# SpectacularAI/3dgs-deblur

Hardware: AMD Instinct MI355X
Metric: fwd+bwd rasterize MPix/s at 1M Gaussians, 1080p, 5 sub-poses (higher is better)
Workload: dtype f32

## Files before the change

3dgs-deblur_amd/_lib.py:

```python
from __future__ import annotations

import ctypes
from pathlib import Path

from ._build import LIB_PATH, build_library

_P, _I, _F, _L = ctypes.c_void_p, ctypes.c_int, ctypes.c_float, ctypes.c_longlong

_SIGS = {
    "gs_subpose_viewmats_fwd": [_I, _P, _P, _P, _P, _P, _P],
    "gs_subpose_viewmats_bwd": [_I, _P, _P, _P, _P, _P, _P, _P, _P, _P],
    "gs_project_fwd": [_I, _P, _P, _F, _P, _P, _F, _F, _F, _F, _I, _I, _F, _P, _P, _P, _P, _P, _P, _P, _P, _P],
    "gs_project_bwd": [_I, _P, _P, _F, _P, _P, _F, _F, _F, _F, _I, _I, _F, _P, _P, _P, _P, _P, _P, _P, _P, _I, _P, _L, _P],
    "gs_sh_fwd": [_I, _I, _I, _P, _P, _P, _P],
    "gs_sh_bwd": [_I, _I, _I, _P, _P, _P, _P],
    "gs_project_fused_fwd": [_I, _I, _P, _P, _F, _P, _P, _P, _I, _I, _P, _F, _F, _F, _F, _I, _I, _F, _I, _I,
                             _P, _P, _P, _P, _P, _I, _P],
    "gs_slice_colors": [_I, _P, _P, _I, _P, _P, _P, _I, _I, _P, _P, _P],
    "gs_project_fused_bwd": [_I, _I, _P, _P, _F, _P, _P, _P, _I, _I, _P, _F, _F, _F, _F, _I, _I, _F, _I,
                             _P, _P, _P, _P, _P, _P, _P, _P, _P, _P, _I, _P, _I, _P, _P, _L, _P],
    "gs_project_pixvel_fwd": [_I, _I, _P, _P, _F, _P, _P, _P, _I, _I, _P, _P, _P, _F, _F, _F, _F, _I, _I, _F, _I, _I,
                              _P, _P, _P, _P, _F, _P, _P, _I, _P],
    "gs_rasterize_fwd_rs_slice": [_P, _P, _P, _P, _I, _I, _I, _P, _P, _P, _P, _P, _I, _I, _P, _I, _P, _P, _P, _I, _F, _P,
                                  _P],
    "gs_rasterize_bwd_rs_slice": [_P, _P, _P, _P, _P, _I, _I, _I, _P, _P, _P, _P, _P, _P, _P, _P, _P, _I, _I, _P, _F, _F,
                                  _P, _I, _F, _P, _P],
    "gs_project_pixvel_bwd": [_I, _I, _P, _P, _F, _P, _P, _P, _I, _I, _P, _P, _P, _F, _F, _F, _F, _I, _I, _F, _I,
                              _P, _P, _P, _P, _P, _P, _P, _P, _P, _P, _P, _I, _P, _I, _P, _P, _L, _P],
    "gs_pack_records": [_I, _P, _P, _P, _P, _P, _P, _I, _I, _P, _P, _P, _P],
    "gs_unpack_record_grads": [_I, _P, _P, _P, _P, _P, _P],
    "gs_exclusive_scan_u32": [_L, _P, _P, _P, _P, _L, _P],
    "gs_radix_sort_pairs_u32": [_L, _P, _P, _P, _P, _I, _I, _I, _P, _L, ctypes.POINTER(_I), _P],
    "gs_radix_sort_pairs_u64": [_L, _P, _P, _P, _P, _I, _I, _I, _P, _L, ctypes.POINTER(_I), _P],
    "gs_radix_sort_pairs_gather_u32": [_L, _P, _P, _P, _P, _I, _I, _I, _P, _L, ctypes.POINTER(_I), _P, _P, _P, _P],
    "gs_radix_sort_pairs_carry_u32": [_L, _P, _P, _P, _P, _I, _I, _I, _P, _L, ctypes.POINTER(_I), _P, _P, _P,
                                      ctypes.POINTER(_I), _P, _P],
    "gs_segmented_sort_pairs_u32": [_L, _L, _P, _P, _P, _P, _I, _I, _I, _P, _L, ctypes.POINTER(_I), _P],
    "gs_segmented_sort_compact_u32": [_L, _L, _P, _P, _P, _P, _I, _I, _I, ctypes.c_uint, _P, _P, _P, _P, _L,
                                      ctypes.POINTER(_I), _P],
    "gs_segmented_sort_select_u32": [_L, _L, _P, _P, _P, _P, _P, _I, _I, _I, ctypes.c_uint, _P, _P, _P, _P, _P, _P, _L,
                                     ctypes.POINTER(_I), _L, _P],
    "gs_depth_select": [_L, _L, _P, _P, _L, _P, _P, _P, _L, _P],
    "gs_exclusive_scan_segments_u32": [_L, _L, _P, _P, _P, _P, _P, _L, _P],
    "gs_make_depth_keys64": [_L, _I, _P, _P, _P],
    "gs_gather_counts": [_L, _P, _P, _P, _P],
    "gs_emit_intersects": [_L, _I, _I, _I, _P, _P, _P, _L, _P, _P, ctypes.c_uint, _P],
    "gs_tile_bin_edges_u32": [_L, _P, _I, _P, _P, _P],
    "gs_tile_bin_edges_u64": [_L, _P, _I, _P, _P],
    "gs_tile_bin_edges_ids_u32": [_L, _P, _I, _P, _P, _P, _P, _P],
    "gs_map_gaussian_to_intersects": [_I, _P, _P, _P, _P, _I, _I, _P, _P, _P],
    "gs_rasterize_fwd": [_P, _P, _P, _P, _P, _I, _I, _I, _I, _P, _P, _P, _I, _I, _P],
    "gs_rasterize_bwd": [_P, _P, _P, _P, _P, _I, _I, _I, _I, _P, _P, _P, _P, _P, _I, _I, _P],
    "gs_slice_plan": [_I, _I, _I, _P, _P, _L, _P, _P, _P, _P, _P, _P],
    "gs_slice_plan_select": [_I, _I, _I, _P, _P, _P, _P, _P, _P, _P, _P, _P],
    "gs_tile_open_sat": [_I, _I, _I, _P, _P, _P, _P, _P],
    "gs_slice_counts": [_I, _I, _I, _P, _P, _P, _P, _P, _I, _I, _P, _P, _P],
    "gs_emit_open_intersects": [_I, _I, _I, _I, _P, _P, _P, _P, _P, _P, _P, ctypes.c_uint, _I, _I, _P, _P, _P, _P],
    "gs_slice_counts_exact": [_I, _I, _I, _P, _P, _P, _P, _P, _P, _I, _I, _P, _P, _I, _P, _P, _P, _P, _P, _P],
    "gs_slice_counts_exact_swept": [_I, _I, _I, _P, _P, _P, _P, _P, _P, _I, _I, _P, _P, _I, _P, _P, _P, _P, _P, _F, _F, _F,
                                    _P],
    "gs_rasterize_fwd_slice": [_P, _P, _P, _P, _P, _I, _I, _I, _I, _P, _P, _P, _P, _P, _I, _I, _P, _P, _I, _P, _P, _P,
                               _I, _P],
    "gs_rasterize_bwd_slice": [_P, _P, _P, _P, _P, _I, _I, _I, _I, _P, _P, _P, _P, _P, _P, _P, _P, _P, _P, _P, _I, _P,
                               _I, _P, _F, _F, _P],
    "gs_rasterize_fwd_slice_stats": [_P, _P, _P, _P, _P, _I, _I, _I, _I, _P, _P, _P, _P, _P, _I, _I, _P, _P, _P, _P],
    "gs_reduce_grad_tuples": [_I, _P, _P, _P, _P, _P, _P, _P, _L, _P, _I, _P],
    "gs_combine_fwd": [_I, _L, _P, _F, _F, _P, _P],
    "gs_combine_bwd": [_I, _L, _P, _F, _F, _P, _P, _P, _P],
    "gs_combine_bwd_scale": [_I, _L, _F, _P, _P, _P, _P],
    "gs_combine_fwd_batched": [_I, _I, _L, _P, _F, _F, _P, _P],
    "gs_combine_bwd_batched": [_I, _I, _L, _P, _F, _F, _P, _P, _P, _P],
    "gs_combine_bwd_scale_batched": [_I, _I, _L, _F, _P, _P, _P, _P],
    "gs_dp_row_mask": [_I, _I, _P, _P, _P, _P],
    "gs_dp_pack_rows": [_L, _P, _I, _P, _P, _P, _P],
    "gs_dp_scatter_add_rows": [_L, _P, _I, _P, _P, _F, _P],
    "gs_dp_pack_masked_rows": [_I, _P, _P, _I, _P, _I, _P, _P, _P, _P],
    "gs_dp_scatter_add_payload": [_I, _P, _I, _P, _P, _F, _P],
    "gs_slice_project_records": [_I, _I, _I, _P, _P, _P, _P, _I, _I, _P, _P],
    "gs_project_records": [_I, _I, _P, _I, _I, _P, _P],
    "gs_frame_forward": [_P, _P, _P, _P, _P, _P, _P, _P, _P, _P, _I, _I, _P, _P, _P, _P, _P, _P, _P, _P, _L, _P, _L, _P, _P],
    "gs_frame_backward": [_P, _P, _P, _P, _P, _P, _P, _P, _F, _F, _I, _P, _P, _P, _P, _P, _L, _P],
    "gs_frame_backward_depth": [_P, _P, _P, _P, _P, _P, _P, _P, _F, _F, _I, _P, _P, _P, _P, _P, _L, _P, _P],
    "gs_xy_absgrad_sum": [_I, _I, _I, _P, _P, _P, _P],
    "gs_frame_profile_enable": [ctypes.c_uint],
    "gs_frame_profile_read": [_I, _P, _P],
    "gs_image_loss_fwd_bwd": [_I, _I, _P, _P, _F, _P, _P, _P, _L, _P],
    "gs_adam_step": [_I, _P, _P, _P, _P, _P, _P, ctypes.c_double, ctypes.c_double, ctypes.c_double, _I, _P],
    "gs_adam_step_rows": [_I, _I, _P, _P, _P, _P, _P, _P, _P, ctypes.c_double, ctypes.c_double, ctypes.c_double, _I,
                          _P, _L, _P],
    "gs_visible_rows": [_I, _I, _P, _P, _P],
    "gs_mcmc_inject_noise": [_I, _P, _P, _P, _P, _F, _L, _L, _P, _P, _P],
    "gs_mcmc_relocation": [_I, _P, _P, _P, _P, _P, _P],
    "gs_bilagrid_slice_fwd": [_I, _I, _I, _I, _I, _I, _I, _P, _P, _P, _P, _P],
    "gs_bilagrid_slice_bwd": [_I, _I, _I, _I, _I, _I, _I, _P, _P, _P, _P, _P, _P, _P, _L, _P],
    "gs_bilagrid_tv_fwd_bwd": [_I, _I, _I, _I, _P, _F, _P, _P, _P, _L, _P],
}
_SIGS_LL = {
    "gs_scan_workspace_bytes": [_L],
    "gs_radix_sort_workspace_bytes": [_L, _I, _I],
    "gs_segmented_sort_workspace_bytes": [_L, _L, _I, _I],
    "gs_segmented_sort_compact_workspace_bytes": [_L, _L, _I, _I, _I],
    "gs_depth_select_workspace_bytes": [_I],
    "gs_project_pose_scratch_bytes": [_I, _I, _I],
    "gs_image_loss_workspace_bytes": [_I, _I],
    "gs_adam_step_rows_workspace_bytes": [_I],
    "gs_frame_backward_bytes": [_P],
    "gs_bilagrid_slice_bwd_workspace_bytes": [_I, _I, _I, _I, _I, _I, _I],
    "gs_bilagrid_tv_workspace_bytes": [_I, _I, _I, _I],
}

_lib = None


class HipLibraryError(RuntimeError):
    pass


def load(build_if_missing: bool = True) -> ctypes.CDLL:
    global _lib
    if _lib is not None:
        return _lib
    import os
    import shutil
    override = os.environ.get("GSD_LIB_PATH")
    path = Path(override) if override else LIB_PATH
    if not override and build_if_missing and shutil.which(os.environ.get("HIPCC", "/opt/rocm/bin/hipcc")):
        from ._build import is_current, HASH_PATH, CSRC
        stale = not is_current()
        if stale and path.exists() and not HASH_PATH.exists():
            t = path.stat().st_mtime
            stale = any(f.stat().st_mtime > t for f in list(CSRC.glob("*.hip")) + list(CSRC.glob("*.h")))
        if stale:
            import fcntl
            try:
                lock = open(str(path) + ".lock", "w")
            except OSError as e:
                if not path.exists():
                    raise HipLibraryError(f"{path} is missing and {path.parent} is not writable: {e}") from e
                import warnings
                warnings.warn(f"{path} may be older than its sources and {path.parent} is not writable; loading it as is")
            else:
                with lock:
                    fcntl.flock(lock, fcntl.LOCK_EX)
                    try:
                        build_library()
                    finally:
                        fcntl.flock(lock, fcntl.LOCK_UN)
    if not path.exists():
        raise HipLibraryError(f"{path} is missing; run __graft_entry__.build()")
    try:
        lib = ctypes.CDLL(str(path))
    except OSError as e:
        raise HipLibraryError(f"cannot load HIP library {path}: {e}") from e
    for name, args in _SIGS.items():
        fn = getattr(lib, name)
        fn.argtypes = args
        fn.restype = _I
    for name, args in _SIGS_LL.items():
        fn = getattr(lib, name)
        fn.argtypes = args
        fn.restype = _L
    lib.gs_version.restype = ctypes.c_char_p
    lib.gs_version.argtypes = []
    _lib = lib
    return lib


def exported_names():
    return sorted(list(_SIGS) + list(_SIGS_LL) + ["gs_version"])


def check(status: int, what: str) -> None:
    if status != 0:
# ... 5 lines not shown
```

3dgs-deblur_amd/csrc/project.hip:

```cpp
#include "gs_common.h"
#include "../../include/gsdeblur.h"

namespace gs {

__global__ void subpose_fwd_kernel(int P, const float* __restrict__ V0, const float* __restrict__ lin,
                                   const float* __restrict__ ang, const float* __restrict__ times,
                                   float* __restrict__ out) {
  int p = blockIdx.x * blockDim.x + threadIdx.x;
  if (p >= P) return;
  float v0[12], l[3], a[3], o[12];
  for (int j = 0; j < 12; ++j) v0[j] = V0[j];
  for (int j = 0; j < 3; ++j) { l[j] = lin[j]; a[j] = ang[j]; }
  subpose_viewmat<float>(v0, l, a, times[p], o);
  for (int j = 0; j < 12; ++j) out[16 * p + j] = o[j];
  out[16 * p + 12] = 0.f; out[16 * p + 13] = 0.f; out[16 * p + 14] = 0.f; out[16 * p + 15] = 1.f;
}

__global__ __launch_bounds__(256) void subpose_bwd_kernel(int P, const float* __restrict__ V0, const float* __restrict__ lin,
                                   const float* __restrict__ ang, const float* __restrict__ times,
                                   const float* __restrict__ v_out, float* __restrict__ v_V0,
                                   float* __restrict__ v_lin, float* __restrict__ v_ang) {
  typedef Dual<1> D;
  extern __shared__ float sp_part[];
  for (int gid = threadIdx.x; gid < P * 18; gid += blockDim.x) {
    const int p = gid / 18, t = gid - p * 18;
    D dV[12], dl[3], da[3], o[12];
    for (int j = 0; j < 12; ++j) { dV[j] = D(V0[j]); dV[j].d[0] = (j == t) ? 1.f : 0.f; }
    for (int j = 0; j < 3; ++j) {
      dl[j] = D(lin[j]); dl[j].d[0] = (12 + j == t) ? 1.f : 0.f;
      da[j] = D(ang[j]); da[j].d[0] = (15 + j == t) ? 1.f : 0.f;
    }
    subpose_viewmat<D>(dV, dl, da, D(times[p]), o);
    float acc = 0.f;
    for (int j = 0; j < 12; ++j) acc += v_out[16 * p + j] * o[j].d[0];
    sp_part[gid] = acc;
  }
  __syncthreads();
  if (threadIdx.x < 18) {
    const int t = threadIdx.x;
    float sum = 0.f;
    for (int p = 0; p < P; ++p) sum += sp_part[p * 18 + t];
    float* dst = t < 12 ? v_V0 + t : (t < 15 ? v_lin + (t - 12) : v_ang + (t - 15));
    *dst += sum;
  }
}

struct Intrin { float fx, fy, cx, cy; int W, H, tiles_x, tiles_y; float clip; };

__global__ __launch_bounds__(256) void project_fwd_kernel(int N, const float* __restrict__ means,
    const float* __restrict__ scales, float glob, const float* __restrict__ quats, const float* __restrict__ V,
    Intrin in, float* __restrict__ xys, float* __restrict__ depths, int* __restrict__ radii,
    float* __restrict__ conics, float* __restrict__ comp, int* __restrict__ ntiles, float* __restrict__ cov3d,
    int* __restrict__ tbounds) {
  int i = blockIdx.x * blockDim.x + threadIdx.x;
  if (i >= N) return;
  float Vm[12];
  for (int j = 0; j < 12; ++j) Vm[j] = V[j];
  float m[3] = {means[3 * i], means[3 * i + 1], means[3 * i + 2]};
  float s[3] = {scales[3 * i], scales[3 * i + 1], scales[3 * i + 2]};
  float q[4] = {quats[4 * i], quats[4 * i + 1], quats[4 * i + 2], quats[4 * i + 3]};
  float R[9], qn[4], inv, M[9], c3[6];
  quat_to_rotmat(q, R, qn, &inv);
  scale_rot_to_cov3d(s, glob, R, M, c3);
  Proj o; ProjCtx k;
  bool ok = project_one(m, c3, Vm, in.fx, in.fy, in.cx, in.cy, in.W, in.H, in.tiles_x, in.tiles_y, in.clip, o, k);
  for (int j = 0; j < 6; ++j) cov3d[6 * i + j] = c3[j];
  depths[i] = o.depth;
  radii[i] = ok ? o.radius : 0;
  ntiles[i] = ok ? o.ntiles : 0;
  xys[2 * i] = ok ? o.x : 0.f; xys[2 * i + 1] = ok ? o.y : 0.f;
  conics[3 * i] = ok ? o.conic_x : 0.f; conics[3 * i + 1] = ok ? o.conic_y : 0.f; conics[3 * i + 2] = ok ? o.conic_z : 0.f;
  comp[i] = ok ? o.comp : 0.f;
  if (tbounds) {
    tbounds[4 * i] = o.tmin_x; tbounds[4 * i + 1] = o.tmin_y; tbounds[4 * i + 2] = o.tmax_x; tbounds[4 * i + 3] = o.tmax_y;
  }
}

__device__ __forceinline__ void reduce_vV(const float vV[12], float* __restrict__ acc , float* lds ) {
  const int lane = lane_id(), wave = threadIdx.x >> 6;
#pragma unroll
  for (int j = 0; j < 12; ++j) {
    float t = wave_sum_to_lane63(vV[j]);
    if (lane == 63) lds[wave * 12 + j] = t;
  }
  __syncthreads();
  if (threadIdx.x < 12) acc[threadIdx.x] += (lds[threadIdx.x] + lds[12 + threadIdx.x]) + (lds[24 + threadIdx.x] + lds[36 + threadIdx.x]);
  __syncthreads();
}

struct PoseDst { float* slot0; float* slot1; int stride; };
__global__ __launch_bounds__(256) void pose_reduce_kernel(const float* __restrict__ partial, int nblocks, int slots,
                                                          PoseDst dst) {
  __shared__ double red[256][13];
  const int sl = blockIdx.x;
  float* out = (sl == 1 && dst.slot1) ? dst.slot1 : dst.slot0 + (size_t)sl * dst.stride;
  if (!out) return;
  double a[12];
#pragma unroll
  for (int j = 0; j < 12; ++j) a[j] = 0.0;
  for (int b = threadIdx.x; b < nblocks; b += 256) {
    const float* row = partial + ((size_t)b * slots + sl) * 12;
#pragma unroll
    for (int j = 0; j < 12; ++j) a[j] += (double)row[j];
  }
#pragma unroll
  for (int j = 0; j < 12; ++j) red[threadIdx.x][j] = a[j];
  __syncthreads();
  for (int w = 128; w > 0; w >>= 1) {
    if ((int)threadIdx.x < w)
#pragma unroll
      for (int j = 0; j < 12; ++j) red[threadIdx.x][j] += red[threadIdx.x + w][j];
    __syncthreads();
  }
  if (threadIdx.x < 12) out[threadIdx.x] += (float)red[0][threadIdx.x];
}

__global__ __launch_bounds__(256) void project_bwd_kernel(int N, const float* __restrict__ means,
    const float* __restrict__ scales, float glob, const float* __restrict__ quats, const float* __restrict__ V,
    Intrin in, const float* __restrict__ v_xys, const float* __restrict__ v_depths,
    const float* __restrict__ v_conics, const float* __restrict__ v_comp, float* __restrict__ v_means,
    float* __restrict__ v_scales, float* __restrict__ v_quats, float* __restrict__ v_V ,
    int flags) {
  __shared__ float lds[48];
  __shared__ float acc[12];
  if (threadIdx.x < 12) acc[threadIdx.x] = 0.f;
  int i = blockIdx.x * blockDim.x + threadIdx.x;
  float vV[12];
  for (int j = 0; j < 12; ++j) vV[j] = 0.f;
  if (i < N) {
    float Vm[12];
    for (int j = 0; j < 12; ++j) Vm[j] = V[j];
    float m[3] = {means[3 * i], means[3 * i + 1], means[3 * i + 2]};
    float s[3] = {scales[3 * i], scales[3 * i + 1], scales[3 * i + 2]};
    float q[4] = {quats[4 * i], quats[4 * i + 1], quats[4 * i + 2], quats[4 * i + 3]};
    float R[9], qn[4], inv, M[9], c3[6];
    quat_to_rotmat(q, R, qn, &inv);
    scale_rot_to_cov3d(s, glob, R, M, c3);
    Proj o; ProjCtx k;
    bool ok = project_one(m, c3, Vm, in.fx, in.fy, in.cx, in.cy, in.W, in.H, in.tiles_x, in.tiles_y, in.clip, o, k);
    float vm[3] = {0.f, 0.f, 0.f}, vs[3] = {0.f, 0.f, 0.f}, vq[4] = {0.f, 0.f, 0.f, 0.f};
    if (ok) {
      float vxy[2] = {v_xys[2 * i], v_xys[2 * i + 1]};
      float vc[3] = {v_conics[3 * i], v_conics[3 * i + 1], v_conics[3 * i + 2]};
      float vc3[6];
      project_one_bwd(m, c3, Vm, in.fx, in.fy, k, o.comp, vxy, v_depths ? v_depths[i] : 0.f, vc,
                      v_comp ? v_comp[i] : 0.f, vm, vc3, vV, nullptr, (flags & 1) != 0);
      cov3d_bwd(s, glob, q, vc3, vs, vq, (flags & 2) != 0);
    }
    for (int j = 0; j < 3; ++j) { v_means[3 * i + j] = vm[j]; v_scales[3 * i + j] = vs[j]; }
    for (int j = 0; j < 4; ++j) v_quats[4 * i + j] = vq[j];
  }
  if (v_V) {
    __syncthreads();
    reduce_vV(vV, acc, lds);
    if (threadIdx.x < 12) v_V[(size_t)blockIdx.x * 12 + threadIdx.x] = acc[threadIdx.x];
  }
}

__global__ __launch_bounds__(256) void sh_fwd_kernel(int N, int K_stride, int deg, const float* __restrict__ dirs,
                                                     const float* __restrict__ coeffs, float* __restrict__ colors) {
  int i = blockIdx.x * blockDim.x + threadIdx.x;
  if (i >= N) return;
  float x = dirs[3 * i], y = dirs[3 * i + 1], z = dirs[3 * i + 2];
  float inv = 1.0f / sqrtf(x * x + y * y + z * z);
  float B[25];
  sh_basis(deg, x * inv, y * inv, z * inv, B);
  int nb = (deg + 1) * (deg + 1);
  float r = 0.f, g = 0.f, b = 0.f;
  const float* c = coeffs + (size_t)i * K_stride * 3;
#pragma unroll
  for (int k = 0; k < 25; ++k)
    if (k < nb) { r += B[k] * c[3 * k]; g += B[k] * c[3 * k + 1]; b += B[k] * c[3 * k + 2]; }
  colors[3 * i] = r; colors[3 * i + 1] = g; colors[3 * i + 2] = b;
}

__global__ __launch_bounds__(256) void sh_bwd_kernel(int N, int K_stride, int deg, const float* __restrict__ dirs,
                                                     const float* __restrict__ v_colors, float* __restrict__ v_coeffs) {
  int i = blockIdx.x * blockDim.x + threadIdx.x;
  if (i >= N) return;
  float x = dirs[3 * i], y = dirs[3 * i + 1], z = dirs[3 * i + 2];
  float inv = 1.0f / sqrtf(x * x + y * y + z * z);
  float B[25];
  sh_basis(deg, x * inv, y * inv, z * inv, B);
  int nb = (deg + 1) * (deg + 1);
  float r = v_colors[3 * i], g = v_colors[3 * i + 1], b = v_colors[3 * i + 2];
  float* c = v_coeffs + (size_t)i * K_stride * 3;
#pragma unroll
  for (int k = 0; k < 25; ++k) {
    if (k < K_stride) {
      float bk = k < nb ? B[k] : 0.f;
      c[3 * k] = bk * r; c[3 * k + 1] = bk * g; c[3 * k + 2] = bk * b;
    }
  }
  for (int k = 25; k < K_stride; ++k) { c[3 * k] = 0.f; c[3 * k + 1] = 0.f; c[3 * k + 2] = 0.f; }
}

__device__ __forceinline__ void tile_bbox(float x, float y, int radius, int tiles_x, int tiles_y, int& x0, int& y0,
                                          int& x1, int& y1) {
  const float inv_tile = 1.0f / (float)K::kTile;
  float radf = (float)radius;
  float tcx = x * inv_tile, tcy = y * inv_tile, tr = radf * inv_tile;
  x0 = (int)(tcx - tr); x1 = (int)(tcx + tr + 1.0f);
  y0 = (int)(tcy - tr); y1 = (int)(tcy + tr + 1.0f);
  x0 = x0 < 0 ? 0 : (x0 > tiles_x ? tiles_x : x0);
  x1 = x1 < 0 ? 0 : (x1 > tiles_x ? tiles_x : x1);
  y0 = y0 < 0 ? 0 : (y0 > tiles_y ? tiles_y : y0);
  y1 = y1 < 0 ? 0 : (y1 > tiles_y ? tiles_y : y1);
}

__global__ __launch_bounds__(256) void pack_records_kernel(int N, const float* __restrict__ xys,
    const float* __restrict__ depths, const int* __restrict__ radii, const float* __restrict__ conics,
    const float* __restrict__ colors, const float* __restrict__ opacity, int tiles_x, int tiles_y,
    float* __restrict__ records, unsigned* __restrict__ depth_keys, int* __restrict__ ntiles) {
  int i = blockIdx.x * blockDim.x + threadIdx.x;
  if (i >= N) return;
  int rad = radii[i];
  int x0 = 0, y0 = 0, x1 = 0, y1 = 0;
  float x = xys[2 * i], y = xys[2 * i + 1];
  if (rad > 0) tile_bbox(x, y, rad, tiles_x, tiles_y, x0, y0, x1, y1);
  int area = (x1 - x0) * (y1 - y0);
  bool ok = rad > 0 && area > 0;
  float4* r = reinterpret_cast<float4*>(records + (size_t)i * kRecFloats);
  float d = depths[i];
  if (ok) {
    r[0] = make_float4(x, y, conics[3 * i], conics[3 * i + 1]);
    r[1] = make_float4(conics[3 * i + 2], opacity[i], colors[3 * i], colors[3 * i + 1]);
    r[2] = make_float4(colors[3 * i + 2], d, __int_as_float(x0 | (y0 << 16)), __int_as_float(x1 | (y1 << 16)));
    float aux[4];
    rec_aux(opacity[i], conics[3 * i], conics[3 * i + 2], aux);
    r[3] = make_float4(aux[0], aux[1], aux[2], aux[3]);
  } else {
    r[0] = make_float4(0.f, 0.f, 0.f, 0.f); r[1] = r[0]; r[2] = r[0]; r[3] = r[0];
  }
  depth_keys[i] = ok ? (unsigned)__float_as_int(d) : 0xFFFFFFFFu;
  ntiles[i] = ok ? area : 0;
}

__global__ __launch_bounds__(256) void unpack_grads_kernel(int N, const float* __restrict__ v_records,
    float* __restrict__ v_xys, float* __restrict__ v_conics, float* __restrict__ v_colors,
    float* __restrict__ v_opacity) {
  int i = blockIdx.x * blockDim.x + threadIdx.x;
  if (i >= N) return;
  const float4* r = reinterpret_cast<const float4*>(v_records + (size_t)i * kGradFloats);
  float4 a = r[0], b = r[1], c = r[2];
  v_xys[2 * i] = a.x; v_xys[2 * i + 1] = a.y;
  v_conics[3 * i] = a.z; v_conics[3 * i + 1] = a.w; v_conics[3 * i + 2] = b.x;
  v_opacity[i] = b.y;
  v_colors[3 * i] = b.z; v_colors[3 * i + 1] = b.w; v_colors[3 * i + 2] = c.x;
}

struct FusedParams {
  int N, P;
  const float* means; const float* scales; const float* quats; const float* opacities;
  const float* sh;
  const float* viewmats;
  float glob;
  int K_stride, deg, antialiased;
  int defer_color;
  int skip_culled;
  int no_records;
  int records_only;
  int rs_bands;
  Intrin in;
  int pixvel;
  const float* twist;
  const float* times;
  int flags;
  float rs_half;
  float* pix_vel_out;
  int act;
  const float* sh_rest;
};
constexpr int GS_ACT_LOG_SCALES = 1, GS_ACT_OPACITY_LOGITS = 2;

__device__ __forceinline__ void load_scales(const FusedParams& fp, int i, float s[3]) {
  s[0] = fp.scales[3 * i]; s[1] = fp.scales[3 * i + 1]; s[2] = fp.scales[3 * i + 2];
  if (fp.act & GS_ACT_LOG_SCALES) { s[0] = expf(s[0]); s[1] = expf(s[1]); s[2] = expf(s[2]); }
}
__device__ __forceinline__ float load_opacity(const FusedParams& fp, int i) {
  const float o = fp.opacities[i];
  return (fp.act & GS_ACT_OPACITY_LOGITS) ? 1.0f / (1.0f + expf(-o)) : o;
}
__device__ __forceinline__ void sh_rows(const float* __restrict__ sh, const float* __restrict__ sh_rest, int K_stride,
                                        size_t i, const float*& c0, const float*& c1) {
  if (sh_rest) { c0 = sh + i * 3; c1 = sh_rest + i * (size_t)(K_stride - 1) * 3; }
  else { c0 = sh + i * (size_t)K_stride * 3; c1 = c0 + 3; }
}

constexpr int GS_FLAG_UPSTREAM_FOV_CLAMP_GRAD = 1;
constexpr int GS_FLAG_RAW_QUAT_GRAD = 2;
constexpr int GS_FLAG_NO_NEEDLE_HP = 8;
constexpr int GS_FLAG_RS_PIXVEL_GRAD = 16;
constexpr int GS_FLAG_DEPTH_GRAD = 64;
constexpr float kNeedleRatio = 8.0f;

template <int MAXB, bool DEFER>
__global__ __launch_bounds__(256) void project_fused_fwd_kernel(FusedParams fp, float* __restrict__ records,
    unsigned* __restrict__ depth_keys, int* __restrict__ ntiles, int* __restrict__ radii) {
  int i = blockIdx.x * blockDim.x + threadIdx.x;
  if (i >= fp.N) return;
  float m[3] = {fp.means[3 * i], fp.means[3 * i + 1], fp.means[3 * i + 2]};
  float s[3];
  load_scales(fp, i, s);
  float q[4] = {fp.quats[4 * i], fp.quats[4 * i + 1], fp.quats[4 * i + 2], fp.quats[4 * i + 3]};
  float opac = load_opacity(fp, i);
  float R[9], qn[4], inv, M[9], c3[6];
  quat_to_rotmat(q, R, qn, &inv);
  scale_rot_to_cov3d(s, fp.glob, R, M, c3);
  const int nb = (fp.deg + 1) * (fp.deg + 1);
  float coef[DEFER ? 1 : MAXB * 3];
  if (!DEFER) {
    const float *c0, *c1;
    sh_rows(fp.sh, fp.sh_rest, fp.K_stride, (size_t)i, c0, c1);
#pragma unroll
    for (int k = 0; k < MAXB * 3; ++k) coef[DEFER ? 0 : k] = (k < nb * 3) ? (k < 3 ? c0[k] : c1[k - 3]) : 0.f;
  }
  Proj o0; ProjCtx k0;
  float pv[2] = {0.f, 0.f};
  if (fp.pixvel) {
    float Vm0[12];
#pragma unroll
    for (int j = 0; j < 12; ++j) Vm0[j] = fp.viewmats[j];
    project_one(m, c3, Vm0, fp.in.fx, fp.in.fy, fp.in.cx, fp.in.cy, fp.in.W, fp.in.H, fp.in.tiles_x, fp.in.tiles_y,
                fp.in.clip, o0, k0);
    if (k0.geom_ok) {
      const float lin[3] = {fp.twist[0], fp.twist[1], fp.twist[2]}, ang[3] = {fp.twist[3], fp.twist[4], fp.twist[5]};
      pixel_velocity(k0.pc, k0.clamp_x ? k0.tx : k0.pc[0], k0.clamp_y ? k0.ty : k0.pc[1], k0.rz, fp.in.fx, fp.in.fy,
                     lin, ang, pv);
    }
    if (fp.pix_vel_out) { fp.pix_vel_out[2 * i] = pv[0]; fp.pix_vel_out[2 * i + 1] = pv[1]; }
  }
  for (int p = 0; p < fp.P; ++p) {
    const float* V = fp.viewmats + (fp.pixvel ? 0 : 16 * p);
    float Vm[12];
#pragma unroll
    for (int j = 0; j < 12; ++j) Vm[j] = V[j];
    Proj o; ProjCtx k;
    bool ok;
    if (fp.pixvel) {
      o = o0; k = k0;
      ok = k0.geom_ok != 0;
      if (ok) {
        const float tau = fp.times[p];
        o.x = o0.x + tau * pv[0];
        o.y = o0.y + tau * pv[1];
        o.radius = (int)k0.radf;
        if (fp.rs_half != 0.f)
          ok = tile_bounds_swept(o.x - fp.rs_half * pv[0], o.y - fp.rs_half * pv[1], o.x + fp.rs_half * pv[0],
                                 o.y + fp.rs_half * pv[1], k0.radf, fp.in.tiles_x, fp.in.tiles_y, o);
        else
          ok = tile_bounds(o.x, o.y, k0.radf, fp.in.tiles_x, fp.in.tiles_y, o);
      }
    } else {
      ok = project_one(m, c3, Vm, fp.in.fx, fp.in.fy, fp.in.cx, fp.in.cy, fp.in.W, fp.in.H, fp.in.tiles_x,
                       fp.in.tiles_y, fp.in.clip, o, k);
    }
    size_t idx = (size_t)p * fp.N + i;
    float4* r = reinterpret_cast<float4*>(records + idx * kRecFloats);
    const int radius_out = ok ? o.radius : 0;
    if (ok && fp.rs_bands > 1) {
      const int rb = p % fp.rs_bands;
      const int by0 = (rb * fp.in.tiles_y) / fp.rs_bands, by1 = ((rb + 1) * fp.in.tiles_y) / fp.rs_bands;
      o.tmin_y = max(o.tmin_y, by0);
      o.tmax_y = min(o.tmax_y, by1);
      ok = o.tmax_y > o.tmin_y;
      o.ntiles = ok ? (o.tmax_x - o.tmin_x) * (o.tmax_y - o.tmin_y) : 0;
    }
    if (fp.no_records) {
    } else if (ok) {
      float cxw = -(Vm[0] * Vm[3] + Vm[4] * Vm[7] + Vm[8] * Vm[11]);
      float cyw = -(Vm[1] * Vm[3] + Vm[5] * Vm[7] + Vm[9] * Vm[11]);
      float czw = -(Vm[2] * Vm[3] + Vm[6] * Vm[7] + Vm[10] * Vm[11]);
      float dx = m[0] - cxw, dy = m[1] - cyw, dz = m[2] - czw;
      float dinv = 1.0f / sqrtf(dx * dx + dy * dy + dz * dz);
      float cr = 0.f, cg = 0.f, cb = 0.f;
      if (!DEFER) {
        float B[MAXB];
        sh_basis(fp.deg, dx * dinv, dy * dinv, dz * dinv, B);
        cr = 0.5f; cg = 0.5f; cb = 0.5f;
#pragma unroll
        for (int b = 0; b < MAXB; ++b) {
          if (b < nb) {
            cr += B[b] * coef[DEFER ? 0 : 3 * b]; cg += B[b] * coef[DEFER ? 0 : 3 * b + 1];
            cb += B[b] * coef[DEFER ? 0 : 3 * b + 2];
          }
        }
        cr = fmaxf(cr, 0.f); cg = fmaxf(cg, 0.f); cb = fmaxf(cb, 0.f);
      }
      float op = fp.antialiased ? opac * o.comp : opac;
      float aux[4];
      rec_aux(op, o.conic_x, o.conic_z, aux);
      r[0] = make_float4(o.x, o.y, o.conic_x, o.conic_y);
      if (fp.records_only) {
        float* rf = reinterpret_cast<float*>(r);
        rf[4] = o.conic_z; rf[5] = op; rf[9] = o.depth;
        rf[10] = __int_as_float(o.tmin_x | (o.tmin_y << 16)); rf[11] = __int_as_float(o.tmax_x | (o.tmax_y << 16));
      } else {
        r[1] = make_float4(o.conic_z, op, cr, cg);
        r[2] = make_float4(cb, o.depth, __int_as_float(o.tmin_x | (o.tmin_y << 16)),
                           __int_as_float(o.tmax_x | (o.tmax_y << 16)));
      }
      r[3] = make_float4(aux[0], aux[1], aux[2], aux[3]);
    } else if (!fp.skip_culled) {
      float4 z = make_float4(0.f, 0.f, 0.f, 0.f);
      r[0] = z; r[1] = z; r[2] = z; r[3] = z;
    }
    if (fp.records_only) continue;
    depth_keys[idx] = ok ? (unsigned)__float_as_int(o.depth) : 0xFFFFFFFFu;
    ntiles[idx] = ok ? o.ntiles : 0;
    if (radii) radii[idx] = radius_out;
  }
}

struct FusedOut {
  float* v_means; float* v_scales; float* v_quats; float* v_opac; float* v_sh; float* v_sh_rest;
  float* v_viewmats;
  float* v_xy_sum;
  float* v_twist;
  float* pose_partial;
};

template <int MAXB, bool DEPTH>
__device__ __forceinline__ void fused_bwd_body(const FusedParams& fp, const float* __restrict__ records,
    const float* __restrict__ v_records, const FusedOut& out, const unsigned char* __restrict__ touched,
    int i, bool live, float* lds, float* __restrict__ blk_acc ) {
  float* __restrict__ v_means = out.v_means; float* __restrict__ v_scales = out.v_scales;
  float* __restrict__ v_quats = out.v_quats; float* __restrict__ v_opac = out.v_opac;
  float* __restrict__ v_sh = out.v_sh; float* __restrict__ v_sh_rest = out.v_sh_rest;
  float* __restrict__ v_viewmats = out.v_viewmats; float* __restrict__ v_xy_sum = out.v_xy_sum;
  float* __restrict__ v_twist = out.v_twist;
  const int ii = live ? i : 0;
  float m[3] = {0.f, 0.f, 1.f}, s[3] = {1.f, 1.f, 1.f}, q[4] = {1.f, 0.f, 0.f, 0.f}, opac = 0.f;
  if (live) {
    m[0] = fp.means[3 * ii]; m[1] = fp.means[3 * ii + 1]; m[2] = fp.means[3 * ii + 2];
    load_scales(fp, ii, s);
    q[0] = fp.quats[4 * ii]; q[1] = fp.quats[4 * ii + 1]; q[2] = fp.quats[4 * ii + 2]; q[3] = fp.quats[4 * ii + 3];
    opac = load_opacity(fp, ii);
  }
  float R[9], qn[4], inv, M[9], c3[6];
  quat_to_rotmat(q, R, qn, &inv);
  scale_rot_to_cov3d(s, fp.glob, R, M, c3);
  const int nb = (fp.deg + 1) * (fp.deg + 1);
  float vcoef[MAXB * 3];
#pragma unroll
  for (int k = 0; k < MAXB * 3; ++k) vcoef[k] = 0.f;
  float vm[3] = {0.f, 0.f, 0.f}, vc3[6] = {0.f, 0.f, 0.f, 0.f, 0.f, 0.f}, vop = 0.f, vxs = 0.f, vys = 0.f;
  const bool up_clamp = (fp.flags & GS_FLAG_UPSTREAM_FOV_CLAMP_GRAD) != 0;
  if (fp.pixvel) {
    float Vm[12];
#pragma unroll
    for (int j = 0; j < 12; ++j) Vm[j] = fp.viewmats[j];
    float vV[12], vtw[12];
#pragma unroll
    for (int j = 0; j < 12; ++j) { vV[j] = 0.f; vtw[j] = 0.f; }
    bool mine = false;
    if (live)
      for (int p = 0; p < fp.P; ++p) mine |= (!touched || touched[(size_t)p * fp.N + ii]);
    if (mine) {
      Proj o; ProjCtx k;
      project_one(m, c3, Vm, fp.in.fx, fp.in.fy, fp.in.cx, fp.in.cy, fp.in.W, fp.in.H, fp.in.tiles_x, fp.in.tiles_y,
                  fp.in.clip, o, k);
      if (k.geom_ok) {
        float vxy[2] = {0.f, 0.f}, vpv[2] = {0.f, 0.f}, vcon[3] = {0.f, 0.f, 0.f}, v_comp = 0.f;
        float vr = 0.f, vg = 0.f, vb = 0.f, vz = 0.f;
        for (int p = 0; p < fp.P; ++p) {
          if (touched && !touched[(size_t)p * fp.N + ii]) continue;
          const float tau = fp.times[p];
          size_t idx = (size_t)p * fp.N + ii;
          const float4* g4 = reinterpret_cast<const float4*>(v_records + idx * kGradFloats);
          float4 ga = g4[0], gb = g4[1], gc = g4[2];
          const float4* r4 = reinterpret_cast<const float4*>(records + idx * kRecFloats);
          float4 ra = r4[0], rb = r4[1], rc = r4[2];
          if (ra.z == 0.f && ra.w == 0.f && rb.x == 0.f) continue;
          vr += rb.z > 0.f ? gb.z : 0.f; vg += rb.w > 0.f ? gb.w : 0.f; vb += rc.x > 0.f ? gc.x : 0.f;
          if (fp.antialiased) { vop += gb.y * o.comp; v_comp += gb.y * opac; } else { vop += gb.y; }
          vxy[0] += ga.x; vxy[1] += ga.y;
          vpv[0] += tau * ga.x; vpv[1] += tau * ga.y;
          if (fp.flags & GS_FLAG_RS_PIXVEL_GRAD) { vpv[0] += gc.y; vpv[1] += gc.z; }
          vcon[0] += ga.z; vcon[1] += ga.w; vcon[2] += gb.x;
          if (DEPTH) vz += gc.w;
        }
        vxs = vxy[0]; vys = vxy[1];
        if (vr != 0.f || vg != 0.f || vb != 0.f) {
          float cxw = -(Vm[0] * Vm[3] + Vm[4] * Vm[7] + Vm[8] * Vm[11]);
          float cyw = -(Vm[1] * Vm[3] + Vm[5] * Vm[7] + Vm[9] * Vm[11]);
          float czw = -(Vm[2] * Vm[3] + Vm[6] * Vm[7] + Vm[10] * Vm[11]);
          float dx = m[0] - cxw, dy = m[1] - cyw, dz = m[2] - czw;
          float dinv = 1.0f / sqrtf(dx * dx + dy * dy + dz * dz);
          float B[MAXB];
          sh_basis(fp.deg, dx * dinv, dy * dinv, dz * dinv, B);
#pragma unroll
          for (int b = 0; b < MAXB; ++b) {
            if (b < nb) { vcoef[3 * b] += B[b] * vr; vcoef[3 * b + 1] += B[b] * vg; vcoef[3 * b + 2] += B[b] * vb; }
          }
        }
        const float lin[3] = {fp.twist[0], fp.twist[1], fp.twist[2]}, ang[3] = {fp.twist[3], fp.twist[4], fp.twist[5]};
        float vpc[3], vlin[3], vang[3];
        pixel_velocity_bwd(k.pc, k.clamp_x ? k.tx : k.pc[0], k.clamp_y ? k.ty : k.pc[1], k.clamp_x, k.clamp_y, up_clamp,
                           k.rz, fp.in.fx, fp.in.fy, lin, ang, vpv, vpc, vlin, vang);
        vtw[0] = vlin[0]; vtw[1] = vlin[1]; vtw[2] = vlin[2]; vtw[3] = vang[0]; vtw[4] = vang[1]; vtw[5] = vang[2];
        project_one_bwd(m, c3, Vm, fp.in.fx, fp.in.fy, k, o.comp, vxy, DEPTH ? vz : 0.f, vcon, v_comp, vm, vc3, vV, vpc,
                        up_clamp);
      }
    }
    if (__syncthreads_or(mine)) {
      if (v_viewmats) reduce_vV(vV, blk_acc, lds);
      if (v_twist) reduce_vV(vtw, blk_acc + 12, lds);
    }
  } else
  for (int p = 0; p < fp.P; ++p) {
    const float* V = fp.viewmats + 16 * p;
    float Vm[12];
#pragma unroll
    for (int j = 0; j < 12; ++j) Vm[j] = V[j];
    float vV[12];
#pragma unroll
    for (int j = 0; j < 12; ++j) vV[j] = 0.f;
    const bool mine = live && (!touched || touched[(size_t)p * fp.N + ii]);
    if (mine) {
      Proj o; ProjCtx k;
      bool ok = project_one(m, c3, Vm, fp.in.fx, fp.in.fy, fp.in.cx, fp.in.cy, fp.in.W, fp.in.H, fp.in.tiles_x,
                            fp.in.tiles_y, fp.in.clip, o, k);
      if (ok) {
        size_t idx = (size_t)p * fp.N + ii;
        const float4* g4 = reinterpret_cast<const float4*>(v_records + idx * kGradFloats);
        float4 ga = g4[0], gb = g4[1], gc = g4[2];
        const float4* r4 = reinterpret_cast<const float4*>(records + idx * kRecFloats);
        float4 rb = r4[1], rc = r4[2];
        float vr = rb.z > 0.f ? gb.z : 0.f, vg = rb.w > 0.f ? gb.w : 0.f, vb = rc.x > 0.f ? gc.x : 0.f;
        if (vr != 0.f || vg != 0.f || vb != 0.f) {
          float cxw = -(Vm[0] * Vm[3] + Vm[4] * Vm[7] + Vm[8] * Vm[11]);
          float cyw = -(Vm[1] * Vm[3] + Vm[5] * Vm[7] + Vm[9] * Vm[11]);
          float czw = -(Vm[2] * Vm[3] + Vm[6] * Vm[7] + Vm[10] * Vm[11]);
          float dx = m[0] - cxw, dy = m[1] - cyw, dz = m[2] - czw;
          float dinv = 1.0f / sqrtf(dx * dx + dy * dy + dz * dz);
          float B[MAXB];
          sh_basis(fp.deg, dx * dinv, dy * dinv, dz * dinv, B);
#pragma unroll
          for (int b = 0; b < MAXB; ++b) {
            if (b < nb) { vcoef[3 * b] += B[b] * vr; vcoef[3 * b + 1] += B[b] * vg; vcoef[3 * b + 2] += B[b] * vb; }
          }
        }
        float v_comp = 0.f;
        if (fp.antialiased) { vop += gb.y * o.comp; v_comp = gb.y * opac; } else { vop += gb.y; }
        float vxy[2] = {ga.x, ga.y};
        vxs += ga.x; vys += ga.y;
        float vcon[3] = {ga.z, ga.w, gb.x};
        float vm1[3], vc31[6];
        project_one_bwd(m, c3, Vm, fp.in.fx, fp.in.fy, k, o.comp, vxy, DEPTH ? gc.w : 0.f, vcon, v_comp, vm1, vc31, vV,
                        nullptr, up_clamp);
        for (int j = 0; j < 3; ++j) vm[j] += vm1[j];
        for (int j = 0; j < 6; ++j) vc3[j] += vc31[j];
      }
    }
    if (v_viewmats && __syncthreads_or(mine)) reduce_vV(vV, blk_acc + 12 * p, lds);
  }
  if (!live) return;
  float vs[3], vq[4];
  cov3d_bwd(s, fp.glob, q, vc3, vs, vq, (fp.flags & GS_FLAG_RAW_QUAT_GRAD) != 0);
  if (fp.act & GS_ACT_LOG_SCALES) { vs[0] *= s[0]; vs[1] *= s[1]; vs[2] *= s[2]; }
  if (fp.act & GS_ACT_OPACITY_LOGITS) vop *= opac * (1.0f - opac);
  for (int j = 0; j < 3; ++j) { v_means[3 * i + j] = vm[j]; v_scales[3 * i + j] = vs[j]; }
  for (int j = 0; j < 4; ++j) v_quats[4 * i + j] = vq[j];
  v_opac[i] = vop;
  if (v_xy_sum) { v_xy_sum[2 * i] = vxs; v_xy_sum[2 * i + 1] = vys; }
  float *c0, *c1;
  if (v_sh_rest) { c0 = v_sh + (size_t)i * 3; c1 = v_sh_rest + (size_t)i * (fp.K_stride - 1) * 3; }
  else { c0 = v_sh + (size_t)i * fp.K_stride * 3; c1 = c0 + 3; }
  const int kn = fp.K_stride * 3;
#pragma unroll
  for (int k = 0; k < MAXB * 3; ++k)
    if (k < kn) { if (k < 3) c0[k] = vcoef[k]; else c1[k - 3] = vcoef[k]; }
  for (int k = MAXB * 3; k < kn; ++k) c1[k - 3] = 0.f;
}

template <bool DEPTH>
__device__ __forceinline__ void needle_item_se3(const FusedParams& fp, const float* __restrict__ records,
                                                const float* __restrict__ v_records,
                                                const unsigned char* __restrict__ touched, int i, int p, double out[9]) {
#pragma unroll
  for (int j = 0; j < 9; ++j) out[j] = 0.0;
  if (touched && !touched[(size_t)p * fp.N + i]) return;
  float s[3];
  load_scales(fp, i, s);
  const float m[3] = {fp.means[3 * i], fp.means[3 * i + 1], fp.means[3 * i + 2]};
  const float q[4] = {fp.quats[4 * i], fp.quats[4 * i + 1], fp.quats[4 * i + 2], fp.quats[4 * i + 3]};
  float R[9], qn[4], inv, M[9], c3[6];
  quat_to_rotmat(q, R, qn, &inv);
  scale_rot_to_cov3d(s, fp.glob, R, M, c3);
  const float* V = fp.viewmats + 16 * p;
  float Vm[12];
#pragma unroll
  for (int j = 0; j < 12; ++j) Vm[j] = V[j];
  Proj o; ProjCtx k;
  if (!project_one(m, c3, Vm, fp.in.fx, fp.in.fy, fp.in.cx, fp.in.cy, fp.in.W, fp.in.H, fp.in.tiles_x, fp.in.tiles_y,
                   fp.in.clip, o, k))
    return;
  double Rd[9], qnd[4], invd, Md[9], c3d[6];
  quat_to_rotmat_t<double>(q, Rd, qnd, &invd);
  scale_rot_to_cov3d_t<double>(s, fp.glob, Rd, Md, c3d);
  ProjCtxT<double> kd;
  project_ctx_t<double>(m, c3d, Vm, fp.in.fx, fp.in.fy, fp.in.W, fp.in.H, kd);
  kd.clamp_x = k.clamp_x; kd.clamp_y = k.clamp_y;
  const double comp = ::sqrt(fmax(0.0, kd.det0 / kd.det));
  const size_t idx = (size_t)p * fp.N + i;
  const float4* g4 = reinterpret_cast<const float4*>(v_records + idx * kGradFloats);
  const float4 ga = g4[0], gb = g4[1];
  const double vxy[2] = {ga.x, ga.y}, vcon[3] = {ga.z, ga.w, gb.x};
  const double v_comp = fp.antialiased ? (double)gb.y * (double)load_opacity(fp, i) : 0.0;
  const double vz = DEPTH ? (double)g4[2].w : 0.0;
  double vV[12];
  project_one_bwd_t<double>(m, c3d, Vm, fp.in.fx, fp.in.fy, kd, comp, vxy, vz, vcon, v_comp, out, out + 3, vV, nullptr,
                            (fp.flags & GS_FLAG_UPSTREAM_FOV_CLAMP_GRAD) != 0);
}

template <bool DEPTH>
__device__ __forceinline__ void needle_item_pixvel(const FusedParams& fp, const float* __restrict__ records,
                                                   const float* __restrict__ v_records,
                                                   const unsigned char* __restrict__ touched, int i, double out[9]) {
#pragma unroll
  for (int j = 0; j < 9; ++j) out[j] = 0.0;
  float s[3];
  load_scales(fp, i, s);
  const float m[3] = {fp.means[3 * i], fp.means[3 * i + 1], fp.means[3 * i + 2]};
  const float q[4] = {fp.quats[4 * i], fp.quats[4 * i + 1], fp.quats[4 * i + 2], fp.quats[4 * i + 3]};
  const float opac = load_opacity(fp, i);
  float R[9], qn[4], inv, M[9], c3[6];
  quat_to_rotmat(q, R, qn, &inv);
  scale_rot_to_cov3d(s, fp.glob, R, M, c3);
  float Vm[12];
#pragma unroll
  for (int j = 0; j < 12; ++j) Vm[j] = fp.viewmats[j];
  Proj o; ProjCtx k;
  project_one(m, c3, Vm, fp.in.fx, fp.in.fy, fp.in.cx, fp.in.cy, fp.in.W, fp.in.H, fp.in.tiles_x, fp.in.tiles_y,
              fp.in.clip, o, k);
  if (!k.geom_ok) return;
  double Rd[9], qnd[4], invd, Md[9], c3d[6];
  quat_to_rotmat_t<double>(q, Rd, qnd, &invd);
  scale_rot_to_cov3d_t<double>(s, fp.glob, Rd, Md, c3d);
  ProjCtxT<double> kd;
  project_ctx_t<double>(m, c3d, Vm, fp.in.fx, fp.in.fy, fp.in.W, fp.in.H, kd);
  kd.clamp_x = k.clamp_x; kd.clamp_y = k.clamp_y;
  const double comp = ::sqrt(fmax(0.0, kd.det0 / kd.det));
  double vxy[2] = {0., 0.}, vcon[3] = {0., 0., 0.}, v_comp = 0., vz = 0.;
  float vpv[2] = {0.f, 0.f};
  for (int p = 0; p < fp.P; ++p) {
    if (touched && !touched[(size_t)p * fp.N + i]) continue;
    const size_t idx = (size_t)p * fp.N + i;
    const float4* g4 = reinterpret_cast<const float4*>(v_records + idx * kGradFloats);
    const float4 ga = g4[0], gb = g4[1], gc = g4[2];
    const float4* r4 = reinterpret_cast<const float4*>(records + idx * kRecFloats);
    const float4 ra = r4[0], rb = r4[1];
    if (ra.z == 0.f && ra.w == 0.f && rb.x == 0.f) continue;
    if (fp.antialiased) v_comp += (double)gb.y * (double)opac;
    vxy[0] += ga.x; vxy[1] += ga.y;
    vpv[0] += fp.times[p] * ga.x; vpv[1] += fp.times[p] * ga.y;
    if (fp.flags & GS_FLAG_RS_PIXVEL_GRAD) { vpv[0] += gc.y; vpv[1] += gc.z; }
    vcon[0] += ga.z; vcon[1] += ga.w; vcon[2] += gb.x;
    if (DEPTH) vz += (double)gc.w;
  }
  const float lin[3] = {fp.twist[0], fp.twist[1], fp.twist[2]}, ang[3] = {fp.twist[3], fp.twist[4], fp.twist[5]};
  float vpc[3], vlin[3], vang[3];
  pixel_velocity_bwd(k.pc, k.clamp_x ? k.tx : k.pc[0], k.clamp_y ? k.ty : k.pc[1], k.clamp_x, k.clamp_y,
                     (fp.flags & GS_FLAG_UPSTREAM_FOV_CLAMP_GRAD) != 0, k.rz, fp.in.fx, fp.in.fy, lin, ang, vpv, vpc,
                     vlin, vang);
  const double vpcd[3] = {vpc[0], vpc[1], vpc[2]};
  double vV[12];
  project_one_bwd_t<double>(m, c3d, Vm, fp.in.fx, fp.in.fy, kd, comp, vxy, vz, vcon, v_comp, out, out + 3, vV, vpcd,
                            (fp.flags & GS_FLAG_UPSTREAM_FOV_CLAMP_GRAD) != 0);
}

constexpr int kNeedleChunk = 2048;

#define GS_NEEDLE_HP_KERNEL(NAME, DEPTH)                                                                                \
__global__ __launch_bounds__(256) void NAME(FusedParams fp, const float* __restrict__ records,                          \
    const float* __restrict__ v_records, float* __restrict__ v_means, float* __restrict__ v_scales,                    \
    float* __restrict__ v_quats, const unsigned char* __restrict__ touched, float ratio_limit) {                       \
  __shared__ int list[kNeedleChunk];                                                                                          \
  __shared__ int n_list;                                                                                                      \
  __shared__ double part[256][9];                                                                                             \
  if (threadIdx.x == 0) n_list = 0;                                                                                           \
  __syncthreads();                                                                                                            \
  const int i0 = blockIdx.x * kNeedleChunk + (int)threadIdx.x * 8;                                                            \
  if (i0 < fp.N) {                                                                                                            \
    unsigned long long any = ~0ull;                                                                                           \
    if (touched) {                                                                                                            \
      any = 0ull;                                                                                                             \
      const bool word = (fp.N % 8) == 0 && i0 + 8 <= fp.N;                                                                    \
      for (int p = 0; p < fp.P; ++p) {                                                                                        \
        const unsigned char* t = touched + (size_t)p * fp.N + i0;                                                             \
        if (word) any |= *reinterpret_cast<const unsigned long long*>(t);                                                     \
        else for (int j = 0; j < 8 && i0 + j < fp.N; ++j) any |= (unsigned long long)t[j] << (8 * j);                         \
      }                                                                                                                       \
    }                                                                                                                         \
    if (any != 0ull) {                                                                                                        \
      for (int j = 0; j < 8 && i0 + j < fp.N; ++j) {                                                                          \
        if (((any >> (8 * j)) & 0xFFull) == 0ull) continue;                                                                   \
        const int i = i0 + j;                                                                                                 \
                                                             \
        const float s0 = fp.scales[3 * i], s1 = fp.scales[3 * i + 1], s2 = fp.scales[3 * i + 2];                              \
        const float smax = fmaxf(s0, fmaxf(s1, s2)), smin = fminf(s0, fminf(s1, s2));                                         \
        const bool needle = (fp.act & GS_ACT_LOG_SCALES) ? (smax - smin > __logf(ratio_limit)) : (smax > ratio_limit * smin); \
        if (needle) list[atomicAdd(&n_list, 1)] = i;                                                                          \
      }                                                                                                                       \
    }                                                                                                                         \
  }                                                                                                                           \
  __syncthreads();                                                                                                            \
  const int n = n_list;                                                                                                       \
  if (n == 0) return;                                                                                                         \
  const int items_per = fp.pixvel ? 1 : fp.P;                                                      \
  const int per_round = max(1, 256 / items_per);                                                       \
  for (int base = 0; base < n; base += per_round) {                                                                           \
    const int cnt = min(per_round, n - base);                                                                                 \
    const int a = (int)threadIdx.x / items_per, p = (int)threadIdx.x - a * items_per;                                         \
    if (a < cnt) {                                                                                                            \
      double o9[9];                                                                                                           \
      if (fp.pixvel) needle_item_pixvel<DEPTH>(fp, records, v_records, touched, list[base + a], o9);                          \
      else needle_item_se3<DEPTH>(fp, records, v_records, touched, list[base + a], p, o9);                                    \
_Pragma("unroll")                                                                                                             \
      for (int j = 0; j < 9; ++j) part[threadIdx.x][j] = o9[j];                                                               \
    }                                                                                                                         \
    __syncthreads();                                                                                                          \
    if ((int)threadIdx.x < cnt) {                                                                                             \
      const int i = list[base + threadIdx.x];                                                                                 \
      double acc[9] = {0., 0., 0., 0., 0., 0., 0., 0., 0.};                                                                   \
      for (int pp = 0; pp < items_per; ++pp)                                                                                  \
_Pragma("unroll")                                                                                                             \
        for (int j = 0; j < 9; ++j) acc[j] += part[threadIdx.x * items_per + pp][j];                                          \
      float s[3];                                                                                                             \
  load_scales(fp, i, s);                                                                                                      \
      const float q[4] = {fp.quats[4 * i], fp.quats[4 * i + 1], fp.quats[4 * i + 2], fp.quats[4 * i + 3]};                    \
      double vs[3], vq[4];                                                                                                    \
      cov3d_bwd_t<double>(s, fp.glob, q, acc + 3, vs, vq, (fp.flags & GS_FLAG_RAW_QUAT_GRAD) != 0);                           \
      if (fp.act & GS_ACT_LOG_SCALES) { vs[0] *= (double)s[0]; vs[1] *= (double)s[1]; vs[2] *= (double)s[2]; }                \
      for (int j = 0; j < 3; ++j) { v_means[3 * i + j] = (float)acc[j]; v_scales[3 * i + j] = (float)vs[j]; }                 \
      for (int j = 0; j < 4; ++j) v_quats[4 * i + j] = (float)vq[j];                                                          \
    }                                                                                                                         \
    __syncthreads();                                                                                                          \
  }                                                                                                                           \
}

GS_NEEDLE_HP_KERNEL(project_needle_hp_kernel, false)
GS_NEEDLE_HP_KERNEL(project_needle_hp_depth_kernel, true)

#define GS_FUSED_BWD_KERNEL(NAME, DEPTH)                                                                                \
template <int MAXB>                                                                                                     \
__global__ __launch_bounds__(256) void NAME(FusedParams fp, const float* __restrict__ records,                          \
    const float* __restrict__ v_records, FusedOut out) {                                                                \
  __shared__ float lds[48];                                                                                               \
  extern __shared__ float blk_acc[];                        \
  const int slots = out.pose_partial ? (fp.pixvel ? 2 : fp.P) : 0;                                                        \
  for (int k = threadIdx.x; k < slots * 12; k += 256) blk_acc[k] = 0.f;                                                   \
  __syncthreads();                                                                                                        \
  const int i = blockIdx.x * blockDim.x + threadIdx.x;                                                                    \
  fused_bwd_body<MAXB, DEPTH>(fp, records, v_records, out, nullptr, i, i < fp.N, lds, blk_acc);                           \
  __syncthreads();                                                                                                        \
  for (int k = threadIdx.x; k < slots * 12; k += 256) out.pose_partial[(size_t)blockIdx.x * slots * 12 + k] = blk_acc[k]; \
}

GS_FUSED_BWD_KERNEL(project_fused_bwd_kernel, false)
GS_FUSED_BWD_KERNEL(project_fused_bwd_depth_kernel, true)

constexpr int kFusedChunk = 2048;

__device__ __forceinline__ void zero_rows(float* __restrict__ base, size_t first, size_t count) {
  if (!base || count == 0) return;
  float* p = base + first;
  const size_t mis = ((reinterpret_cast<uintptr_t>(p) & 15u) != 0) ? ((16u - (reinterpret_cast<uintptr_t>(p) & 15u)) >> 2) : 0;
  const size_t head = mis < count ? mis : count;
  for (size_t k = threadIdx.x; k < head; k += blockDim.x) p[k] = 0.f;
  const size_t n4 = (count - head) >> 2;
  float4* p4 = reinterpret_cast<float4*>(p + head);
  for (size_t k = threadIdx.x; k < n4; k += blockDim.x) p4[k] = make_float4(0.f, 0.f, 0.f, 0.f);
  for (size_t k = head + 4 * n4 + threadIdx.x; k < count; k += blockDim.x) p[k] = 0.f;
}

#define GS_FUSED_BWD_SPARSE_KERNEL(NAME, DEPTH)                                                                         \
template <int MAXB, bool ZERO_FILL>                                                                                     \
__global__ __launch_bounds__(256, 2) void NAME(FusedParams fp,                                                          \
    const float* __restrict__ records, const float* __restrict__ v_records, FusedOut out,                               \
    const unsigned char* __restrict__ touched ) {                                                            \
  __shared__ float lds[48];                                                                                               \
  __shared__ int list[kFusedChunk];                                                                                       \
  __shared__ int wave_cnt[4];                                                                                             \
  extern __shared__ float blk_acc[];                        \
  const int slots = out.pose_partial ? (fp.pixvel ? 2 : fp.P) : 0;                                                        \
  for (int k = threadIdx.x; k < slots * 12; k += 256) blk_acc[k] = 0.f;                                                   \
  const int lane = lane_id(), wave = threadIdx.x >> 6;                                                                    \
  const int base = blockIdx.x * kFusedChunk;                                                                              \
  if (ZERO_FILL) {                                                                                                        \
    const size_t g0 = (size_t)base, cnt = (size_t)min(kFusedChunk, fp.N - base);                                          \
    zero_rows(out.v_means, 3 * g0, 3 * cnt);                                                                              \
    zero_rows(out.v_scales, 3 * g0, 3 * cnt);                                                                             \
    zero_rows(out.v_quats, 4 * g0, 4 * cnt);                                                                              \
    zero_rows(out.v_opac, g0, cnt);                                                                                       \
    if (out.v_sh_rest) {                                                                                                  \
      zero_rows(out.v_sh, 3 * g0, 3 * cnt);                                                                               \
      zero_rows(out.v_sh_rest, (size_t)(fp.K_stride - 1) * 3 * g0, (size_t)(fp.K_stride - 1) * 3 * cnt);                  \
    } else {                                                                                                              \
      zero_rows(out.v_sh, (size_t)fp.K_stride * 3 * g0, (size_t)fp.K_stride * 3 * cnt);                                   \
    }                                                                                                                     \
    zero_rows(out.v_xy_sum, 2 * g0, 2 * cnt);                                                                             \
                   \
    __threadfence_block();                                                                                                \
  }                                                                                                                       \
  int n_list = 0;                                                                                                         \
  for (int r = 0; r < kFusedChunk / 256; ++r) {                                                                           \
    const int g = base + r * 256 + (int)threadIdx.x;                                                                      \
    bool any = false;                                                                                                     \
    if (g < fp.N)                                                                                                         \
      for (int p = 0; p < fp.P; ++p) any |= touched[(size_t)p * fp.N + g] != 0;                                           \
    const unsigned long long bal = __ballot(any);                                                                         \
    if (lane == 0) wave_cnt[wave] = __popcll(bal);                                                                        \
    __syncthreads();                                                                                                      \
    int off = n_list, total = 0;                                                                                          \
_Pragma("unroll")                                                                                                         \
    for (int w = 0; w < 4; ++w) { const int c = wave_cnt[w]; if (w < wave) off += c; total += c; }                        \
    if (any) list[off + __popcll(bal & ((1ull << lane) - 1ull))] = g;                                                     \
    n_list += total;                                                                                                      \
    __syncthreads();                                                                                                      \
  }                                                                                                                       \
  for (int k0 = 0; k0 < n_list; k0 += 256) {                                                                              \
    const int k = k0 + (int)threadIdx.x;                                                                                  \
    const bool live = k < n_list;                                                                                         \
    fused_bwd_body<MAXB, DEPTH>(fp, records, v_records, out, touched, live ? list[k] : 0, live, lds, blk_acc);            \
  }                                                                                                                       \
  __syncthreads();                                                                                                        \
  for (int k = threadIdx.x; k < slots * 12; k += 256) out.pose_partial[(size_t)blockIdx.x * slots * 12 + k] = blk_acc[k]; \
}

GS_FUSED_BWD_SPARSE_KERNEL(project_fused_bwd_sparse_kernel, false)
GS_FUSED_BWD_SPARSE_KERNEL(project_fused_bwd_sparse_depth_kernel, true)

__global__ __launch_bounds__(256) void slice_records_kernel(int n_slice, SliceDesc sd, const unsigned* __restrict__ sorted_gi,
                                                            FusedParams fp, float* __restrict__ records) {
  const int j = blockIdx.x * 256 + threadIdx.x;
  if (j >= n_slice) return;
  const unsigned gi = sorted_gi[slice_rank(sd, j)];
  const int p = (int)(gi / (unsigned)fp.N), i = (int)(gi - (unsigned)p * (unsigned)fp.N);
  float m[3] = {fp.means[3 * i], fp.means[3 * i + 1], fp.means[3 * i + 2]};
  float sc[3];
  load_scales(fp, i, sc);
  float q[4] = {fp.quats[4 * i], fp.quats[4 * i + 1], fp.quats[4 * i + 2], fp.quats[4 * i + 3]};
  const float opac = load_opacity(fp, i);
  float R[9], qn[4], inv, M[9], c3[6];
  quat_to_rotmat(q, R, qn, &inv);
  scale_rot_to_cov3d(sc, fp.glob, R, M, c3);
  const float* V = fp.viewmats + 16 * p;
  float Vm[12];
#pragma unroll
  for (int k = 0; k < 12; ++k) Vm[k] = V[k];
  Proj o; ProjCtx k;
  bool ok = project_one(m, c3, Vm, fp.in.fx, fp.in.fy, fp.in.cx, fp.in.cy, fp.in.W, fp.in.H, fp.in.tiles_x,
                        fp.in.tiles_y, fp.in.clip, o, k);
  if (ok && fp.rs_bands > 1) {
    const int rb = p % fp.rs_bands;
    const int by0 = (rb * fp.in.tiles_y) / fp.rs_bands, by1 = ((rb + 1) * fp.in.tiles_y) / fp.rs_bands;
    o.tmin_y = max(o.tmin_y, by0);
    o.tmax_y = min(o.tmax_y, by1);
    ok = o.tmax_y > o.tmin_y;
  }
  float4* r = reinterpret_cast<float4*>(records + (size_t)gi * kRecFloats);
  if (ok) {
    const float op = fp.antialiased ? opac * o.comp : opac;
    float aux[4];
    rec_aux(op, o.conic_x, o.conic_z, aux);
    r[0] = make_float4(o.x, o.y, o.conic_x, o.conic_y);
    r[1] = make_float4(o.conic_z, op, 0.f, 0.f);
    r[2] = make_float4(0.f, o.depth, __int_as_float(o.tmin_x | (o.tmin_y << 16)),
                       __int_as_float(o.tmax_x | (o.tmax_y << 16)));
    r[3] = make_float4(aux[0], aux[1], aux[2], aux[3]);
  } else {
    const float4 z = make_float4(0.f, 0.f, 0.f, 0.f);
    r[0] = z; r[1] = z; r[2] = z; r[3] = z;
  }
}

template <int MAXB> constexpr int slice_colors_waves() { return MAXB <= 16 ? 4 : 2; }

template <int MAXB>
__global__ __launch_bounds__(256) void slice_colors_kernel(int n_slice, const unsigned* __restrict__ slice_gi,
                                                           const unsigned* __restrict__ counts, int N,
                                                           const float* __restrict__ means,
                                                           const float* __restrict__ sh,
                                                           const float* __restrict__ sh_rest, int K_stride, int deg,
                                                           const float* __restrict__ viewmats,
                                                           float* __restrict__ records) {
  constexpr int kRow = MAXB * 3 + 1;
  constexpr int kRowPad = (kRow & 1) ? kRow : kRow + 1;
  __shared__ float s_coef[slice_colors_waves<MAXB>()][64 * kRowPad];
  const int lane = threadIdx.x & 63;
  float* rows = s_coef[threadIdx.x >> 6];
  const int j = blockIdx.x * blockDim.x + threadIdx.x;
  const bool active = j < n_slice && counts[j] != 0;
  const unsigned gi = active ? slice_gi[j] : 0u;
  const unsigned p = gi / (unsigned)N, g = gi - p * (unsigned)N;
  const int nb = (deg + 1) * (deg + 1);
  const int grp = lane >> 4, q = lane & 15;
#pragma unroll 4
  for (int it = 0; it < 16; ++it) {
    const int r = it * 4 + grp;
    const unsigned g_r = (unsigned)__shfl((int)g, r);
    const int act_r = __shfl((int)active, r);
    if (act_r) {
      const float *r0, *r1;
      sh_rows(sh, sh_rest, K_stride, (size_t)g_r, r0, r1);
      for (int b = q; b < nb; b += 16) {
        const float* c = b == 0 ? r0 : r1 + 3 * (b - 1);
        const float c0 = c[0], c1 = c[1], c2 = c[2];
        float* d = rows + r * kRowPad + 3 * b;
        d[0] = c0; d[1] = c1; d[2] = c2;
      }
    }
  }
  __builtin_amdgcn_wave_barrier();
  if (!active) return;
  const float* V = viewmats + 16 * p;
  const float m0 = means[3 * g], m1 = means[3 * g + 1], m2 = means[3 * g + 2];
  float cxw = -(V[0] * V[3] + V[4] * V[7] + V[8] * V[11]);
  float cyw = -(V[1] * V[3] + V[5] * V[7] + V[9] * V[11]);
  float czw = -(V[2] * V[3] + V[6] * V[7] + V[10] * V[11]);
  float dx = m0 - cxw, dy = m1 - cyw, dz = m2 - czw;
  float dinv = 1.0f / sqrtf(dx * dx + dy * dy + dz * dz);
  float B[MAXB];
  sh_basis(deg, dx * dinv, dy * dinv, dz * dinv, B);
  const float* coef = rows + lane * kRowPad;
  float cr = 0.5f, cg = 0.5f, cb = 0.5f;
#pragma unroll
  for (int b = 0; b < MAXB; ++b) {
    if (b < nb) { cr += B[b] * coef[3 * b]; cg += B[b] * coef[3 * b + 1]; cb += B[b] * coef[3 * b + 2]; }
  }
  float* r = records + (size_t)gi * kRecFloats;
  r[6] = fmaxf(cr, 0.f); r[7] = fmaxf(cg, 0.f); r[8] = fmaxf(cb, 0.f);
}

}

using namespace gs;

static inline Intrin make_intrin(float fx, float fy, float cx, float cy, int H, int W, float clip) {
  Intrin in;
  in.fx = fx; in.fy = fy; in.cx = cx; in.cy = cy; in.W = W; in.H = H;
  in.tiles_x = (W + K::kTile - 1) / K::kTile; in.tiles_y = (H + K::kTile - 1) / K::kTile; in.clip = clip;
  return in;
}

GS_EXPORT int gs_subpose_viewmats_fwd(int P, const float* viewmat, const float* lin_vel, const float* ang_vel,
                                      const float* times, float* out_viewmats, void* stream) {
  if (P <= 0) return GS_ERR_INVALID;
  hipLaunchKernelGGL(subpose_fwd_kernel, dim3((P + 63) / 64), dim3(64), 0, (hipStream_t)stream, P, viewmat, lin_vel,
                     ang_vel, times, out_viewmats);
  return gs_launch_status();
}

GS_EXPORT int gs_subpose_viewmats_bwd(int P, const float* viewmat, const float* lin_vel, const float* ang_vel,
                                      const float* times, const float* v_out, float* v_viewmat, float* v_lin,
                                      float* v_ang, void* stream) {
  if (P <= 0) return GS_ERR_INVALID;
  hipLaunchKernelGGL(subpose_bwd_kernel, dim3(1), dim3(256), (size_t)P * 18 * sizeof(float), (hipStream_t)stream, P, viewmat, lin_vel,
                     ang_vel, times, v_out, v_viewmat, v_lin, v_ang);
  return gs_launch_status();
}

GS_EXPORT int gs_project_fwd(int N, const float* means, const float* scales, float glob_scale, const float* quats,
                             const float* viewmat, float fx, float fy, float cx, float cy, int H, int W, float clip,
                             float* xys, float* depths, int* radii, float* conics, float* comp, int* num_tiles_hit,
                             float* cov3d, int* tile_bounds, void* stream) {
  if (N <= 0) return GS_ERR_INVALID;
  Intrin in = make_intrin(fx, fy, cx, cy, H, W, clip);
  hipLaunchKernelGGL(project_fwd_kernel, dim3((N + 255) / 256), dim3(256), 0, (hipStream_t)stream, N, means, scales,
                     glob_scale, quats, viewmat, in, xys, depths, radii, conics, comp, num_tiles_hit, cov3d,
                     tile_bounds);
  return gs_launch_status();
}

GS_EXPORT int gs_project_bwd(int N, const float* means, const float* scales, float glob_scale, const float* quats,
                             const float* viewmat, float fx, float fy, float cx, float cy, int H, int W, float clip,
                             const float* v_xys, const float* v_depths, const float* v_conics, const float* v_comp,
                             float* v_means, float* v_scales, float* v_quats, float* v_viewmat, int grad_flags,
                             void* pose_scratch, long long pose_scratch_bytes_, void* stream) {
  if (N <= 0) return GS_ERR_INVALID;
  Intrin in = make_intrin(fx, fy, cx, cy, H, W, clip);
  const int blocks = (N + 255) / 256;
  if (v_viewmat && (!pose_scratch || pose_scratch_bytes_ < (long long)blocks * 12 * (long long)sizeof(float)))
    return GS_ERR_WORKSPACE;
  float* rows = v_viewmat ? reinterpret_cast<float*>(pose_scratch) : nullptr;
  hipLaunchKernelGGL(project_bwd_kernel, dim3(blocks), dim3(256), 0, (hipStream_t)stream, N, means, scales,
                     glob_scale, quats, viewmat, in, v_xys, v_depths, v_conics, v_comp, v_means, v_scales, v_quats,
                     rows, grad_flags);
  if (v_viewmat)
    hipLaunchKernelGGL(pose_reduce_kernel, dim3(1), dim3(256), 0, (hipStream_t)stream, rows, blocks, 1,
                       PoseDst{v_viewmat, nullptr, 0});
  return gs_launch_status();
}

GS_EXPORT int gs_sh_fwd(int N, int K_stride, int degrees_to_use, const float* dirs, const float* coeffs,
                        float* colors, void* stream) {
  if (N <= 0 || degrees_to_use < 0 || degrees_to_use > 4 || (degrees_to_use + 1) * (degrees_to_use + 1) > K_stride)
    return GS_ERR_INVALID;
  hipLaunchKernelGGL(sh_fwd_kernel, dim3((N + 255) / 256), dim3(256), 0, (hipStream_t)stream, N, K_stride,
                     degrees_to_use, dirs, coeffs, colors);
  return gs_launch_status();
}

GS_EXPORT int gs_sh_bwd(int N, int K_stride, int degrees_to_use, const float* dirs, const float* v_colors,
                        float* v_coeffs, void* stream) {
  if (N <= 0 || degrees_to_use < 0 || degrees_to_use > 4 || (degrees_to_use + 1) * (degrees_to_use + 1) > K_stride)
    return GS_ERR_INVALID;
  hipLaunchKernelGGL(sh_bwd_kernel, dim3((N + 255) / 256), dim3(256), 0, (hipStream_t)stream, N, K_stride,
                     degrees_to_use, dirs, v_colors, v_coeffs);
  return gs_launch_status();
}

GS_EXPORT int gs_pack_records(int N, const float* xys, const float* depths, const int* radii, const float* conics,
                              const float* colors, const float* opacity, int H, int W, float* records,
                              unsigned* depth_keys, int* ntiles, void* stream) {
  if (N <= 0) return GS_ERR_INVALID;
  int tiles_x = (W + K::kTile - 1) / K::kTile, tiles_y = (H + K::kTile - 1) / K::kTile;
  hipLaunchKernelGGL(pack_records_kernel, dim3((N + 255) / 256), dim3(256), 0, (hipStream_t)stream, N, xys, depths,
                     radii, conics, colors, opacity, tiles_x, tiles_y, records, depth_keys, ntiles);
  return gs_launch_status();
}

GS_EXPORT int gs_unpack_record_grads(int N, const float* v_records, float* v_xys, float* v_conics, float* v_colors,
                                     float* v_opacity, void* stream) {
  if (N <= 0) return GS_ERR_INVALID;
  hipLaunchKernelGGL(unpack_grads_kernel, dim3((N + 255) / 256), dim3(256), 0, (hipStream_t)stream, N, v_records,
                     v_xys, v_conics, v_colors, v_opacity);
  return gs_launch_status();
}

static inline FusedParams make_fused(int N, int P, const float* means, const float* scales, float glob,
                                     const float* quats, const float* opac, const float* sh, int K_stride, int deg,
                                     const float* viewmats, float fx, float fy, float cx, float cy, int H, int W,
                                     float clip, int antialiased, int defer_color = 0) {
  FusedParams fp;
  fp.N = N; fp.P = P; fp.means = means; fp.scales = scales; fp.quats = quats; fp.opacities = opac; fp.sh = sh;
  fp.viewmats = viewmats; fp.glob = glob; fp.K_stride = K_stride; fp.deg = deg; fp.antialiased = antialiased;
  fp.defer_color = defer_color & 1;
  fp.skip_culled = (defer_color >> 1) & 1;
  fp.no_records = (defer_color >> 4) & 1;
  fp.records_only = 0;
  fp.rs_bands = (defer_color & 4) ? ((defer_color >> 8) & 0xFFFF) : 0;
  fp.in = make_intrin(fx, fy, cx, cy, H, W, clip);
  fp.pixvel = 0; fp.twist = nullptr; fp.times = nullptr; fp.flags = 0; fp.rs_half = 0.f; fp.pix_vel_out = nullptr;
  fp.act = 0; fp.sh_rest = nullptr;
  return fp;
}

GS_EXPORT int gs_project_fused_fwd(int N, int P, const float* means, const float* scales, float glob_scale,
                                   const float* quats, const float* opacities, const float* sh, int K_stride,
                                   int sh_degree, const float* viewmats, float fx, float fy, float cx, float cy,
                                   int H, int W, float clip, int antialiased, int defer_color, float* records,
                                   unsigned* depth_keys, int* num_tiles_hit, int* radii, const float* sh_rest,
                                   int param_flags, void* stream) {
  if (N <= 0 || P <= 0 || sh_degree < 0 || sh_degree > 4 || (sh_degree + 1) * (sh_degree + 1) > K_stride)
    return GS_ERR_INVALID;
  FusedParams fp = make_fused(N, P, means, scales, glob_scale, quats, opacities, sh, K_stride, sh_degree, viewmats,
                              fx, fy, cx, cy, H, W, clip, antialiased, defer_color);
  fp.act = param_flags; fp.sh_rest = sh_rest;
  dim3 grid((N + 255) / 256), block(256);
  if (fp.defer_color)
    hipLaunchKernelGGL((project_fused_fwd_kernel<16, true>), grid, block, 0, (hipStream_t)stream, fp, records,
                       depth_keys, num_tiles_hit, radii);
  else if (sh_degree <= 3)
    hipLaunchKernelGGL((project_fused_fwd_kernel<16, false>), grid, block, 0, (hipStream_t)stream, fp, records,
                       depth_keys, num_tiles_hit, radii);
  else
    hipLaunchKernelGGL((project_fused_fwd_kernel<25, false>), grid, block, 0, (hipStream_t)stream, fp, records,
                       depth_keys, num_tiles_hit, radii);
  return gs_launch_status();
}

GS_EXPORT int gs_slice_project_records(int n_slice, int P, int N, const int* slice_begin, const int* slice_prefix,
                                       const unsigned* sorted_gi, const gs_project_inputs* in, int H, int W,
                                       float* records, void* stream) {
  SliceDesc sd;
  if (n_slice <= 0 || N <= 0 || !in || !sorted_gi || !records || !make_slice_desc(P, slice_begin, slice_prefix, sd))
    return GS_ERR_INVALID;
  if (!in->means || !in->scales || !in->quats || !in->opacities || !in->viewmats) return GS_ERR_INVALID;
  FusedParams fp = make_fused(N, P, in->means, in->scales, in->glob_scale, in->quats, in->opacities, nullptr, 1, 0,
                              in->viewmats, in->fx, in->fy, in->cx, in->cy, H, W, in->clip_thresh, in->antialiased,
                              in->defer_color | 1);
  fp.act = in->param_flags;
  hipLaunchKernelGGL(slice_records_kernel, dim3((n_slice + 255) / 256), dim3(256), 0, (hipStream_t)stream, n_slice, sd,
                     sorted_gi, fp, records);
  return gs_launch_status();
}

GS_EXPORT int gs_project_records(int P, int N, const gs_project_inputs* in, int H, int W, float* records, void* stream) {
  if (P <= 0 || N <= 0 || !in || !records) return GS_ERR_INVALID;
  if (!in->means || !in->scales || !in->quats || !in->opacities || !in->viewmats) return GS_ERR_INVALID;
  FusedParams fp = make_fused(N, P, in->means, in->scales, in->glob_scale, in->quats, in->opacities, nullptr, 1, 0,
                              in->viewmats, in->fx, in->fy, in->cx, in->cy, H, W, in->clip_thresh, in->antialiased,
                              (in->defer_color | 1 | 2) & ~16);
  fp.act = in->param_flags;
  fp.records_only = 1;
  hipLaunchKernelGGL((project_fused_fwd_kernel<16, true>), dim3((N + 255) / 256), dim3(256), 0, (hipStream_t)stream, fp,
                     records, (unsigned*)nullptr, (int*)nullptr, (int*)nullptr);
  return gs_launch_status();
}

GS_EXPORT int gs_slice_colors(int n_slice, const unsigned* slice_gi, const unsigned* counts, int N,
                              const float* means, const float* sh, const float* sh_rest, int K_stride, int sh_degree,
                              const float* viewmats, float* records, void* stream) {
  if (n_slice <= 0 || N <= 0 || sh_degree < 0 || sh_degree > 4 || (sh_degree + 1) * (sh_degree + 1) > K_stride)
    return GS_ERR_INVALID;
  if (sh_degree <= 3) {
    const int th = 64 * slice_colors_waves<16>();
    hipLaunchKernelGGL(slice_colors_kernel<16>, dim3((n_slice + th - 1) / th), dim3(th), 0, (hipStream_t)stream,
                       n_slice, slice_gi, counts, N, means, sh, sh_rest, K_stride, sh_degree, viewmats, records);
  } else {
    const int th = 64 * slice_colors_waves<25>();
    hipLaunchKernelGGL(slice_colors_kernel<25>, dim3((n_slice + th - 1) / th), dim3(th), 0, (hipStream_t)stream,
                       n_slice, slice_gi, counts, N, means, sh, sh_rest, K_stride, sh_degree, viewmats, records);
  }
  return gs_launch_status();
}

constexpr int GS_FLAG_XY_PER_CAMERA = 128;
constexpr int GS_FLAG_ZERO_FILL = 32;

static long long pose_scratch_bytes(int N, int P, bool pixvel, bool with_touched) {
  const long long blocks = with_touched ? (N + kFusedChunk - 1) / kFusedChunk : (N + 255) / 256;
  return blocks * (long long)(pixvel ? 2 : P) * 12 * (long long)sizeof(float);
}

static int launch_fused_bwd(const FusedParams& fp, int sh_degree, const float* records, const float* v_records,
                            FusedOut out, const unsigned char* touched, void* scratch, long long scratch_bytes,
                            hipStream_t st) {
  dim3 block(256);
  const int N = fp.N;
  const bool pose = out.v_viewmats || out.v_twist;
  const int slots = pose ? (fp.pixvel ? 2 : fp.P) : 0;
  const size_t lds = (size_t)slots * 12 * sizeof(float);
  if (pose) {
    if (!scratch || scratch_bytes < pose_scratch_bytes(N, fp.P, fp.pixvel != 0, touched != nullptr)) return GS_ERR_WORKSPACE;
    out.pose_partial = reinterpret_cast<float*>(scratch);
  }
  dim3 grid(touched ? (N + kFusedChunk - 1) / kFusedChunk : (N + 255) / 256);
  const bool depth = (fp.flags & GS_FLAG_DEPTH_GRAD) != 0;
  if (touched) {
    const bool zf = (fp.flags & GS_FLAG_ZERO_FILL) != 0;
    if (depth) {
      if (sh_degree <= 3 && zf)
        hipLaunchKernelGGL((project_fused_bwd_sparse_depth_kernel<16, true>), grid, block, lds, st, fp, records, v_records, out, touched);
      else if (sh_degree <= 3)
        hipLaunchKernelGGL((project_fused_bwd_sparse_depth_kernel<16, false>), grid, block, lds, st, fp, records, v_records, out, touched);
      else if (zf)
        hipLaunchKernelGGL((project_fused_bwd_sparse_depth_kernel<25, true>), grid, block, lds, st, fp, records, v_records, out, touched);
      else
        hipLaunchKernelGGL((project_fused_bwd_sparse_depth_kernel<25, false>), grid, block, lds, st, fp, records, v_records, out, touched);
    } else if (sh_degree <= 3 && zf)
      hipLaunchKernelGGL((project_fused_bwd_sparse_kernel<16, true>), grid, block, lds, st, fp, records, v_records, out, touched);
    else if (sh_degree <= 3)
      hipLaunchKernelGGL((project_fused_bwd_sparse_kernel<16, false>), grid, block, lds, st, fp, records, v_records, out, touched);
    else if (zf)
      hipLaunchKernelGGL((project_fused_bwd_sparse_kernel<25, true>), grid, block, lds, st, fp, records, v_records, out, touched);
    else
      hipLaunchKernelGGL((project_fused_bwd_sparse_kernel<25, false>), grid, block, lds, st, fp, records, v_records, out, touched);
  } else {
    if (depth && sh_degree <= 3)
      hipLaunchKernelGGL(project_fused_bwd_depth_kernel<16>, grid, block, lds, st, fp, records, v_records, out);
    else if (depth)
      hipLaunchKernelGGL(project_fused_bwd_depth_kernel<25>, grid, block, lds, st, fp, records, v_records, out);
    else if (sh_degree <= 3)
      hipLaunchKernelGGL(project_fused_bwd_kernel<16>, grid, block, lds, st, fp, records, v_records, out);
    else
      hipLaunchKernelGGL(project_fused_bwd_kernel<25>, grid, block, lds, st, fp, records, v_records, out);
  }
  if (pose) {
    PoseDst dst{out.v_viewmats, fp.pixvel ? out.v_twist : nullptr, fp.pixvel ? 0 : 16};
    hipLaunchKernelGGL(pose_reduce_kernel, dim3(slots), dim3(256), 0, st, out.pose_partial, (int)grid.x, slots, dst);
  }
  if (!(fp.flags & GS_FLAG_NO_NEEDLE_HP))
  {
    if (depth)
      hipLaunchKernelGGL(project_needle_hp_depth_kernel, dim3((N + kNeedleChunk - 1) / kNeedleChunk), dim3(256), 0, st, fp,
                         records, v_records, out.v_means, out.v_scales, out.v_quats, touched, kNeedleRatio);
    else
      hipLaunchKernelGGL(project_needle_hp_kernel, dim3((N + kNeedleChunk - 1) / kNeedleChunk), dim3(256), 0, st, fp,
                         records, v_records, out.v_means, out.v_scales, out.v_quats, touched, kNeedleRatio);
  }
  return gs_launch_status();
}

__global__ __launch_bounds__(256) void xy_grad_cams_kernel(int N, int P, int B, const float* __restrict__ v_records,
                                                           const unsigned char* __restrict__ touched,
                                                           float* __restrict__ v_xy) {
  const int i = blockIdx.x * blockDim.x + threadIdx.x;
  if (i >= N) return;
  const int Pc = P / B;
  for (int b = 0; b < B; ++b) {
    float vxs = 0.f, vys = 0.f;
    for (int p = b * Pc; p < (b + 1) * Pc; ++p) {
      const size_t idx = (size_t)p * N + i;
      if (!touched[idx]) continue;
      const float2 g = *reinterpret_cast<const float2*>(v_records + idx * kGradFloats);
      vxs += g.x; vys += g.y;
    }
    *reinterpret_cast<float2*>(v_xy + ((size_t)b * N + i) * 2) = make_float2(vxs, vys);
  }
}

__global__ __launch_bounds__(256) void xy_absgrad_cams_kernel(int N, int P, int B, const float* __restrict__ v_records,
                                                              const unsigned char* __restrict__ touched,
                                                              float* __restrict__ out) {
  const int i = blockIdx.x * blockDim.x + threadIdx.x;
  if (i >= N) return;
  const int Pc = P / B;
  for (int b = 0; b < B; ++b) {
    float ax = 0.f, ay = 0.f;
    for (int p = b * Pc; p < (b + 1) * Pc; ++p) {
      const size_t idx = (size_t)p * N + i;
      if (!touched[idx]) continue;
      const float* g = v_records + idx * kGradFloats;
      ax += g[9]; ay += g[10];
    }
    *reinterpret_cast<float2*>(out + ((size_t)b * N + i) * 2) = make_float2(ax, ay);
  }
}

GS_EXPORT int gs_xy_absgrad_sum(int N, int P, int cameras, const float* v_records, const unsigned char* touched,
                                float* out, void* stream) {
  if (N <= 0 || P <= 0 || cameras < 1 || P % cameras != 0 || !v_records || !touched || !out) return GS_ERR_INVALID;
  hipLaunchKernelGGL(xy_absgrad_cams_kernel, dim3((N + 255) / 256), dim3(256), 0, (hipStream_t)stream, N, P, cameras,
                     v_records, touched, out);
  return gs_launch_status();
}

GS_EXPORT long long gs_project_pose_scratch_bytes(int N, int P, int with_touched) {
  if (N <= 0 || P <= 0) return 0;
  return pose_scratch_bytes(N, std::max(P, 2), false, with_touched != 0) + 256;
}

GS_EXPORT int gs_project_fused_bwd(int N, int P, const float* means, const float* scales, float glob_scale,
                                   const float* quats, const float* opacities, const float* sh, int K_stride,
                                   int sh_degree, const float* viewmats, float fx, float fy, float cx, float cy,
                                   int H, int W, float clip, int antialiased, const float* records,
                                   const float* v_records, float* v_means, float* v_scales, float* v_quats,
                                   float* v_opacities, float* v_sh, float* v_viewmats,
                                   const unsigned char* touched, float* v_xy_sum, int grad_flags, const float* sh_rest,
                                   int param_flags, float* v_sh_rest, void* pose_scratch, long long pose_scratch_bytes_,
                                   void* stream) {
  if (N <= 0 || P <= 0 || sh_degree < 0 || sh_degree > 4 || (sh_degree + 1) * (sh_degree + 1) > K_stride ||
      (sh_rest != nullptr) != (v_sh_rest != nullptr) || ((grad_flags & GS_FLAG_ZERO_FILL) && !touched))
    return GS_ERR_INVALID;
  FusedParams fp = make_fused(N, P, means, scales, glob_scale, quats, opacities, sh, K_stride, sh_degree, viewmats,
                              fx, fy, cx, cy, H, W, clip, antialiased);
  const bool per_cam = (grad_flags & GS_FLAG_XY_PER_CAMERA) != 0;
  const int cams = (grad_flags >> 8) & 0x1ff;
  if (per_cam && (!touched || !v_xy_sum || cams < 1 || P % cams != 0)) return GS_ERR_INVALID;
  fp.flags = per_cam ? (grad_flags & ~(GS_FLAG_XY_PER_CAMERA | (0x1ff << 8))) : grad_flags;
  fp.act = param_flags; fp.sh_rest = sh_rest;
  const FusedOut out = {v_means, v_scales, v_quats, v_opacities, v_sh, v_sh_rest, v_viewmats,
                        per_cam ? nullptr : v_xy_sum, nullptr, nullptr};
  const int rc = launch_fused_bwd(fp, sh_degree, records, v_records, out, touched, pose_scratch, pose_scratch_bytes_,
                                  (hipStream_t)stream);
  if (rc != GS_OK || !per_cam) return rc;
  hipLaunchKernelGGL(xy_grad_cams_kernel, dim3((N + 255) / 256), dim3(256), 0, (hipStream_t)stream, N, P, cams, v_records,
                     touched, v_xy_sum);
  return gs_launch_status();
}

GS_EXPORT int gs_project_pixvel_fwd(int N, int P, const float* means, const float* scales, float glob_scale,
                                    const float* quats, const float* opacities, const float* sh, int K_stride,
                                    int sh_degree, const float* viewmat, const float* twist, const float* times,
                                    float fx, float fy, float cx, float cy, int H, int W, float clip, int antialiased,
                                    int defer_color, float* records, unsigned* depth_keys, int* num_tiles_hit,
                                    int* radii, float rolling_shutter_time, float* pix_vel, const float* sh_rest,
                                    int param_flags, void* stream) {
  if (N <= 0 || P <= 0 || sh_degree < 0 || sh_degree > 4 || (sh_degree + 1) * (sh_degree + 1) > K_stride || !twist ||
      !times)
    return GS_ERR_INVALID;
  if (rolling_shutter_time != 0.f && !pix_vel) return GS_ERR_INVALID;
  FusedParams fp = make_fused(N, P, means, scales, glob_scale, quats, opacities, sh, K_stride, sh_degree, viewmat,
                              fx, fy, cx, cy, H, W, clip, antialiased, defer_color);
  fp.pixvel = 1; fp.twist = twist; fp.times = times;
  fp.rs_half = 0.5f * rolling_shutter_time; fp.pix_vel_out = pix_vel;
  fp.act = param_flags; fp.sh_rest = sh_rest;
  dim3 grid((N + 255) / 256), block(256);
  if (fp.defer_color)
    hipLaunchKernelGGL((project_fused_fwd_kernel<16, true>), grid, block, 0, (hipStream_t)stream, fp, records,
                       depth_keys, num_tiles_hit, radii);
  else if (sh_degree <= 3)
    hipLaunchKernelGGL((project_fused_fwd_kernel<16, false>), grid, block, 0, (hipStream_t)stream, fp, records,
                       depth_keys, num_tiles_hit, radii);
  else
    hipLaunchKernelGGL((project_fused_fwd_kernel<25, false>), grid, block, 0, (hipStream_t)stream, fp, records,
                       depth_keys, num_tiles_hit, radii);
  return gs_launch_status();
}

GS_EXPORT int gs_project_pixvel_bwd(int N, int P, const float* means, const float* scales, float glob_scale,
                                    const float* quats, const float* opacities, const float* sh, int K_stride,
                                    int sh_degree, const float* viewmat, const float* twist, const float* times,
                                    float fx, float fy, float cx, float cy, int H, int W, float clip, int antialiased,
                                    const float* records, const float* v_records, float* v_means, float* v_scales,
                                    float* v_quats, float* v_opacities, float* v_sh, float* v_viewmat, float* v_twist,
                                    const unsigned char* touched, float* v_xy_sum, int grad_flags, const float* sh_rest,
                                    int param_flags, float* v_sh_rest, void* pose_scratch, long long pose_scratch_bytes_,
                                    void* stream) {
  if (N <= 0 || P <= 0 || sh_degree < 0 || sh_degree > 4 || (sh_degree + 1) * (sh_degree + 1) > K_stride || !twist ||
      !times || (sh_rest != nullptr) != (v_sh_rest != nullptr) || ((grad_flags & GS_FLAG_ZERO_FILL) && !touched))
    return GS_ERR_INVALID;
  FusedParams fp = make_fused(N, P, means, scales, glob_scale, quats, opacities, sh, K_stride, sh_degree, viewmat,
                              fx, fy, cx, cy, H, W, clip, antialiased);
  fp.pixvel = 1; fp.twist = twist; fp.times = times; fp.flags = grad_flags;
  fp.act = param_flags; fp.sh_rest = sh_rest;
  const FusedOut out = {v_means, v_scales, v_quats, v_opacities, v_sh, v_sh_rest, v_viewmat, v_xy_sum, v_twist, nullptr};
  return launch_fused_bwd(fp, sh_degree, records, v_records, out, touched, pose_scratch, pose_scratch_bytes_,
                          (hipStream_t)stream);
}
```

3dgs-deblur_amd/dp.py:

```python
from __future__ import annotations

from typing import Iterable, List, Optional, Sequence

import torch
import torch.distributed as dist


def shard_views(num_views: int, rank: int, world_size: int) -> List[int]:
    if not (0 <= rank < world_size):
        raise ValueError("rank out of range")
    return list(range(rank, num_views, world_size))


def flatten_grads(params: Sequence[torch.Tensor]) -> torch.Tensor:
    total = sum(p.numel() for p in params)
    ref = params[0]
    flat = torch.zeros(total, dtype=torch.float32, device=ref.device)
    off = 0
    for p in params:
        n = p.numel()
        if p.grad is not None:
            flat[off:off + n].copy_(p.grad.reshape(-1))
        off += n
    return flat


def unflatten_grads(flat: torch.Tensor, params: Sequence[torch.Tensor]) -> None:
    off = 0
    for p in params:
        n = p.numel()
        g = flat[off:off + n].view_as(p)
        if p.grad is None:
            p.grad = g.clone()
        else:
            p.grad.copy_(g)
        off += n


FORCE = bool(int(__import__("os").environ.get("GSD_DP_FORCE", "0")))


def allreduce_gradients(params: Iterable[torch.Tensor], group: Optional[dist.ProcessGroup] = None,
                        mode: str = "allreduce", average: bool = False, sync_free: Optional[bool] = None,
                        force: Optional[bool] = None) -> None:
    params = [p for p in params if p.requires_grad]
    if not params or not dist.is_available() or not dist.is_initialized():
        return
    world = dist.get_world_size(group)
    if world == 1 and not (FORCE if force is None else force):
        return
    if mode == "sparse":
        if _allreduce_sparse_rows(params, group, world, average, sync_free):
            return
        mode = "allreduce"
    flat = flatten_grads(params)
    if mode == "allreduce":
        dist.all_reduce(flat, op=dist.ReduceOp.SUM, group=group)
    elif mode == "rs_ag":
        n = flat.numel()
        pad = (-n) % world
        if pad:
            flat = torch.cat([flat, flat.new_zeros(pad)])
        chunk = flat.numel() // world
        mine = torch.empty(chunk, dtype=flat.dtype, device=flat.device)
        if dist.get_backend(group) == "gloo":
            dist.all_reduce(flat, op=dist.ReduceOp.SUM, group=group)
        else:
            dist.reduce_scatter_tensor(mine, flat, op=dist.ReduceOp.SUM, group=group)
            dist.all_gather_into_tensor(flat, mine, group=group)
        flat = flat[:n]
    else:
        raise ValueError(f"unknown mode {mode!r}")
    if average:
        flat.div_(world)
    unflatten_grads(flat, params)


class _RowOps:

    def __init__(self, grads: Sequence[torch.Tensor]):
        self.grads = grads
        self.N = grads[0].shape[0]
        self.widths = [g[0].numel() if self.N else 1 for g in grads]
        self.wtot = sum(self.widths)
        self.dev = grads[0].device
        self.hip = self.dev.type == "cuda"
        if self.hip:
            import ctypes
            from . import _lib
            self._L = _lib.load()
            self._check = _lib.check
            n = len(grads)
            self._ptrs = (ctypes.c_void_p * n)(*[g.data_ptr() for g in grads])
            self._w = (ctypes.c_int * n)(*self.widths)
            self._stream = ctypes.c_void_p(torch.cuda.current_stream(self.dev).cuda_stream)
            self._vp = ctypes.c_void_p

    def row_mask(self) -> torch.Tensor:
        if self.hip:
            mask = torch.empty(self.N, dtype=torch.uint8, device=self.dev)
            self._check(self._L.gs_dp_row_mask(self.N, len(self.grads), self._ptrs, self._w,
                                               self._vp(mask.data_ptr()), self._stream), "dp_row_mask")
            return mask.bool()
        mask = torch.zeros(self.N, dtype=torch.bool, device=self.dev)
        for g in self.grads:
            mask |= (g.reshape(self.N, -1) != 0).any(dim=1)
        return mask

    def pack(self, idx: torch.Tensor, rows_padded: int) -> torch.Tensor:
        M = idx.numel()
        pay = torch.zeros(rows_padded, self.wtot + 1, dtype=torch.float32, device=self.dev)
        if M == 0:
            return pay
        if self.hip:
            self._check(self._L.gs_dp_pack_rows(M, self._vp(idx.data_ptr()), len(self.grads), self._ptrs, self._w,
                                                self._vp(pay.data_ptr()), self._stream), "dp_pack_rows")
        else:
            pay[:M, :self.wtot] = torch.cat([g.reshape(self.N, -1)[idx] for g in self.grads], dim=1)
            pay[:M, self.wtot] = idx.to(torch.int32).view(torch.float32)
        return pay

    def pack_masked(self, cap: int) -> torch.Tensor:
        stride = self.wtot + 1
        mask = self.row_mask()
        pay = torch.zeros(cap + 1, stride, dtype=torch.float32, device=self.dev)
        if self.hip:
            m8 = mask.view(torch.uint8) if mask.dtype == torch.bool else mask
            pos = torch.cumsum(m8, 0, dtype=torch.int32) - m8.to(torch.int32)
            idx_ws = torch.empty(cap, dtype=torch.int32, device=self.dev)
            self._check(self._L.gs_dp_pack_masked_rows(self.N, self._vp(m8.data_ptr()), self._vp(pos.data_ptr()), cap,
                                                       self._vp(idx_ws.data_ptr()), len(self.grads), self._ptrs, self._w,
                                                       self._vp(pay.data_ptr()), self._stream), "dp_pack_masked_rows")
            return pay
        idx = mask.nonzero(as_tuple=False).reshape(-1)
        total = idx.numel()
        idx = idx[:cap]
        M = idx.numel()
        hdr = torch.tensor([total, M], dtype=torch.int32).view(torch.float32)
        pay[0, :2] = hdr
        if M:
            pay[1:1 + M, :self.wtot] = torch.cat([g.reshape(self.N, -1)[idx] for g in self.grads], dim=1)
            pay[1:1 + M, self.wtot] = idx.to(torch.int32).view(torch.float32)
        return pay

    def scatter_add_payload(self, payload: torch.Tensor, cap: int, scale: float) -> None:
        if self.hip:
            payload = payload.contiguous()
            self._check(self._L.gs_dp_scatter_add_payload(cap, self._vp(payload.data_ptr()), len(self.grads), self._ptrs,
                                                          self._w, float(scale), self._stream), "dp_scatter_add_payload")
            return
        M = int(payload[0, 1].view(torch.int32))
        self.scatter_add(payload[1:], M, scale)

    def scatter_add(self, payload: torch.Tensor, M: int, scale: float) -> None:
        if M == 0:
            return
        if self.hip:
            self._check(self._L.gs_dp_scatter_add_rows(M, self._vp(payload.data_ptr()), len(self.grads), self._ptrs,
                                                       self._w, float(scale), self._stream), "dp_scatter_add_rows")
            return
        rows = payload[:M, self.wtot].contiguous().view(torch.int32).to(torch.int64)
        off = 0
        for g, w in zip(self.grads, self.widths):
            g.reshape(self.N, -1).index_add_(0, rows, payload[:M, off:off + w] * scale)
            off += w


class SparseExchangeState:

    def __init__(self, N: int, world: int, cap_min: int = 1024, dense_fraction: float = 0.25):
        self.N, self.world = N, world
        self.cap_max = max(1, int(N * dense_fraction / max(1, world)))
        self.cap_min = min(cap_min, self.cap_max)
        self.cap = self.cap_max
        self.dense = False
        self.pending = None
        self.history = []
        self.overflows = 0

    def observe(self, totals) -> None:
        self.history = (self.history + [max(int(v) for v in totals)])[-8:]
        want = 2 * max(self.history)
        if want > self.cap_max:
            self.dense = True
        else:
            self.dense = False
            cap = self.cap_min
            while cap < want:
                cap *= 2
            self.cap = min(cap, self.cap_max)

    def forget(self) -> None:
        self.pending = None
        self.history = []
        self.dense = False
        self.cap = self.cap_max

    def settle(self) -> None:
        if self.pending is None:
            return
        host, ev, cap_used = self.pending
        self.pending = None
        if ev is not None:
            ev.synchronize()
        totals = [int(v) for v in host.tolist()]
        if cap_used is not None and max(totals) > cap_used:
            self.forget()
            raise RuntimeError(f"row-sparse gradient exchange overflowed: a rank had {max(totals)} rows with a gradient, "
                               f"capacity was {cap_used}; the previous step's gradients are incomplete "
                               f"(use the guarded exchange, raise cap_min / dense_fraction or mode='allreduce')")
        self.observe(totals)


_SPARSE_STATES = {}
SYNC_FREE = bool(int(__import__("os").environ.get("GSD_DP_SYNC_FREE", "0")))


def _sparse_state(N: int, world: int, group) -> SparseExchangeState:
    key = (world, id(group))
    st = _SPARSE_STATES.get(key)
    if st is None or st.N != N:
        st = _SPARSE_STATES[key] = SparseExchangeState(N, world)
    return st


def reset_sparse_exchange_state() -> None:
    _SPARSE_STATES.clear()


def notify_regime_change() -> None:
    for st in _SPARSE_STATES.values():
        try:
            st.settle()
        finally:
            st.forget()


def _allreduce_sparse_rows(params: Sequence[torch.Tensor], group, world: int, average: bool,
                           sync_free: Optional[bool] = None) -> bool:
    N = params[0].shape[0]
    if N == 0 or any(p.shape[0] != N for p in params):
        return False
    sync_free = SYNC_FREE if sync_free is None else bool(sync_free)
    st = _sparse_state(N, world, group)
    st.settle()
    for p in params:
        if p.grad is None:
            p.grad = torch.zeros_like(p)
        elif not p.grad.is_contiguous() or p.grad.dtype != torch.float32:
            p.grad = p.grad.contiguous().float()
    ops = _RowOps([p.grad for p in params])
    stride = ops.wtot + 1
    if not st.history:
        total = ops.row_mask().sum(dtype=torch.int32).reshape(1)
        totals = torch.empty(world, dtype=torch.int32, device=ops.dev)
        dist.all_gather_into_tensor(totals, total, group=group)
        st.observe(totals.cpu().tolist())
    if st.dense:
        total = ops.row_mask().sum(dtype=torch.int32).reshape(1)
        totals = torch.empty(world, dtype=torch.int32, device=ops.dev)
        dist.all_gather_into_tensor(totals, total, group=group)
        st.pending = _async_to_host(totals) + (None,)
        return False
    cap = st.cap
    pay = ops.pack_masked(cap)
    pay_all = torch.empty(world * (cap + 1) * stride, dtype=torch.float32, device=ops.dev)
    dist.all_gather_into_tensor(pay_all, pay.reshape(-1), group=group)
    pay_all = pay_all.view(world, cap + 1, stride)
    headers = pay_all[:, 0, 0].contiguous().view(torch.int32)
    if sync_free:
        st.pending = _async_to_host(headers) + (cap,)
    else:
        totals = headers.cpu().tolist()
        st.observe(totals)
        if max(totals) > cap:
            st.overflows += 1
            return False
    for p in params:
        p.grad.zero_()
    scale = 1.0 / world if average else 1.0
    for r in range(world):
        ops.scatter_add_payload(pay_all[r], cap, scale)
    return True


def _async_to_host(t: torch.Tensor):
    if t.device.type != "cuda":
        return t.clone(), None
    host = torch.empty(t.shape, dtype=t.dtype, pin_memory=True)
    host.copy_(t, non_blocking=True)
    ev = torch.cuda.Event()
    ev.record()
    return host, ev


def allreduce_dense_(tensors: Sequence[torch.Tensor], group: Optional[dist.ProcessGroup] = None,
                     average: bool = False, force: Optional[bool] = None) -> None:
    tensors = [t for t in tensors if t is not None]
    if not tensors or not dist.is_available() or not dist.is_initialized():
        return
    world = dist.get_world_size(group)
    if world == 1 and not (FORCE if force is None else force):
        return
    flat = torch.cat([t.reshape(-1).float() for t in tensors])
    dist.all_reduce(flat, op=dist.ReduceOp.SUM, group=group)
    if average:
        flat.div_(world)
    off = 0
    for t in tensors:
        n = t.numel()
# ... 14 lines not shown
```

3dgs-deblur_amd/ops.py:

```python
from __future__ import annotations

import ctypes
import math
from typing import Optional, Tuple

import torch
from torch import Tensor
from torch.autograd import Function

from . import _lib

import os
import threading

TILE = 16
REC = 16
GRAD = 12
MAX_SUBPOSES = 256
SLICE_BASE = int(os.environ.get("GSD_SLICE_BASE", "512"))
SLICE_ADAPT = int(os.environ.get("GSD_SLICE_ADAPT", "1"))
SLICE_GROW_OPEN = float(os.environ.get("GSD_SLICE_GROW_OPEN", "0.5"))
_state_lock = threading.RLock()


# ... 396 lines not shown
        _band_done_cache[key] = t
    return t


def _background(background: Optional[Tensor], device) -> Tensor:
    if background is None:
        return torch.zeros(3, dtype=torch.float32, device=device)
    bg = background.detach().to(device=device, dtype=torch.float32).contiguous()
    if bg.numel() != 3:
        raise ValueError("background must have 3 channels")
    return bg


frame_backend = None


class _FrameDesc(ctypes.Structure):
    _fields_ = [(k, ctypes.c_int) for k in ("N", "P", "S", "R", "H", "W", "slice_base", "depth_sort_digit",
                                             "fwd_variant", "reserve_backward")] + [("merge_open_fraction", ctypes.c_float),
                                                                                     ("rolling_shutter_time", ctypes.c_float),
                                                                                     ("poll_readback", ctypes.c_int),
                                                                                     ("shared_list", ctypes.c_int),
                                                                                     ("combine_gamma", ctypes.c_float),
                                                                                     ("combine_min_level", ctypes.c_float),
                                                                                     ("band_clipped", ctypes.c_int),
                                                                                     ("depth_select", ctypes.c_int),
                                                                                     ("select_cap", ctypes.c_int),
                                                                                     ("sweep_t_min", ctypes.c_float),
                                                                                     ("sweep_t_max", ctypes.c_float),
                                                                                     ("lazy_records", ctypes.c_void_p),
                                                                                     ("cameras", ctypes.c_int)]


class _ProjectInputs(ctypes.Structure):
    _fields_ = ([(k, ctypes.c_void_p) for k in ("means", "scales", "quats", "opacities", "viewmats")] +
                [(k, ctypes.c_float) for k in ("glob_scale", "fx", "fy", "cx", "cy", "clip_thresh")] +
                [(k, ctypes.c_int) for k in ("antialiased", "defer_color", "param_flags")])


class _FrameSlice(ctypes.Structure):
    _fields_ = ([("I", ctypes.c_longlong)] + [(k, ctypes.c_int) for k in ("n", "wave_per_gaussian", "first", "last")] +
                [(k, ctypes.c_longlong) for k in ("svals", "bins", "fidx", "gi_of_e", "sorted_ids", "slice_gi", "counts",
                                                  "cum", "tile_hot", "n_emitted_dev")])


class _FrameState(ctypes.Structure):
    _fields_ = ([(k, ctypes.c_int) for k in ("n_slices", "P", "N", "S", "R", "H", "W")] +
                [("rolling_shutter_time", ctypes.c_float), ("shared_list", ctypes.c_int), ("depth_select", ctypes.c_int),
                 ("select_overflow", ctypes.c_int), ("open_after_first", ctypes.c_float)] +
                [(k, ctypes.c_longlong) for k in ("n_total", "max_selected", "arena_used", "arena_required")] +
                [("slice", _FrameSlice * 16), ("cameras", ctypes.c_int)])


def _box_share(state) -> Optional[float]:
    n_total = int(state.n_total)
    if n_total <= 0:
        return None
    held = sum(int(state.slice[i].I) for i in range(int(state.n_slices)))
    return min(1.0, held / n_total)


class _ArenaTooSmall(Exception):
    pass


_ARENA_ATTEMPTS = 16
_arena_pool = {}


class _Arena:
    __slots__ = ("tensor", "gen")

    def __init__(self, tensor):
        self.tensor, self.gen = tensor, 0

    def numel(self):
        return self.tensor.numel()

    def data_ptr(self):
        return self.tensor.data_ptr()


_lease_counter = 0


class _ArenaLease:
    __slots__ = ("arena", "key", "gen")

    def __init__(self, arena: _Arena, key):
        global _lease_counter
        self.arena, self.key = arena, key
        with _state_lock:
            _lease_counter += 1
            self.gen = arena.gen = _lease_counter

    @property
    def tensor(self):
        a = self.arena
        return None if a is None else a.tensor

    def release(self):
        try:
            with _state_lock:
                a, self.arena = self.arena, None
                if a is None:
                    return
                free = _arena_pool.setdefault(self.key, [])
                free.append(a)
                if len(free) > 2:
                    free.remove(min(free, key=lambda x: x.numel()))
        except Exception:
            pass

    __del__ = release


def _arena_acquire(dev, want_bytes: int) -> _ArenaLease:
    key = (str(dev), torch.cuda.current_stream(dev).cuda_stream)
    with _state_lock:
        free = _arena_pool.setdefault(key, [])
        free[:] = [x if isinstance(x, _Arena) else _Arena(x) for x in free]
        a = max(free, key=lambda x: x.numel()) if free else None
        if a is not None:
            free.remove(a)
    if a is None or a.numel() < want_bytes:
        a = None
        a = _Arena(torch.empty(int(want_bytes), dtype=torch.uint8, device=dev))
    return _ArenaLease(a, key)


def _arena_relend(frame) -> bool:
    a = frame["arena_obj"]
    with _state_lock:
        free = _arena_pool.get(frame["lease"].key, [])
        if a.gen != frame["gen"] or a not in free:
            raise RuntimeError("this frame's arena was handed back after its first backward and a later frame has "
                               "used it since: a second backward of one frame (retain_graph=True) must run before "
                               "the next frame's forward")
        free.remove(a)
    return True


def _arena_return(frame) -> None:
    with _state_lock:
        free = _arena_pool.setdefault(frame["lease"].key, [])
        free.append(frame["arena_obj"])
        if len(free) > 2:
            free.remove(min(free, key=lambda x: x.numel()))


def release_arenas() -> None:
    with _state_lock:
        _arena_pool.clear()


_pinned_cache = {}


def _profile_mask() -> int:
    if profiler is None:
        return 0
    names = FRAME_STAGES if profiler.only is None else [n for n in FRAME_STAGES if n in profiler.only]
    return sum(1 << FRAME_STAGES.index(n) for n in names)


def native_frame_forward(records: Tensor, depth_keys: Tensor, num_tiles_hit: Tensor, P: int, N: int, S: int, R: int,
                         H: int, W: int, bg: Tensor, edges: Tensor, slice_base: int, color=None,
                         out_depth: Optional[Tensor] = None, reserve_backward: bool = True, rs=None, combine=None,
                         hints: Optional[FrameHints] = None, band_clipped: bool = False, lazy=None,
                         depth_select: Optional[bool] = None, cameras: int = 1):
    global last_num_intersects, _slice_totals, last_depth_select
    L = _L()
    dev = records.device
    tx, ty = _tiles(H, W)
    shared = rs is not None and len(rs) > 2 and rs[2] is not None
    if hints is None:
        hints = hints_for((str(dev), N, P, S, H, W, shared))
    if depth_select is None:
        depth_select = bool(DEPTH_SELECT == 2 or (DEPTH_SELECT and hints.depth_select()))
    n = P * N
    nbytes = hints.arena_bytes
    if not nbytes:
        I0 = max(1, slice_base) * tx * ty * P
        nbytes = 44 * n + 16 * S * H * W + (80 + (56 * S if shared else 0)) * I0 + (64 << 20)
    lease = _arena_acquire(dev, nbytes)
    arena = lease.tensor
    nbytes = arena.numel()
    pin_key = (str(dev), threading.get_ident(), torch.cuda.current_stream().cuda_stream)
    pin = _pinned_cache.get(pin_key)
    need_pin = 4 * (2 * P * 16 + 2 * P + 2) + 64
    if pin is None or pin.numel() < need_pin:
        pin = _pinned_cache[pin_key] = torch.empty(max(8192, need_pin), dtype=torch.uint8, pin_memory=True)
    desc = _FrameDesc(N, P, S, R, H, W, int(slice_base), DEPTH_SORT_DIGIT, 0, int(reserve_backward),
                      float(SLICE_MERGE), float(rs[1]) if rs is not None else 0.0, frame_poll(), int(shared),
                      float(combine[0]) if combine is not None else 1.0, float(combine[1]) if combine is not None else 0.0,
                      int(bool(band_clipped)), int(bool(depth_select and slice_base > 0)),
                      int(min(hints.select_cap, 2 ** 31 - 1)) if depth_select else 0,
                      float(rs[3][0]) if shared and len(rs) > 3 else 0.0, float(rs[3][1]) if shared and len(rs) > 3 else 0.0,
                      ctypes.addressof(lazy) if lazy is not None else None, int(cameras))
    state = _FrameState()
    out_img = torch.empty(S, H, W, 3, device=dev)
    out_T = torch.empty(S, H, W, device=dev)
    band_done = _band_tile_done(S, R, ty, tx, dev) if R > 1 else None
    c_means = c_sh = c_rest = c_V = None
    c_K = c_deg = 0
    if color is not None:
        c_means, c_sh, c_rest, c_K, c_deg, c_V = color
    L.gs_frame_profile_enable(_profile_mask())
    st = L.gs_frame_forward(ctypes.byref(desc), _ptr(records), _ptr(depth_keys), _ptr(num_tiles_hit), _ptr(bg), _ptr(edges),
                            _ptr(band_done), _ptr(c_means), _ptr(c_sh), _ptr(c_rest), int(c_K), int(c_deg), _ptr(c_V),
                            _ptr(rs[0]) if rs is not None else None, _ptr(rs[2]) if shared else None, _ptr(out_img),
                            _ptr(out_T), _ptr(out_depth), _ptr(combine[2]) if combine is not None else None,
                            _ptr(arena), arena.numel(), ctypes.c_void_p(pin.data_ptr()), pin.numel(), ctypes.byref(state),
                            _stream())
    if st == 3:
        hints.arena_bytes = max(int(state.arena_required * 1.15) + (32 << 20), int(nbytes * 1.5))
        raise _ArenaTooSmall()
    _check(st, "frame_forward")
    hints.arena_bytes = max(int(hints.arena_bytes),
                            int((state.arena_used + L.gs_frame_backward_bytes(ctypes.byref(state))) * 1.15))
    last_num_intersects = int(state.n_total)
    last_depth_select = int(state.depth_select)
    _slice_totals = [arena[sl.n_emitted_dev:sl.n_emitted_dev + 4].view(torch.int32)
                     for sl in (state.slice[i] for i in range(state.n_slices))]
    return out_img, out_T, dict(arena=arena, arena_obj=lease.arena, lease=lease, gen=lease.gen, state=state,
                                pix_vel=rs[0] if rs is not None else None,
                                sample_times=rs[2] if shared else None)


def native_frame_backward(frame, records: Tensor, bg: Tensor, edges: Tensor, out_T: Tensor, v_img: Tensor,
                          v_alpha: Optional[Tensor], v_records: Tensor, touched: Tensor, combine=None,
                          v_depth: Optional[Tensor] = None, absgrad: bool = False):
    L = _L()
    cmb = combine if combine is not None else (None, 1.0, 0.0)
    arena, state = frame["arena"], frame["state"]
    lease = frame["lease"]
    relent = lease.arena is None and _arena_relend(frame)
    try:
        _native_frame_backward(L, frame, arena, state, records, bg, edges, out_T, v_img, v_alpha, v_records, touched, cmb,
                               v_depth, absgrad)
    finally:
        if relent:
            _arena_return(frame)
        else:
            lease.release()


def _native_frame_backward(L, frame, arena, state, records, bg, edges, out_T, v_img, v_alpha, v_records, touched, cmb,
                           v_depth=None, absgrad=False):
    L.gs_frame_profile_enable(_profile_mask())
    if v_depth is None:
        st = L.gs_frame_backward(ctypes.byref(state), _ptr(records), _ptr(bg), _ptr(edges), _ptr(out_T), _ptr(v_img),
                                 _ptr(v_alpha), _ptr(cmb[0]), float(cmb[1]), float(cmb[2]), _bwd_variant(absgrad),
                                 _ptr(v_records), _ptr(touched), _ptr(frame.get("pix_vel")), _ptr(frame.get("sample_times")), _ptr(arena),
                                 arena.numel(), _stream())
    else:
        st = L.gs_frame_backward_depth(ctypes.byref(state), _ptr(records), _ptr(bg), _ptr(edges), _ptr(out_T),
                                       _ptr(v_img), _ptr(v_alpha), _ptr(cmb[0]), float(cmb[1]), float(cmb[2]),
                                       _bwd_variant(absgrad), _ptr(v_records), _ptr(touched),
                                       _ptr(frame.get("pix_vel")),
                                       _ptr(frame.get("sample_times")), _ptr(arena), arena.numel(), _ptr(v_depth),
                                       _stream())
    if st == 3:
        raise _lib.HipLibraryError("frame_backward: the forward's arena cannot hold the backward's buffers "
                                   "(call native_frame_forward with reserve_backward=True)")
    _check(st, "frame_backward")


class _ProjectGaussians(Function):
    @staticmethod
    def forward(ctx, means3d, scales, glob_scale, quats, viewmat, fx, fy, cx, cy, img_height, img_width,
                block_width, clip_thresh):
        if block_width != TILE:
            raise ValueError("only block_width=16 is supported")
        means3d, scales, quats = _f32(means3d, "means3d"), _f32(scales, "scales"), _f32(quats, "quats")
        V = _viewmat16(viewmat)
        N = means3d.shape[0]
        dev = means3d.device
        xys = torch.empty(N, 2, device=dev)
        depths = torch.empty(N, device=dev)
        radii = torch.empty(N, dtype=torch.int32, device=dev)
        conics = torch.empty(N, 3, device=dev)
        comp = torch.empty(N, device=dev)
        ntiles = torch.empty(N, dtype=torch.int32, device=dev)
        cov3d = torch.empty(N, 6, device=dev)
        _check(_L().gs_project_fwd(N, _ptr(means3d), _ptr(scales), float(glob_scale), _ptr(quats), _ptr(V),
                                   float(fx), float(fy), float(cx), float(cy), int(img_height), int(img_width),
                                   float(clip_thresh), _ptr(xys), _ptr(depths), _ptr(radii), _ptr(conics),
                                   _ptr(comp), _ptr(ntiles), _ptr(cov3d), None, _stream()), "project_fwd")
        ctx.save_for_backward(means3d, scales, quats, V)
        ctx.args = (float(glob_scale), float(fx), float(fy), float(cx), float(cy), int(img_height),
                    int(img_width), float(clip_thresh))
        ctx.mark_non_differentiable(radii, ntiles)
        return xys, depths, radii, conics, comp, ntiles, cov3d

    @staticmethod
    def backward(ctx, v_xys, v_depths, v_radii, v_conics, v_comp, v_ntiles, v_cov3d):
        means3d, scales, quats, V = ctx.saved_tensors
        glob, fx, fy, cx, cy, H, W, clip = ctx.args
        N = means3d.shape[0]
        dev = means3d.device

        def z(g, shape):
            return torch.zeros(shape, device=dev) if g is None else g.contiguous().float()
        v_xys, v_depths, v_conics, v_comp = z(v_xys, (N, 2)), z(v_depths, (N,)), z(v_conics, (N, 3)), z(v_comp, (N,))
        v_means = torch.empty(N, 3, device=dev)
# ... 59 lines not shown
    def forward(ctx, xys, depths, radii, conics, num_tiles_hit, colors, opacity, img_height, img_width,
                block_width, background, return_alpha):
        if block_width != TILE:
            raise ValueError("only block_width=16 is supported")
        assert colors.shape[-1] == 3
        xys, depths, conics = _f32(xys, "xys"), _f32(depths, "depths"), _f32(conics, "conics")
        colors, opacity = _f32(colors, "colors"), _f32(opacity, "opacity").reshape(-1)
        radii = radii.to(torch.int32).contiguous()
        N = xys.shape[0]
        dev = xys.device
        H, W = int(img_height), int(img_width)
        L = _L()
        records = torch.empty(N, REC, device=dev)
        dkeys = torch.empty(N, dtype=torch.int32, device=dev)
        ntiles = torch.empty(N, dtype=torch.int32, device=dev)
        _check(L.gs_pack_records(N, _ptr(xys), _ptr(depths), _ptr(radii), _ptr(conics), _ptr(colors), _ptr(opacity),
                                 H, W, _ptr(records), _ptr(dkeys), _ptr(ntiles), _stream()), "pack_records")
        svals, bins, n_isect, _ = bin_and_sort_records(records, dkeys, ntiles, 1, N, H, W)
        bg = _background(background, dev)
        edges = _band_edges(H, 1, dev)
        out_img = torch.empty(1, H, W, 3, device=dev)
        out_T = torch.empty(1, H, W, device=dev)
        fidx = torch.empty(1, H, W, dtype=torch.int32, device=dev)
        _check(L.gs_rasterize_fwd(_ptr(records), _ptr(svals), _ptr(bins), _ptr(edges), _ptr(bg), 1, 1, H, W,
                                  _ptr(out_img), _ptr(out_T), _ptr(fidx), N if n_isect > 0 else 0, 0,
                                  _stream()), "rasterize_fwd")
        ctx.save_for_backward(records, svals, bins, edges, bg, out_T, fidx)
        ctx.dims = (N, H, W)
        ctx.bg_grad = background is not None and ctx.needs_input_grad[10]
        out = out_img[0]
        if return_alpha:
            return out, 1.0 - out_T[0]
        return out

    @staticmethod
    def backward(ctx, v_img, v_alpha=None):
        records, svals, bins, edges, bg, out_T, fidx = ctx.saved_tensors
        N, H, W = ctx.dims
        dev = records.device
        L = _L()
        v_img = v_img.contiguous().float()
        v_al = None if v_alpha is None else v_alpha.contiguous().float()
        v_records = torch.zeros(N, GRAD, device=dev)
        _check(L.gs_rasterize_bwd(_ptr(records), _ptr(svals), _ptr(bins), _ptr(edges), _ptr(bg), 1, 1, H, W,
                                  _ptr(out_T), _ptr(fidx), _ptr(v_img), _ptr(v_al), _ptr(v_records), N, _bwd_variant(),
                                  _stream()), "rasterize_bwd")
        v_xys = torch.empty(N, 2, device=dev)
        v_conics = torch.empty(N, 3, device=dev)
        v_colors = torch.empty(N, 3, device=dev)
        v_opacity = torch.empty(N, 1, device=dev)
        _check(L.gs_unpack_record_grads(N, _ptr(v_records), _ptr(v_xys), _ptr(v_conics), _ptr(v_colors),
                                        _ptr(v_opacity), _stream()), "unpack grads")
        v_bg = (out_T[0][..., None] * v_img).sum(dim=(0, 1)) if ctx.bg_grad else None
        return (v_xys, None, None, v_conics, None, v_colors, v_opacity, None, None, None, v_bg, None)


def rasterize_gaussians(xys: Tensor, depths: Tensor, radii: Tensor, conics: Tensor, num_tiles_hit: Tensor,
                        colors: Tensor, opacity: Tensor, img_height: int, img_width: int, block_width: int = TILE,
                        background: Optional[Tensor] = None, return_alpha: bool = False, *,
                        pix_vels: Optional[Tensor] = None, exposure_time: float = 0.0, rolling_shutter_time: float = 0.0,
                        blur_samples: int = 0, return_samples: bool = False):
    if pix_vels is not None:
        if block_width != TILE:
            raise ValueError("only block_width=16 is supported")
        if colors.shape[-1] != 3:
            raise ValueError("rasterize_gaussians with pix_vels composites 3 channels")
        from . import velocity_ops as VO
        _, times, span = VO.sample_span(blur_samples, exposure_time, rolling_shutter_time)
        img, alpha = VO.RasterizeGaussiansPixvel.apply(xys, depths, radii, conics, colors, opacity.reshape(-1, 1), pix_vels,
                                                       int(img_height), int(img_width), background, times,
                                                       float(rolling_shutter_time), span)
        if not return_samples:
            img, alpha = img.mean(dim=0), alpha.mean(dim=0)
        return (img, alpha) if return_alpha else img
    C = colors.shape[-1]
    if C == 3:
        return _RasterizeGaussians.apply(xys, depths, radii, conics, num_tiles_hit, colors, opacity.reshape(-1, 1),
                                         img_height, img_width, block_width, background, return_alpha)
    if background is not None and background.numel() != C:
        raise ValueError(f"background must have {C} channels")
    imgs, alpha = [], None
    for c0 in range(0, C, 3):
        n = min(3, C - c0)
        col = colors[:, c0:c0 + n]
        bg = None if background is None else background.reshape(-1)[c0:c0 + n]
        if n < 3:
            col = torch.cat([col, col.new_zeros(col.shape[0], 3 - n)], dim=1)
            bg = None if bg is None else torch.cat([bg, bg.new_zeros(3 - n)])
        res = _RasterizeGaussians.apply(xys, depths, radii, conics, num_tiles_hit, col, opacity.reshape(-1, 1),
                                        img_height, img_width, block_width, bg, return_alpha and alpha is None)
        if return_alpha and alpha is None:
            res, alpha = res
        imgs.append(res[..., :n])
    out = torch.cat(imgs, dim=-1)
    return (out, alpha) if return_alpha else out


def compute_cumulative_intersects(num_tiles_hit: Tensor) -> Tuple[int, Tensor]:
    nt = num_tiles_hit.to(torch.int32).contiguous()
    ex, total = exclusive_scan_u32(nt)
    return int(total.item()), ex + nt


def map_gaussian_to_intersects(num_points: int, num_intersects: int, xys: Tensor, depths: Tensor, radii: Tensor,
                               cum_tiles_hit: Tensor, tile_bounds, block_width: int = TILE):
    dev = xys.device
    isect = torch.zeros(max(1, num_intersects), dtype=torch.int64, device=dev)
    gids = torch.zeros(max(1, num_intersects), dtype=torch.int32, device=dev)
    W, H = int(tile_bounds[0]) * TILE, int(tile_bounds[1]) * TILE
    _check(_L().gs_map_gaussian_to_intersects(int(num_points), _ptr(_f32(xys, "xys")), _ptr(_f32(depths, "depths")),
                                              _ptr(radii.to(torch.int32).contiguous()),
                                              _ptr(cum_tiles_hit.to(torch.int32).contiguous()), H, W, _ptr(isect),
                                              _ptr(gids), _stream()), "map_gaussian_to_intersects")
    return isect[:num_intersects], gids[:num_intersects]


def get_tile_bin_edges(num_intersects: int, isect_ids_sorted: Tensor, tile_bounds) -> Tensor:
    T = int(tile_bounds[0]) * int(tile_bounds[1])
    bins = torch.empty(T, 2, dtype=torch.int32, device=isect_ids_sorted.device)
    _check(_L().gs_tile_bin_edges_u64(int(num_intersects), _ptr(isect_ids_sorted.contiguous()), T, _ptr(bins),
                                      _stream()), "tile_bin_edges")
    return bins


def bin_and_sort_gaussians(num_points: int, num_intersects: int, xys: Tensor, depths: Tensor, radii: Tensor,
                           cum_tiles_hit: Tensor, tile_bounds, block_width: int = TILE):
    isect, gids = map_gaussian_to_intersects(num_points, num_intersects, xys, depths, radii, cum_tiles_hit,
                                             tile_bounds, block_width)
    T = int(tile_bounds[0]) * int(tile_bounds[1])
    if num_intersects == 0:
        return isect, gids, isect, gids, torch.zeros(T, 2, dtype=torch.int32, device=xys.device)
    ks, vs = radix_sort_pairs(isect.clone(), gids.clone(), 0, 32 + _bits(T))
    bins = get_tile_bin_edges(num_intersects, ks, tile_bounds)
    return isect, gids, ks, vs, bins


class _SubposeViewmats(Function):
    @staticmethod
    def forward(ctx, viewmat, lin_vel, ang_vel, times):
        V = _viewmat16(viewmat)
        lin, ang, times = _f32(lin_vel, "lin_vel"), _f32(ang_vel, "ang_vel"), _f32(times, "times")
        P = times.numel()
        out = torch.empty(P, 4, 4, device=V.device)
        _check(_L().gs_subpose_viewmats_fwd(P, _ptr(V), _ptr(lin), _ptr(ang), _ptr(times), _ptr(out), _stream()),
               "subpose_viewmats_fwd")
        ctx.save_for_backward(V, lin, ang, times)
        return out

    @staticmethod
    def backward(ctx, v_out):
        V, lin, ang, times = ctx.saved_tensors
        P = times.numel()
        dev = V.device
        acc = torch.zeros(22, device=dev)
        v_V, v_lin, v_ang = acc[:16].view(4, 4), acc[16:19], acc[19:22]
        _check(_L().gs_subpose_viewmats_bwd(P, _ptr(V), _ptr(lin), _ptr(ang), _ptr(times),
                                            _ptr(v_out.contiguous().float()), _ptr(v_V), _ptr(v_lin), _ptr(v_ang),
                                            _stream()), "subpose_viewmats_bwd")
        return v_V, v_lin, v_ang, None


def subpose_viewmats(viewmat: Tensor, lin_vel: Tensor, ang_vel: Tensor, times: Tensor) -> Tensor:
    return _SubposeViewmats.apply(viewmat, lin_vel, ang_vel, times)


def subpose_schedule(blur_samples: int, exposure_time: float, rs_bands: int, rolling_shutter_time: float):
    S, R = max(1, int(blur_samples)), max(1, int(rs_bands))
    times, samp, band = [], [], []
    for s in range(S):
        ts = ((s + 0.5) / S - 0.5) * exposure_time if S > 1 else 0.0
        for r in range(R):
            tr = ((r + 0.5) / R - 0.5) * rolling_shutter_time if R > 1 else 0.0
            times.append(ts + tr)
            samp.append(s)
            band.append(r)
    return times, samp, band


class _RenderSubposes(Function):
    @staticmethod
    def forward(ctx, means3d, scales, quats, opacities, sh, viewmats, background, S, R, fx, fy, cx, cy,
                img_height, img_width, sh_degree, antialiased, glob_scale, clip_thresh, xy_grad_out, return_alpha,
                gamma, min_rgb_level, lin_vel=None, ang_vel=None, times=None, return_depth=False, rs_time=0.0,
                sh_rest=None, param_flags=0, shared_list=False, hints=None, cameras=1, xy_absgrad_out=None):
        ctx.set_materialize_grads(False)
        if xy_absgrad_out is not None:
            if times is not None:
                raise ValueError("xy_absgrad_out is not available with the pixel-velocity model (times=): its backward "
                                 "compositor uses gradient slots 9 and 10 for d loss / d pixel velocity")
            if frame_backend is not None and not frame_backend.native_ok():
                raise ValueError("xy_absgrad_out needs the library's frame path (the absgrad backward compositors); the "
                                 "frame backend in use has none")
        means3d, scales, quats = _f32(means3d, "means3d"), _f32(scales, "scales"), _f32(quats, "quats")
        opacities, sh = _f32(opacities, "opacities").reshape(-1), _f32(sh, "sh")
        param_flags = int(param_flags)
        if sh_rest is not None:
            sh_rest = _f32(sh_rest, "sh_rest")
            if sh.reshape(sh.shape[0], -1).shape[1] != 3 or sh_rest.dim() != 3 or sh_rest.shape[0] != sh.shape[0]:
                raise ValueError("with sh_rest [N,K-1,3], sh must be features_dc [N,3] (or [N,1,3])")
        B = max(1, int(cameras))
        xy_shape = (means3d.shape[0], 2) if B == 1 else (B, means3d.shape[0], 2)
        if xy_grad_out is not None:
            if (xy_grad_out.shape != xy_shape or xy_grad_out.dtype != torch.float32
                    or not xy_grad_out.is_contiguous() or xy_grad_out.device != means3d.device):
                raise ValueError(f"xy_grad_out must be a contiguous float32 {list(xy_shape)} tensor on the Gaussians' "
                                 f"device")
        ctx.xy_grad_out = xy_grad_out
        if xy_absgrad_out is not None:
            if (xy_absgrad_out.shape != xy_shape or xy_absgrad_out.dtype != torch.float32
                    or not xy_absgrad_out.is_contiguous() or xy_absgrad_out.device != means3d.device):
                raise ValueError(f"xy_absgrad_out must be a contiguous float32 {list(xy_shape)} tensor on the Gaussians' "
                                 f"device")
        ctx.xy_absgrad_out = xy_absgrad_out
        N, K = means3d.shape[0], (sh.shape[1] if sh_rest is None else 1 + sh_rest.shape[1])
        P = S * R
        if P > MAX_SUBPOSES:
            raise ValueError(f"{S} blur samples x {R} row bands = {P} sub-poses per frame; the slice descriptors travel "
                             f"in kernel arguments and hold at most {MAX_SUBPOSES} (kMaxSubposes, csrc/binning.hip)")
        pixvel = times is not None
        rs_time = float(rs_time or 0.0)
        if rs_time != 0.0 and (not pixvel or R != 1):
            raise ValueError("exact rolling shutter (rolling_shutter_time != 0) needs the pixel-velocity model "
                             "(times / lin_vel / ang_vel) and rs_bands == 1")
        shared = None
        if shared_list:
            if not pixvel or R != 1:
                raise ValueError("shared_list needs the pixel-velocity model (times / lin_vel / ang_vel) and rs_bands == 1")
            tl = [float(t) for t in (times.reshape(-1).tolist() if isinstance(times, Tensor) else times)]
            if len(tl) != S:
                raise ValueError(f"times must hold {S} sample times")
            t_c = 0.5 * (min(tl) + max(tl))
            shared = (torch.tensor([t - t_c for t in tl], dtype=torch.float32, device=means3d.device),
                      (max(tl) - min(tl)) + abs(rs_time), (min(tl) - t_c, max(tl) - t_c))
            times = torch.tensor([t_c], dtype=torch.float32, device=means3d.device)
            P = 1
        if pixvel:
            V = _viewmat16(viewmats).reshape(4, 4)
            twist = torch.cat([_f32(lin_vel, "lin_vel").reshape(3), _f32(ang_vel, "ang_vel").reshape(3)]).contiguous()
            times = _f32(times, "times").reshape(-1)
            if times.numel() != P:
                raise ValueError(f"times must hold {P} sub-pose times")
        else:
            V = _f32(viewmats, "viewmats")
            twist = None
            if V.shape != (P, 4, 4):
                raise ValueError(f"viewmats must be [{P},4,4]")
        H, W = int(img_height), int(img_width)
        dev = means3d.device
        L = _L()
        records = torch.empty(P * N, REC, device=dev)
        dkeys = torch.empty(P * N, dtype=torch.int32, device=dev)
        ntiles = torch.empty(P * N, dtype=torch.int32, device=dev)
        radii = torch.empty(P, N, dtype=torch.int32, device=dev)
        args = (N, P, float(glob_scale), K, int(sh_degree), float(fx), float(fy), float(cx), float(cy), H, W,
                float(clip_thresh), int(bool(antialiased)))
        backend = frame_backend if (frame_backend is not None and not frame_backend.native_ok()) else None
        defer_flags = 3 if backend is None else backend.defer_flags()
        if backend is None and R > 1 and BAND_AWARE:
            defer_flags |= 4 | (R << 8)
        if B > 1 and (pixvel or shared is not None or backend is not None):
            raise NotImplementedError("a frame of several cameras renders SE(3) sub-poses through the library's frame "
                                      "path (no pixel-velocity model, shared list or frame backend)")
        if backend is None and hints is None:
            key = (str(dev), N, P, S, H, W, shared is not None, means3d.untyped_storage().data_ptr())
            hints = hints_for(key if B == 1 else key + (B,))
        lazy = None
        if (backend is None and not pixvel and LAZY_RECORDS and hints.slice_base() > 0
                and (LAZY_RECORDS == 2 or hints.lazy_records())):
            defer_flags |= 16
        if shared is not None and backend is not None:
            raise ValueError("the shared-list mode runs through the library's frame path only")
        pix_vel = torch.empty(N, 2, device=dev) if (rs_time != 0.0 or shared is not None) else None
        rs = None if pix_vel is None else (pix_vel, rs_time) + ((shared[0], shared[2]) if shared is not None else ())
        box_sweep = shared[1] if shared is not None else rs_time
        ctx.rs = rs

        def _project():
            if pixvel:
                _check(L.gs_project_pixvel_fwd(N, P, _ptr(means3d), _ptr(scales), args[2], _ptr(quats), _ptr(opacities),
                                               _ptr(sh), K, args[4], _ptr(V), _ptr(twist), _ptr(times), args[5], args[6],
                                               args[7], args[8], H, W, args[11], args[12], defer_flags,
                                               _ptr(records), _ptr(dkeys), _ptr(ntiles), _ptr(radii), box_sweep,
                                               _ptr(pix_vel), _ptr(sh_rest), param_flags, _stream()),
                       "project_pixvel_fwd")
            else:
                _check(L.gs_project_fused_fwd(N, P, _ptr(means3d), _ptr(scales), args[2], _ptr(quats), _ptr(opacities),
                                              _ptr(sh), K, args[4], _ptr(V), args[5], args[6], args[7], args[8], H, W,
                                              args[11], args[12], defer_flags, _ptr(records), _ptr(dkeys),
                                              _ptr(ntiles), _ptr(radii), _ptr(sh_rest), param_flags, _stream()),
                       "project_fused_fwd")

        with _stage("project_fwd"):
            _project()
        if defer_flags & 16:
            lazy = _ProjectInputs(means3d.data_ptr(), scales.data_ptr(), quats.data_ptr(), opacities.data_ptr(),
                                  V.data_ptr(), args[2], args[5], args[6], args[7], args[8], args[11], args[12],
                                  defer_flags & ~16, param_flags)
        bg = _background(background, dev)
        edges = _band_edges(H, R, dev)
        V_col = V.reshape(1, 16).expand(P, 16).contiguous() if pixvel else V
        color = (means3d, sh, sh_rest, K, args[4], V_col) if (defer_flags & 1) else None
        depth_acc = torch.zeros(S, H, W, device=dev) if return_depth else None
        ctx.prealloc = None
        ctx.frame = None
        ctx.backend = backend
        if backend is None:
            if rs is not None and R != 1:
                raise ValueError("exact rolling shutter renders with rs_bands == 1")
            if any(ctx.needs_input_grad):
                t_len = (P * N + 15) // 16 * 16
                zbuf = torch.zeros(t_len + 4 * (16 * P + 12), dtype=torch.uint8, device=dev)
                zf = zbuf[t_len:].view(torch.float32)
                ctx.prealloc = {"touched": zbuf[:P * N], "v_records": torch.empty(P * N, GRAD, device=dev),
                                "v_V": zf[:16 * P], "v_tw": zf[16 * P:16 * P + 12],
                                "pose_scratch": _pose_scratch(N, P, True, dev)}
            averaged = None
            if gamma is not None:
                averaged = (float(gamma), float(min_rgb_level) / 255.0,
                            torch.empty((H, W, 3) if B == 1 else (B, H, W, 3), device=dev))
            retries = 0
            for attempt in range(_ARENA_ATTEMPTS):
                try:
                    out_img, out_T, ctx.frame = native_frame_forward(records, dkeys, ntiles, P, N, S, R, H, W, bg, edges,
                                                                     hints.slice_base(), color, depth_acc,
                                                                     any(ctx.needs_input_grad), rs, averaged, hints,
                                                                     bool(defer_flags & 4), lazy, cameras=B)
                    hints.feedback(int(ctx.frame["state"].n_slices), retries, _box_share(ctx.frame["state"]),
                                   int(ctx.frame["state"].depth_select), float(ctx.frame["state"].open_after_first),
                                   int(ctx.frame["state"].max_selected), int(ctx.frame["state"].select_overflow))
                    break
                except _ArenaTooSmall:
                    retries += 1
                    if attempt == _ARENA_ATTEMPTS - 1:
                        raise _lib.HipLibraryError("frame_forward: the arena estimate did not converge")
                    if depth_acc is not None:
                        depth_acc.zero_()
                    with _stage("project_fwd"):
                        _project()
            slices = []
        else:
            ctx.prealloc = {} if any(ctx.needs_input_grad) else None
            out_img, out_T, slices = backend.sliced_forward(records, dkeys, ntiles, P, N, S, R, H, W, bg, edges, SLICE_BASE,
                                                            color, depth_acc, ctx.prealloc, rs)
        ctx.slices = slices
        svals = bins = fidx = _placeholder_i32(dev)
        n_isect = last_num_intersects
        ctx.combine = None
        first = cmb_samples = cmb_rgb = out_img
        if gamma is not None:
            m = float(min_rgb_level) / 255.0
            if backend is None:
                first = cmb_rgb = averaged[2]
            else:
                first = cmb_rgb = torch.empty(H, W, 3, device=dev)
                with _stage("combine"):
                    _check(L.gs_combine_fwd(S, H * W * 3, _ptr(out_img), float(gamma), m, _ptr(first), _stream()),
                           "combine_fwd")
            ctx.combine = (float(gamma), m)
        else:
            cmb_samples = cmb_rgb = svals
        ctx.pixvel = (twist, times) if pixvel else None
        ctx.param_flags = param_flags
        ctx.sh_rest = sh_rest
        ctx.save_for_backward(means3d, scales, quats, opacities, sh, V, records, svals, bins, edges, bg, out_T, fidx,
                              cmb_samples, cmb_rgb)
        ctx.args = args
        ctx.SR = (S, R)
        ctx.n_isect = n_isect
        ctx.bg_grad = background is not None and ctx.needs_input_grad[6]
        ctx.mark_non_differentiable(radii)
        ctx.img_shape = (S, H, W, 3) if gamma is None else ((H, W, 3) if B == 1 else (B, H, W, 3))
        ctx.cameras = B
        return first, (1.0 - out_T) if return_alpha else None, radii, depth_acc

    @staticmethod
    def backward(ctx, v_img, v_alpha, _v_radii, v_depth=None):
        (means3d, scales, quats, opacities, sh, V, records, svals, bins, edges, bg, out_T, fidx, cmb_samples,
         cmb_rgb) = ctx.saved_tensors
        N, P, glob, K, deg, fx, fy, cx, cy, H, W, clip, aa = ctx.args
        S, R = ctx.SR
        dev = means3d.device
        L = _L()
        if v_img is None and v_alpha is None and v_depth is None:
            return (None,) * 34
        B = ctx.cameras
        if v_depth is not None:
            if ctx.frame is None:
                raise NotImplementedError("a depth gradient needs the native frame backward (gs_frame_backward_depth); "
                                          "the frame backend in use has no depth channel")
            v_depth = v_depth.contiguous().float()
        v_img = torch.zeros(ctx.img_shape, device=dev) if v_img is None else v_img.contiguous().float()
        v_al = None if v_alpha is None else v_alpha.contiguous().float()
        combine = None
        if ctx.combine is not None:
            samples, rgb = cmb_samples, cmb_rgb
            gamma, m = ctx.combine
            if ctx.bg_grad:
                v_samples = torch.empty_like(samples)
                if B > 1:
                    _check(L.gs_combine_bwd_batched(B, S // B, rgb.numel() // B, _ptr(samples), gamma, m, _ptr(rgb),
                                                    _ptr(v_img), _ptr(v_samples), _stream()), "combine_bwd_batched")
                else:
                    _check(L.gs_combine_bwd(S, rgb.numel(), _ptr(samples), gamma, m, _ptr(rgb), _ptr(v_img),
                                            _ptr(v_samples), _stream()), "combine_bwd")
                v_img = v_samples
            else:
                scale = torch.empty_like(rgb)
                with _stage("combine"):
                    if B > 1:
                        _check(L.gs_combine_bwd_scale_batched(B, S // B, rgb.numel() // B, gamma, _ptr(rgb), _ptr(v_img),
                                                              _ptr(scale), _stream()), "combine_bwd_scale_batched")
                    else:
                        _check(L.gs_combine_bwd_scale(S, rgb.numel(), gamma, _ptr(rgb), _ptr(v_img), _ptr(scale),
                                                      _stream()), "combine_bwd_scale")
                combine = (scale, gamma, m)
                v_img = samples
        all_tuples = ctx.frame is not None or all(sl["gi_of_e"] is not None for sl in ctx.slices)
        pre = ctx.prealloc if ctx.prealloc else {}
        ctx.prealloc = None
        if all_tuples and "touched" in pre:
            v_records, touched = pre["v_records"], pre["touched"]
        elif all_tuples:
            v_records = torch.empty(P * N, GRAD, device=dev)
            touched = torch.zeros(P * N, dtype=torch.uint8, device=dev)
        else:
            v_records = torch.zeros(P * N, GRAD, device=dev)
            touched = None

        if ctx.frame is not None:
            native_frame_backward(ctx.frame, records, bg, edges, out_T, v_img, v_al, v_records, touched, combine, v_depth,
                                  ctx.xy_absgrad_out is not None)
            if ctx.xy_absgrad_out is not None:
                _check(L.gs_xy_absgrad_sum(N, P, B, _ptr(v_records), _ptr(touched), _ptr(ctx.xy_absgrad_out), _stream()),
                       "xy_absgrad_sum")
        else:
            ctx.backend.sliced_backward(records, ctx.slices, S, R, H, W, bg, edges, out_T, v_img, v_al, v_records, touched,
                                        combine, ctx.rs)
        sh_rest = ctx.sh_rest
        sizes = [3 * N, 3 * N, 4 * N, N] + ([3 * K * N] if sh_rest is None else [3 * N, 3 * (K - 1) * N])
        shapes = [(N, 3), (N, 3), (N, 4), (N,)] + ([(N, K, 3)] if sh_rest is None else [tuple(sh.shape), (N, K - 1, 3)])
        flat = torch.empty(sum(sizes), device=dev)
        outs = [t.view(shape) for t, shape in zip(flat.split(sizes), shapes)]
        v_means, v_scales, v_quats, v_opac, v_sh = outs[:5]
        v_sh_rest = outs[5] if sh_rest is not None else None
        need_v = ctx.needs_input_grad[5]
        xy_out = ctx.xy_grad_out
        fill_flag = (32 if touched is not None else 0) | (64 if v_depth is not None else 0)
        xy_cams = (128 | (B << 8)) if (B > 1 and xy_out is not None) else 0
        pf = ctx.param_flags
        v_lin = v_ang = None
        psc = pre.get("pose_scratch") if touched is not None else None
        if psc is None and (need_v or ctx.needs_input_grad[23] or ctx.needs_input_grad[24]):
            psc = _pose_scratch(N, P, touched is not None, dev)
        psc_n = 0 if psc is None else psc.numel()
        with _stage("project_bwd"):
            if ctx.pixvel is not None:
                twist, times = ctx.pixvel
                v_V = (pre["v_V"][:16].view(4, 4) if "v_V" in pre else torch.zeros(4, 4, device=dev)) if need_v else None
                need_tw = ctx.needs_input_grad[23] or ctx.needs_input_grad[24]
                v_tw = (pre["v_tw"] if "v_tw" in pre else torch.zeros(12, device=dev)) if need_tw else None
                _check(L.gs_project_pixvel_bwd(N, P, _ptr(means3d), _ptr(scales), glob, _ptr(quats), _ptr(opacities),
                                               _ptr(sh), K, deg, _ptr(V), _ptr(twist), _ptr(times), fx, fy, cx, cy, H, W,
                                               clip, aa, _ptr(records), _ptr(v_records), _ptr(v_means), _ptr(v_scales),
                                               _ptr(v_quats), _ptr(v_opac), _ptr(v_sh), _ptr(v_V), _ptr(v_tw),
                                               _ptr(touched), _ptr(xy_out),
                                               _proj_grad_flags() | (16 if ctx.rs is not None else 0) | fill_flag,
                                               _ptr(sh_rest), pf, _ptr(v_sh_rest), _ptr(psc), psc_n, _stream()),
                       "project_pixvel_bwd")
                if v_tw is not None:
                    v_lin, v_ang = v_tw[0:3], v_tw[3:6]
            else:
                v_V = (pre["v_V"].view(P, 4, 4) if "v_V" in pre else torch.zeros(P, 4, 4, device=dev)) if need_v else None
                _check(L.gs_project_fused_bwd(N, P, _ptr(means3d), _ptr(scales), glob, _ptr(quats), _ptr(opacities),
                                              _ptr(sh), K, deg, _ptr(V), fx, fy, cx, cy, H, W, clip, aa, _ptr(records),
                                              _ptr(v_records), _ptr(v_means), _ptr(v_scales), _ptr(v_quats),
                                              _ptr(v_opac), _ptr(v_sh), _ptr(v_V), _ptr(touched), _ptr(xy_out),
                                              _proj_grad_flags() | fill_flag | xy_cams, _ptr(sh_rest), pf, _ptr(v_sh_rest),
                                              _ptr(psc), psc_n, _stream()), "project_fused_bwd")
        v_bg = (out_T[..., None] * v_img).sum(dim=(0, 1, 2)) if ctx.bg_grad else None
        return ((v_means, v_scales, v_quats, v_opac, v_sh, v_V, v_bg) + (None,) * 16
                + (v_lin, v_ang, None, None, None, v_sh_rest, None, None, None, None, None))


def render_subposes(means3d: Tensor, scales: Tensor, quats: Tensor, opacities: Tensor, sh: Tensor,
                    viewmats: Tensor, background: Optional[Tensor], blur_samples: int, rs_bands: int,
                    fx: float, fy: float, cx: float, cy: float, img_height: int, img_width: int,
                    sh_degree: int = 3, antialiased: bool = True, glob_scale: float = 1.0,
                    clip_thresh: float = 0.01, xy_grad_out: Optional[Tensor] = None, return_alpha: bool = True,
                    lin_vel: Optional[Tensor] = None, ang_vel: Optional[Tensor] = None,
                    times: Optional[Tensor] = None, return_depth: bool = False, rolling_shutter_time: float = 0.0,
                    sh_rest: Optional[Tensor] = None, raw_params: bool = False, shared_list: bool = False,
                    hints: Optional[FrameHints] = None, xy_absgrad_out: Optional[Tensor] = None):
    S, R = max(1, int(blur_samples)), max(1, int(rs_bands))
    out = _RenderSubposes.apply(means3d, scales, quats, opacities, sh, viewmats, background, S, R, fx, fy, cx, cy,
                                img_height, img_width, sh_degree, antialiased, glob_scale, clip_thresh, xy_grad_out,
                                bool(return_alpha), None, None, lin_vel, ang_vel, times, bool(return_depth),
                                float(rolling_shutter_time), sh_rest, 3 if raw_params else 0,
                                bool(shared_list), hints, 1, xy_absgrad_out)
    return out if return_depth else out[:3]


def render_combined(means3d: Tensor, scales: Tensor, quats: Tensor, opacities: Tensor, sh: Tensor,
                    viewmats: Tensor, background: Optional[Tensor], blur_samples: int, rs_bands: int,
                    fx: float, fy: float, cx: float, cy: float, img_height: int, img_width: int,
                    gamma: float = 1.0, min_rgb_level: float = 0.0, sh_degree: int = 3, antialiased: bool = True,
                    glob_scale: float = 1.0, clip_thresh: float = 0.01, xy_grad_out: Optional[Tensor] = None,
                    return_alpha: bool = True, lin_vel: Optional[Tensor] = None, ang_vel: Optional[Tensor] = None,
                    times: Optional[Tensor] = None, return_depth: bool = False, rolling_shutter_time: float = 0.0,
                    sh_rest: Optional[Tensor] = None, raw_params: bool = False, shared_list: bool = False,
                    hints: Optional[FrameHints] = None, xy_absgrad_out: Optional[Tensor] = None):
    S, R = max(1, int(blur_samples)), max(1, int(rs_bands))
    out = _RenderSubposes.apply(means3d, scales, quats, opacities, sh, viewmats, background, S, R, fx, fy, cx, cy,
                                img_height, img_width, sh_degree, antialiased, glob_scale, clip_thresh, xy_grad_out,
                                bool(return_alpha), float(gamma), float(min_rgb_level), lin_vel, ang_vel, times,
                                bool(return_depth), float(rolling_shutter_time), sh_rest, 3 if raw_params else 0,
                                bool(shared_list), hints, 1, xy_absgrad_out)
    return out if return_depth else out[:3]


MAX_FRAME_PIXELS = 1 << 30


def check_batch(n_cameras: int, blur_samples: int, rs_bands: int, img_height: int, img_width: int) -> None:
    B, S, R = int(n_cameras), int(blur_samples), int(rs_bands)
    if B < 1:
        raise ValueError("render_batch needs at least one camera")
    if B * S * R > MAX_SUBPOSES:
        raise ValueError(f"{B} cameras x {S} blur samples x {R} row bands = {B * S * R} sub-poses in one frame; a frame "
                         f"holds at most {MAX_SUBPOSES} (kMaxSubposes): render fewer cameras per call")
    if B * S * int(img_height) * int(img_width) >= MAX_FRAME_PIXELS:
        raise ValueError(f"{B} cameras x {S} blur samples x {img_height}x{img_width} pixels = "
                         f"{B * S * int(img_height) * int(img_width)} sample pixels in one frame; the compositors' 32-bit "
                         f"offsets need fewer than 2^30: render fewer cameras per call")


def render_batch(means3d: Tensor, scales: Tensor, quats: Tensor, opacities: Tensor, sh: Tensor, viewmats: Tensor,
                 background: Optional[Tensor], blur_samples: int, rs_bands: int, fx: float, fy: float, cx: float,
                 cy: float, img_height: int, img_width: int, gamma: float = 1.0, min_rgb_level: float = 0.0,
                 sh_degree: int = 3, antialiased: bool = True, glob_scale: float = 1.0, clip_thresh: float = 0.01,
                 return_alpha: bool = True, return_depth: bool = False, sh_rest: Optional[Tensor] = None,
                 raw_params: bool = False, xy_grad_out: Optional[Tensor] = None, hints: Optional[FrameHints] = None,
                 times: Optional[Tensor] = None, shared_list: bool = False, xy_absgrad_out: Optional[Tensor] = None):
    if times is not None and xy_absgrad_out is not None:
        raise ValueError("xy_absgrad_out is not available with the pixel-velocity model (times=)")
    if times is not None:
        raise NotImplementedError("render_batch renders SE(3) sub-poses; the pixel-velocity model (times=) renders one "
                                  "camera per call (render_combined)")
    if shared_list:
        raise NotImplementedError("render_batch has no shared-list mode (pixel-velocity model, one camera per call)")
    if frame_backend is not None and not frame_backend.native_ok():
        raise NotImplementedError("render_batch runs through the library's frame path only; the Python frame backend "
                                  "renders one camera per call")
    S, R = max(1, int(blur_samples)), max(1, int(rs_bands))
    if viewmats.dim() != 4 or tuple(viewmats.shape[1:]) != (S * R, 4, 4):
        raise ValueError(f"viewmats must be [B,{S * R},4,4] (B cameras x {S} blur samples x {R} row bands)")
    B = int(viewmats.shape[0])
    H, W = int(img_height), int(img_width)
    check_batch(B, S, R, H, W)
    N = means3d.shape[0]
    if xy_grad_out is not None and tuple(xy_grad_out.shape) != (B, N, 2):
        raise ValueError(f"xy_grad_out must be [B,N,2] = [{B},{N},2]")
    if xy_absgrad_out is not None and tuple(xy_absgrad_out.shape) != (B, N, 2):
        raise ValueError(f"xy_absgrad_out must be [B,N,2] = [{B},{N},2]")
    if B == 1:
        out = _RenderSubposes.apply(means3d, scales, quats, opacities, sh, viewmats[0], background, S, R, fx, fy, cx, cy,
                                    H, W, sh_degree, antialiased, glob_scale, clip_thresh,
                                    None if xy_grad_out is None else xy_grad_out[0], bool(return_alpha), float(gamma),
                                    float(min_rgb_level), None, None, None, bool(return_depth), 0.0, sh_rest,
                                    3 if raw_params else 0, False, hints, 1,
                                    None if xy_absgrad_out is None else xy_absgrad_out[0])
    else:
        out = _RenderSubposes.apply(means3d, scales, quats, opacities, sh, viewmats.reshape(B * S * R, 4, 4), background,
                                    B * S, R, fx, fy, cx, cy, H, W, sh_degree, antialiased, glob_scale, clip_thresh,
                                    xy_grad_out, bool(return_alpha), float(gamma), float(min_rgb_level), None, None, None,
                                    bool(return_depth), 0.0, sh_rest, 3 if raw_params else 0, False, hints, B,
                                    xy_absgrad_out)
    rgb, alphas, radii, depth = out
    rgb = rgb.reshape(B, H, W, 3)
    alphas = alphas.reshape(B, S, H, W) if alphas is not None else None
    radii = radii.reshape(B, S * R, N)
    if return_depth:
        return rgb, alphas, radii, depth.reshape(B, S, H, W)
    return rgb, alphas, radii


class _CombineSamples(Function):
    @staticmethod
    def forward(ctx, samples, gamma, min_rgb_level):
        samples = _f32(samples, "samples")
        S = samples.shape[0]
        n = samples[0].numel()
        out = torch.empty_like(samples[0])
        m = float(min_rgb_level) / 255.0
        _check(_L().gs_combine_fwd(S, n, _ptr(samples), float(gamma), m, _ptr(out), _stream()), "combine_fwd")
        ctx.save_for_backward(samples, out)
        ctx.gm = (float(gamma), m)
        return out

    @staticmethod
    def backward(ctx, v_out):
        samples, out = ctx.saved_tensors
        gamma, m = ctx.gm
        S = samples.shape[0]
        n = samples[0].numel()
        v_samples = torch.empty_like(samples)
        _check(_L().gs_combine_bwd(S, n, _ptr(samples), gamma, m, _ptr(out), _ptr(v_out.contiguous().float()),
                                   _ptr(v_samples), _stream()), "combine_bwd")
        return v_samples, None, None


def combine_samples(samples: Tensor, gamma: float = 1.0, min_rgb_level: float = 0.0) -> Tensor:
    return _CombineSamples.apply(samples, gamma, min_rgb_level)
```

include/gsdeblur.h:

```cpp
#ifndef GSDEBLUR_H
#define GSDEBLUR_H

#ifdef __cplusplus
extern "C" {
#endif

#define GS_BWD_ABSGRAD 2048

const char* gs_version(void);

int gs_subpose_viewmats_fwd(int P, const float* viewmat , const float* lin_vel ,
                            const float* ang_vel , const float* times ,
                            float* out_viewmats , void* stream);
int gs_subpose_viewmats_bwd(int P, const float* viewmat, const float* lin_vel, const float* ang_vel,
                            const float* times, const float* v_out , float* v_viewmat,
                            float* v_lin, float* v_ang, void* stream);

int gs_project_fwd(int N, const float* means3d , const float* scales , float glob_scale,
                   const float* quats , const float* viewmat , float fx, float fy,
                   float cx, float cy, int img_height, int img_width, float clip_thresh,
                   float* xys , float* depths , int* radii , float* conics ,
                   float* compensation , int* num_tiles_hit , float* cov3d ,
                   int* tile_bounds , void* stream);
long long gs_project_pose_scratch_bytes(int N, int P, int with_touched);
int gs_project_bwd(int N, const float* means3d, const float* scales, float glob_scale, const float* quats,
                   const float* viewmat, float fx, float fy, float cx, float cy, int img_height,
                   int img_width, float clip_thresh, const float* v_xys, const float* v_depths,
                   const float* v_conics, const float* v_comp, float* v_means3d, float* v_scales,
                   float* v_quats, float* v_viewmat,
                   int grad_flags ,
                   void* pose_scratch ,
                         long long pose_scratch_bytes,
                         void* stream);

int gs_sh_fwd(int N, int K_stride, int degrees_to_use, const float* viewdirs ,
              const float* coeffs, float* colors , void* stream);
int gs_sh_bwd(int N, int K_stride, int degrees_to_use, const float* viewdirs, const float* v_colors,
              float* v_coeffs , void* stream);

int gs_project_fused_fwd(int N, int P, const float* means3d, const float* scales, float glob_scale,
                         const float* quats, const float* opacities ,
                         const float* sh , int K_stride, int sh_degree,
                         const float* viewmats , float fx, float fy, float cx, float cy,
                         int img_height, int img_width, float clip_thresh, int antialiased,
                         int defer_color ,
                         float* records , unsigned* depth_keys ,
                         int* num_tiles_hit , int* radii ,
                         const float* sh_rest ,
                         int param_flags ,
                         void* stream);
int gs_slice_colors(int n_slice, const unsigned* slice_gi, const unsigned* counts, int N, const float* means3d,
                    const float* sh, const float* sh_rest , int K_stride, int sh_degree,
                    const float* viewmats, float* records, void* stream);
int gs_project_fused_bwd(int N, int P, const float* means3d, const float* scales, float glob_scale,
                         const float* quats, const float* opacities, const float* sh, int K_stride,
                         int sh_degree, const float* viewmats, float fx, float fy, float cx, float cy,
                         int img_height, int img_width, float clip_thresh, int antialiased,
                         const float* records, const float* v_records, float* v_means3d, float* v_scales,
                         float* v_quats, float* v_opacities, float* v_sh, float* v_viewmats,
                         const unsigned char* touched ,
                         float* v_xy_sum ,
                         int grad_flags ,
                         const float* sh_rest, int param_flags ,
                         float* v_sh_rest ,
                         void* pose_scratch ,
                         long long pose_scratch_bytes,
                         void* stream);

int gs_project_pixvel_fwd(int N, int P, const float* means3d, const float* scales, float glob_scale,
                          const float* quats, const float* opacities, const float* sh, int K_stride, int sh_degree,
                          const float* viewmat , const float* twist , const float* times ,
                          float fx, float fy, float cx, float cy, int img_height, int img_width, float clip_thresh,
                          int antialiased, int defer_color, float* records, unsigned* depth_keys,
                          int* num_tiles_hit, int* radii, float rolling_shutter_time ,
                          float* pix_vel ,
                          const float* sh_rest, int param_flags , void* stream);
int gs_project_pixvel_bwd(int N, int P, const float* means3d, const float* scales, float glob_scale,
                          const float* quats, const float* opacities, const float* sh, int K_stride, int sh_degree,
                          const float* viewmat, const float* twist, const float* times, float fx, float fy,
                          float cx, float cy, int img_height, int img_width, float clip_thresh, int antialiased,
                          const float* records, const float* v_records, float* v_means3d, float* v_scales,
                          float* v_quats, float* v_opacities, float* v_sh, float* v_viewmat, float* v_twist,
                          const unsigned char* touched, float* v_xy_sum, int grad_flags, const float* sh_rest,
                          int param_flags, float* v_sh_rest , void* pose_scratch ,
                         long long pose_scratch_bytes,
                         void* stream);

int gs_pack_records(int N, const float* xys, const float* depths, const int* radii, const float* conics,
                    const float* colors , const float* opacity , int img_height, int img_width,
                    float* records , unsigned* depth_keys , int* num_tiles_hit ,
                    void* stream);
int gs_unpack_record_grads(int N, const float* v_records, float* v_xys, float* v_conics, float* v_colors,
                           float* v_opacity, void* stream);

long long gs_scan_workspace_bytes(long long n);
long long gs_radix_sort_workspace_bytes(long long n, int begin_bit, int end_bit);
int gs_exclusive_scan_u32(long long n, const unsigned* in, unsigned* out, unsigned* total_out, void* ws,
                          long long ws_bytes, void* stream);
int gs_radix_sort_pairs_u32(long long n, unsigned* keys0, unsigned* vals0, unsigned* keys1,
                            unsigned* vals1, int vals0_is_iota, int begin_bit, int end_bit, void* ws,
                            long long ws_bytes, int* result_buf , void* stream);
int gs_radix_sort_pairs_gather_u32(long long n, unsigned* keys0, unsigned* vals0, unsigned* keys1, unsigned* vals1,
                                   int vals0_is_iota, int begin_bit, int end_bit, void* ws, long long ws_bytes,
                                   int* result_buf , const unsigned* gather_src, unsigned* gather_out,
                                   const unsigned* n_dev ,
                                   void* stream);
int gs_radix_sort_pairs_carry_u32(long long n, unsigned* keys0, unsigned* vals0, unsigned* keys1, unsigned* vals1,
                                  int vals0_is_iota, int begin_bit, int end_bit, void* ws, long long ws_bytes,
                                  int* result_buf , const unsigned* payload2_in, unsigned* payload2_a,
                                  unsigned* payload2_b, int* result_p2 ,
                                  const unsigned* n_dev , void* stream);
int gs_radix_sort_pairs_u64(long long n, unsigned long long* keys0, unsigned* vals0,
                            unsigned long long* keys1, unsigned* vals1, int vals0_is_iota, int begin_bit,
                            int end_bit, void* ws, long long ws_bytes, int* result_buf ,
                            void* stream);
long long gs_segmented_sort_workspace_bytes(long long n, long long seg_len, int begin_bit, int end_bit);
int gs_segmented_sort_pairs_u32(long long n, long long seg_len, unsigned* keys0, unsigned* vals0,
                                unsigned* keys1, unsigned* vals1, int vals0_is_iota, int begin_bit, int end_bit,
                                void* ws, long long ws_bytes, int* result_buf , void* stream);
long long gs_segmented_sort_compact_workspace_bytes(long long n, long long seg_len, int begin_bit, int end_bit,
                                                    int max_digit_bits);
int gs_segmented_sort_compact_u32(long long n, long long seg_len, unsigned* keys0, unsigned* vals0,
                                  unsigned* keys1, unsigned* vals1, int begin_bit, int end_bit,
                                  int max_digit_bits ,
                                  unsigned skip_key,
                                  unsigned* seg_counts , const unsigned* gather_src,
                                  unsigned* gather_out, void* ws, long long ws_bytes, int* result_buf ,
                                  void* stream);
long long gs_depth_select_workspace_bytes(int segments);
int gs_depth_select(long long n, long long seg_len, const unsigned* keys, const unsigned* weights, long long budget,
                    unsigned* thr_out , unsigned* grand_out, void* ws, long long ws_bytes,
                    void* stream);
int gs_segmented_sort_select_u32(long long n, long long seg_len, const unsigned* keys_src, unsigned* keys0,
                                 unsigned* vals0, unsigned* keys1, unsigned* vals1, int begin_bit, int end_bit,
                                 int max_digit_bits, unsigned skip_key, const unsigned* key_lo, const unsigned* key_hi,
                                 unsigned* seg_counts, const unsigned* gather_src, unsigned* gather_out, void* ws,
                                 long long ws_bytes, int* result_buf ,
                                 long long tail_cap ,
                                 void* stream);
int gs_exclusive_scan_segments_u32(long long n, long long seg_len, const unsigned* seg_counts ,
                                   const unsigned* in, unsigned* out, unsigned* total_out , void* ws,
                                   long long ws_bytes, void* stream);
int gs_make_depth_keys64(long long n, int N, const unsigned* depth_keys, unsigned long long* out,
                         void* stream);
int gs_gather_counts(long long n, const unsigned* sorted_gi, const int* num_tiles_hit,
                     unsigned* counts_out, void* stream);
int gs_emit_intersects(long long n_ranked, int N, int img_height, int img_width, const unsigned* sorted_gi,
                       const unsigned* cum_excl, const float* records, long long n_isect, unsigned* keys,
                       unsigned* vals, unsigned invalid_key, void* stream);
int gs_tile_bin_edges_u32(long long n, const unsigned* sorted_keys, int num_bins, int* bins ,
                          const unsigned* n_dev ,
                          void* stream);
int gs_tile_bin_edges_u64(long long n, const unsigned long long* sorted_isect_ids, int num_bins,
                          int* bins , void* stream);
int gs_tile_bin_edges_ids_u32(long long n, const unsigned* sorted_keys, int num_bins, int* bins ,
                              const unsigned* sorted_vals, const unsigned* gi_of_e, unsigned* ids_out ,
                              void* stream);
int gs_map_gaussian_to_intersects(int N, const float* xys, const float* depths, const int* radii,
                                  const int* cum_tiles_hit, int img_height, int img_width,
                                  long long* isect_ids, int* gaussian_ids, void* stream);

int gs_rasterize_fwd(const float* records, const int* sorted_vals, const int* tile_bins,
                     const int* band_edges , const float* background , int S, int R,
                     int img_height, int img_width, float* out_img , float* out_T ,
                     int* final_idx ,
                     int n_records ,
                     int variant ,
                     void* stream);
int gs_rasterize_bwd(const float* records, const int* sorted_vals, const int* tile_bins,
                     const int* band_edges, const float* background, int S, int R, int img_height,
                     int img_width, const float* out_T, const int* final_idx, const float* v_img,
                     const float* v_alpha, float* v_records,
                     int n_records ,
                     int variant ,
                     void* stream);

int gs_slice_plan(int P, int N, int K, const unsigned* cum_excl ,
                  const unsigned* total , long long base,
                  int* bounds , unsigned* rels ,
                  unsigned* seg_totals ,
                  const unsigned* n_live ,
                  unsigned* tail ,
                  void* stream);
int gs_slice_plan_select(int P, int N, int K, const unsigned* cum_excl, const unsigned* total, int* bounds,
                         unsigned* rels, unsigned* seg_totals, const unsigned* n_live, unsigned* tail,
                         const unsigned* grand, void* stream);
int gs_tile_open_sat(int P, int img_height, int img_width, const unsigned char* tile_done, int* sat,
                     unsigned long long* open_bits ,
                     const int* gate ,
                     void* stream);
int gs_slice_counts(int n_slice, int P, int N, const int* slice_begin , const int* slice_prefix ,
                    const unsigned* sorted_gi, const float* records, const int* sat, int img_height,
                    int img_width, unsigned* slice_gi, unsigned* counts, void* stream);
int gs_slice_counts_exact(int n_slice, int P, int N, const int* slice_begin , const int* slice_prefix ,
                          const unsigned* sorted_gi, const float* records, const int* sat,
                          const unsigned char* tile_done, int img_height, int img_width, unsigned* slice_gi,
                          unsigned* counts, int wave_per_gaussian ,
                          const unsigned* cum_rank ,
                          unsigned long long* hit_masks ,
                          unsigned* mask_off ,
                          const unsigned long long* open_bits ,
                          const int* gate ,
                          void* stream);
int gs_slice_counts_exact_swept(int n_slice, int P, int N, const int* slice_begin, const int* slice_prefix,
                                const unsigned* sorted_gi, const float* records, const int* sat,
                                const unsigned char* tile_done, int img_height, int img_width, unsigned* slice_gi,
                                unsigned* counts, int wave_per_gaussian, const unsigned* cum_rank,
                                unsigned long long* hit_masks, unsigned* mask_off, const unsigned long long* open_bits,
                                const float* pix_vel, float t_min, float t_max, float rolling_shutter_time,
                                void* stream);
int gs_emit_open_intersects(int n_slice, int N, int img_height, int img_width, const unsigned* slice_gi,
                            const unsigned* counts, const unsigned* cum_excl, const float* records,
                            const unsigned char* tile_done , unsigned* keys, unsigned* vals,
                            unsigned invalid_key, int compact ,
                            int wave_per_gaussian,
                            const unsigned long long* hit_masks ,
                            const unsigned* mask_off,
                            unsigned char* tile_hot ,
                            void* stream);
int gs_rasterize_fwd_slice(const float* records, const int* sorted_vals, const int* tile_bins,
// ... 185 lines not shown
```

Before: 1204.

## Pool gradient buffers across backward calls and zero only dirty rows

Adds a Python-side pool that recycles the flat gradient buffer, its per-Gaussian dirty mask and the touched mask across backward calls. A new pooled fused-backward entry zeroes only rows marked dirty from the previous call when few are dirty, and streams a full zero otherwise. The needle kernel clears the touched bytes itself, which removes a separate memset. Pose reductions and the subpose backward now store results instead of accumulating, so the zeros allocation for those outputs can go. Correctness now depends on version tracking and storage use counts detecting when the recycled gradient tensors are still referenced or were modified.

```diff
diff --git a/3dgs-deblur_amd/_lib.py b/3dgs-deblur_amd/_lib.py
--- a/3dgs-deblur_amd/_lib.py
+++ b/3dgs-deblur_amd/_lib.py
@@ -10,6 +10,7 @@
 _SIGS = {
     "gs_subpose_viewmats_fwd": [_I, _P, _P, _P, _P, _P, _P],
     "gs_subpose_viewmats_bwd": [_I, _P, _P, _P, _P, _P, _P, _P, _P, _P],
+    "gs_subpose_viewmats_bwd_store": [_I, _P, _P, _P, _P, _P, _P, _P, _P, _P],
     "gs_project_fwd": [_I, _P, _P, _F, _P, _P, _F, _F, _F, _F, _I, _I, _F, _P, _P, _P, _P, _P, _P, _P, _P, _P],
     "gs_project_bwd": [_I, _P, _P, _F, _P, _P, _F, _F, _F, _F, _I, _I, _F, _P, _P, _P, _P, _P, _P, _P, _P, _I, _P, _L, _P],
     "gs_sh_fwd": [_I, _I, _I, _P, _P, _P, _P],
@@ -19,6 +20,8 @@
     "gs_slice_colors": [_I, _P, _P, _I, _P, _P, _P, _I, _I, _P, _P, _P],
     "gs_project_fused_bwd": [_I, _I, _P, _P, _F, _P, _P, _P, _I, _I, _P, _F, _F, _F, _F, _I, _I, _F, _I,
                              _P, _P, _P, _P, _P, _P, _P, _P, _P, _P, _I, _P, _I, _P, _P, _L, _P],
+    "gs_project_fused_bwd_pooled": [_I, _I, _P, _P, _F, _P, _P, _P, _I, _I, _P, _F, _F, _F, _F, _I, _I, _F, _I,
+                                    _P, _P, _P, _P, _P, _P, _P, _P, _P, _P, _I, _P, _I, _P, _P, _L, _P, _P],
     "gs_project_pixvel_fwd": [_I, _I, _P, _P, _F, _P, _P, _P, _I, _I, _P, _P, _P, _F, _F, _F, _F, _I, _I, _F, _I, _I,
                               _P, _P, _P, _P, _F, _P, _P, _I, _P],
     "gs_rasterize_fwd_rs_slice": [_P, _P, _P, _P, _I, _I, _I, _P, _P, _P, _P, _P, _I, _I, _P, _I, _P, _P, _P, _I, _F, _P,
diff --git a/3dgs-deblur_amd/csrc/project.hip b/3dgs-deblur_amd/csrc/project.hip
--- a/3dgs-deblur_amd/csrc/project.hip
+++ b/3dgs-deblur_amd/csrc/project.hip
@@ -19,7 +19,7 @@
 __global__ __launch_bounds__(256) void subpose_bwd_kernel(int P, const float* __restrict__ V0, const float* __restrict__ lin,
                                    const float* __restrict__ ang, const float* __restrict__ times,
                                    const float* __restrict__ v_out, float* __restrict__ v_V0,
-                                   float* __restrict__ v_lin, float* __restrict__ v_ang) {
+                                   float* __restrict__ v_lin, float* __restrict__ v_ang, int store) {
   typedef Dual<1> D;
   extern __shared__ float sp_part[];
   for (int gid = threadIdx.x; gid < P * 18; gid += blockDim.x) {
@@ -41,8 +41,9 @@
     float sum = 0.f;
     for (int p = 0; p < P; ++p) sum += sp_part[p * 18 + t];
     float* dst = t < 12 ? v_V0 + t : (t < 15 ? v_lin + (t - 12) : v_ang + (t - 15));
-    *dst += sum;
-  }
+    *dst = (store ? 0.f : *dst) + sum;
+  }
+  if (store && threadIdx.x >= 18 && threadIdx.x < 22) v_V0[threadIdx.x - 6] = 0.f;
 }
 
 struct Intrin { float fx, fy, cx, cy; int W, H, tiles_x, tiles_y; float clip; };
@@ -88,7 +89,7 @@
   __syncthreads();
 }
 
-struct PoseDst { float* slot0; float* slot1; int stride; };
+struct PoseDst { float* slot0; float* slot1; int stride; int store; };
 __global__ __launch_bounds__(256) void pose_reduce_kernel(const float* __restrict__ partial, int nblocks, int slots,
                                                           PoseDst dst) {
   __shared__ double red[256][13];
@@ -112,7 +113,8 @@
       for (int j = 0; j < 12; ++j) red[threadIdx.x][j] += red[threadIdx.x + w][j];
     __syncthreads();
   }
-  if (threadIdx.x < 12) out[threadIdx.x] += (float)red[0][threadIdx.x];
+  if (threadIdx.x < 12) out[threadIdx.x] = (dst.store ? 0.f : out[threadIdx.x]) + (float)red[0][threadIdx.x];
+  else if (dst.store && threadIdx.x < 16) out[threadIdx.x] = 0.f;
 }
 
 __global__ __launch_bounds__(256) void project_bwd_kernel(int N, const float* __restrict__ means,
@@ -418,6 +420,8 @@
   float* v_xy_sum;
   float* v_twist;
   float* pose_partial;
+  unsigned char* dirty;
+  int clear_touched;
 };
 
 template <int MAXB, bool DEPTH>
@@ -672,10 +676,22 @@
 
 constexpr int kNeedleChunk = 2048;
 
+__device__ __noinline__ void needle_clear_touched(int N, int P, unsigned char* touched) {
+  if (!touched) return;
+  const int c0 = blockIdx.x * kNeedleChunk + (int)threadIdx.x * 8;
+  if (c0 >= N) return;
+  const bool word = (N % 8) == 0 && c0 + 8 <= N;
+  for (int p = 0; p < P; ++p) {
+    unsigned char* t = touched + (size_t)p * N + c0;
+    if (word) { unsigned long long* w = reinterpret_cast<unsigned long long*>(t); if (*w != 0ull) *w = 0ull; }
+    else for (int j = 0; j < 8 && c0 + j < N; ++j) if (t[j]) t[j] = 0;
+  }
+}
+
 #define GS_NEEDLE_HP_KERNEL(NAME, DEPTH)                                                                                \
 __global__ __launch_bounds__(256) void NAME(FusedParams fp, const float* __restrict__ records,                          \
     const float* __restrict__ v_records, float* __restrict__ v_means, float* __restrict__ v_scales,                    \
-    float* __restrict__ v_quats, const unsigned char* __restrict__ touched, float ratio_limit) {                       \
+    float* __restrict__ v_quats, unsigned char* __restrict__ touched, float ratio_limit, int clear_touched) {         \
   __shared__ int list[kNeedleChunk];                                                                                          \
   __shared__ int n_list;                                                                                                      \
   __shared__ double part[256][9];                                                                                             \
@@ -707,7 +723,10 @@
   }                                                                                                                           \
   __syncthreads();                                                                                                            \
   const int n = n_list;                                                                                                       \
-  if (n == 0) return;                                                                                                         \
+  if (n == 0) {                                                                                                               \
+    if (clear_touched) needle_clear_touched(fp.N, fp.P, touched);                                                                     \
+    return;                                                                                                                   \
+  }                                                                                                                           \
   const int items_per = fp.pixvel ? 1 : fp.P;                                                      \
   const int per_round = max(1, 256 / items_per);                                                       \
   for (int base = 0; base < n; base += per_round) {                                                                           \
@@ -738,6 +757,7 @@
     }                                                                                                                         \
     __syncthreads();                                                                                                          \
   }                                                                                                                           \
+  if (clear_touched) needle_clear_touched(fp.N, fp.P, touched);                                                                       \
 }
 
 GS_NEEDLE_HP_KERNEL(project_needle_hp_kernel, false)
@@ -775,55 +795,107 @@
   for (size_t k = head + 4 * n4 + threadIdx.x; k < count; k += blockDim.x) p[k] = 0.f;
 }
 
+__device__ __forceinline__ void zero_span(float* __restrict__ base, size_t first, size_t count) {
+  float* p = base + first;
+  size_t k = 0;
+  for (; k < count && (reinterpret_cast<uintptr_t>(p + k) & 15u) != 0; ++k) p[k] = 0.f;
+  for (; k + 4 <= count; k += 4) *reinterpret_cast<float4*>(p + k) = make_float4(0.f, 0.f, 0.f, 0.f);
+  for (; k < count; ++k) p[k] = 0.f;
+}
+
 #define GS_FUSED_BWD_SPARSE_KERNEL(NAME, DEPTH)                                                                         \
 template <int MAXB, bool ZERO_FILL>                                                                                     \
 __global__ __launch_bounds__(256, 2) void NAME(FusedParams fp,                                                          \
     const float* __restrict__ records, const float* __restrict__ v_records, FusedOut out,                               \
-    const unsigned char* __restrict__ touched ) {                                                            \
+    unsigned char* __restrict__ touched ) {                                                                  \
   __shared__ float lds[48];                                                                                               \
   __shared__ int list[kFusedChunk];                                                                                       \
-  __shared__ int wave_cnt[4];                                                                                             \
+  __shared__ int wave_cnt[kFusedChunk / 256][4];                                                                          \
+  __shared__ int n_dirty;                                                                                                 \
   extern __shared__ float blk_acc[];                        \
   const int slots = out.pose_partial ? (fp.pixvel ? 2 : fp.P) : 0;                                                        \
   for (int k = threadIdx.x; k < slots * 12; k += 256) blk_acc[k] = 0.f;                                                   \
   const int lane = lane_id(), wave = threadIdx.x >> 6;                                                                    \
   const int base = blockIdx.x * kFusedChunk;                                                                              \
+  const int g_first = base + (int)threadIdx.x;                    \
+  unsigned any_m = 0u;                                                               \
+  for (int p = 0; p < fp.P; ++p) {                                                                                        \
+    const unsigned char* t = touched + (size_t)p * fp.N;                                                                  \
+    unsigned char v[kFusedChunk / 256];                                                                                   \
+_Pragma("unroll")                                                                                                         \
+    for (int r = 0; r < kFusedChunk / 256; ++r) v[r] = t[min(g_first + r * 256, fp.N - 1)];                               \
+_Pragma("unroll")                                                                                                         \
+    for (int r = 0; r < kFusedChunk / 256; ++r) any_m |= (v[r] != 0 && g_first + r * 256 < fp.N) ? (1u << r) : 0u;        \
+  }                                                                                                                       \
   if (ZERO_FILL) {                                                                                                        \
     const size_t g0 = (size_t)base, cnt = (size_t)min(kFusedChunk, fp.N - base);                                          \
-    zero_rows(out.v_means, 3 * g0, 3 * cnt);                                                                              \
-    zero_rows(out.v_scales, 3 * g0, 3 * cnt);                                                                             \
-    zero_rows(out.v_quats, 4 * g0, 4 * cnt);                                                                              \
-    zero_rows(out.v_opac, g0, cnt);                                                                                       \
-    if (out.v_sh_rest) {                                                                                                  \
-      zero_rows(out.v_sh, 3 * g0, 3 * cnt);                                                                               \
-      zero_rows(out.v_sh_rest, (size_t)(fp.K_stride - 1) * 3 * g0, (size_t)(fp.K_stride - 1) * 3 * cnt);                  \
-    } else {                                                                                                              \
-      zero_rows(out.v_sh, (size_t)fp.K_stride * 3 * g0, (size_t)fp.K_stride * 3 * cnt);                                   \
+    const size_t sh_row = out.v_sh_rest ? 3 : (size_t)fp.K_stride * 3, rest_row = (size_t)(fp.K_stride - 1) * 3;         \
+    bool stream = true;                                                                                                   \
+    if (out.dirty) {                                                                                                      \
+      if (threadIdx.x == 0) n_dirty = 0;                                                                                  \
+      __syncthreads();                                                                                                    \
+      unsigned char d[kFusedChunk / 256];                                                                                 \
+_Pragma("unroll")                                                                                                         \
+      for (int r = 0; r < kFusedChunk / 256; ++r) d[r] = out.dirty[min(g_first + r * 256, fp.N - 1)];                     \
+      unsigned dirty_m = 0u;                                                                                              \
+_Pragma("unroll")                                                                                                         \
+      for (int r = 0; r < kFusedChunk / 256; ++r) dirty_m |= (d[r] != 0 && g_first + r * 256 < fp.N) ? (1u << r) : 0u;    \
+      if (dirty_m) atomicAdd(&n_dirty, __popc(dirty_m));                                                                  \
+      __syncthreads();                                                                                                    \
+      stream = (size_t)n_dirty * 4 > cnt;                                                                                 \
+      if (!stream) {                                                                                                      \
+        for (int r = 0; r < kFusedChunk / 256; ++r) {                                                                     \
+          if (!((dirty_m >> r) & 1u)) continue;                                                                           \
+          const size_t g = (size_t)(g_first + r * 256);                                                                   \
+          zero_span(out.v_means, 3 * g, 3);                                                                               \
+          zero_span(out.v_scales, 3 * g, 3);                                                                              \
+          zero_span(out.v_quats, 4 * g, 4);                                                                               \
+          out.v_opac[g] = 0.f;                                                                                            \
+          zero_span(out.v_sh, sh_row * g, sh_row);                                                                        \
+          if (out.v_sh_rest) zero_span(out.v_sh_rest, rest_row * g, rest_row);                                            \
+        }                                                                                                                 \
+      }                                                                                                                   \
+               \
+      for (int r = 0; r < kFusedChunk / 256; ++r)                                                                         \
+        if (((dirty_m ^ any_m) >> r) & 1u) out.dirty[g_first + r * 256] = (unsigned char)((any_m >> r) & 1u);             \
+    }                                                                                                                     \
+    if (stream) {                                                                                                         \
+      zero_rows(out.v_means, 3 * g0, 3 * cnt);                                                                            \
+      zero_rows(out.v_scales, 3 * g0, 3 * cnt);                                                                           \
+      zero_rows(out.v_quats, 4 * g0, 4 * cnt);                                                                            \
+      zero_rows(out.v_opac, g0, cnt);                                                                                     \
+      zero_rows(out.v_sh, sh_row * g0, sh_row * cnt);                                                                     \
+      if (out.v_sh_rest) zero_rows(out.v_sh_rest, rest_row * g0, rest_row * cnt);                                         \
     }                                                                                                                     \
     zero_rows(out.v_xy_sum, 2 * g0, 2 * cnt);                                                                             \
                    \
     __threadfence_block();                                                                                                \
   }                                                                                                                       \
+_Pragma("unroll")                                                                                                         \
+  for (int r = 0; r < kFusedChunk / 256; ++r) {                                                                           \
+    const unsigned long long bal = __ballot((any_m >> r) & 1u);                                                           \
+    if (lane == 0) wave_cnt[r][wave] = __popcll(bal);                                                                     \
+  }                                                                                                                       \
+  __syncthreads();                                                                                                        \
   int n_list = 0;                                                                                                         \
+_Pragma("unroll")                                                                                                         \
   for (int r = 0; r < kFusedChunk / 256; ++r) {                                                                           \
-    const int g = base + r * 256 + (int)threadIdx.x;                                                                      \
-    bool any = false;                                                                                                     \
-    if (g < fp.N)                                                                                                         \
-      for (int p = 0; p < fp.P; ++p) any |= touched[(size_t)p * fp.N + g] != 0;                                           \
+    const bool any = (any_m >> r) & 1u;                                                                                   \
     const unsigned long long bal = __ballot(any);                                                                         \
-    if (lane == 0) wave_cnt[wave] = __popcll(bal);                                                                        \
-    __syncthreads();                                                                                                      \
     int off = n_list, total = 0;                                                                                          \
 _Pragma("unroll")                                                                                                         \
-    for (int w = 0; w < 4; ++w) { const int c = wave_cnt[w]; if (w < wave) off += c; total += c; }                        \
-    if (any) list[off + __popcll(bal & ((1ull << lane) - 1ull))] = g;                                                     \
+    for (int w = 0; w < 4; ++w) { const int c = wave_cnt[r][w]; if (w < wave) off += c; total += c; }                     \
+    if (any) list[off + __popcll(bal & ((1ull << lane) - 1ull))] = g_first + r * 256;                                     \
     n_list += total;                                                                                                      \
-    __syncthreads();                                                                                                      \
   }                                                                                                                       \
+  __syncthreads();                                                                                                        \
   for (int k0 = 0; k0 < n_list; k0 += 256) {                                                                              \
     const int k = k0 + (int)threadIdx.x;                                                                                  \
     const bool live = k < n_list;                                                                                         \
     fused_bwd_body<MAXB, DEPTH>(fp, records, v_records, out, touched, live ? list[k] : 0, live, lds, blk_acc);            \
+                                                          \
+    if (out.clear_touched && live)                                                                                        \
+      for (int p = 0; p < fp.P; ++p) touched[(size_t)p * fp.N + list[k]] = 0;                                             \
   }                                                                                                                       \
   __syncthreads();                                                                                                        \
   for (int k = threadIdx.x; k < slots * 12; k += 256) out.pose_partial[(size_t)blockIdx.x * slots * 12 + k] = blk_acc[k]; \
@@ -958,7 +1030,16 @@
                                       float* v_ang, void* stream) {
   if (P <= 0) return GS_ERR_INVALID;
   hipLaunchKernelGGL(subpose_bwd_kernel, dim3(1), dim3(256), (size_t)P * 18 * sizeof(float), (hipStream_t)stream, P, viewmat, lin_vel,
-                     ang_vel, times, v_out, v_viewmat, v_lin, v_ang);
+                     ang_vel, times, v_out, v_viewmat, v_lin, v_ang, 0);
+  return gs_launch_status();
+}
+
+GS_EXPORT int gs_subpose_viewmats_bwd_store(int P, const float* viewmat, const float* lin_vel, const float* ang_vel,
+                                            const float* times, const float* v_out, float* v_viewmat, float* v_lin,
+                                            float* v_ang, void* stream) {
+  if (P <= 0 || !v_viewmat || !v_lin || !v_ang) return GS_ERR_INVALID;
+  hipLaunchKernelGGL(subpose_bwd_kernel, dim3(1), dim3(256), (size_t)P * 18 * sizeof(float), (hipStream_t)stream, P, viewmat, lin_vel,
+                     ang_vel, times, v_out, v_viewmat, v_lin, v_ang, 1);
   return gs_launch_status();
 }
 
@@ -990,7 +1071,7 @@
                      rows, grad_flags);
   if (v_viewmat)
     hipLaunchKernelGGL(pose_reduce_kernel, dim3(1), dim3(256), 0, (hipStream_t)stream, rows, blocks, 1,
-                       PoseDst{v_viewmat, nullptr, 0});
+                       PoseDst{v_viewmat, nullptr, 0, 0});
   return gs_launch_status();
 }
 
@@ -1127,8 +1208,12 @@
 }
 
 static int launch_fused_bwd(const FusedParams& fp, int sh_degree, const float* records, const float* v_records,
-                            FusedOut out, const unsigned char* touched, void* scratch, long long scratch_bytes,
-                            hipStream_t st) {
+                            FusedOut out, const unsigned char* touched_in, void* scratch, long long scratch_bytes,
+                            hipStream_t st, int clear_touched = 0) {
+  unsigned char* touched = const_cast<unsigned char*>(touched_in);
+  const bool needles = !(fp.flags & GS_FLAG_NO_NEEDLE_HP);
+  out.clear_touched = (clear_touched == 1 && !needles) ? 1 : 0;
+  const int needle_clears = (clear_touched == 1 && needles) ? 1 : 0;
   dim3 block(256);
   const int N = fp.N;
   const bool pose = out.v_viewmats || out.v_twist;
@@ -1170,24 +1255,24 @@
       hipLaunchKernelGGL(project_fused_bwd_kernel<25>, grid, block, lds, st, fp, records, v_records, out);
   }
   if (pose) {
-    PoseDst dst{out.v_viewmats, fp.pixvel ? out.v_twist : nullptr, fp.pixvel ? 0 : 16};
+    PoseDst dst{out.v_viewmats, fp.pixvel ? out.v_twist : nullptr, fp.pixvel ? 0 : 16, (!fp.pixvel && out.dirty) ? 1 : 0};
     hipLaunchKernelGGL(pose_reduce_kernel, dim3(slots), dim3(256), 0, st, out.pose_partial, (int)grid.x, slots, dst);
   }
-  if (!(fp.flags & GS_FLAG_NO_NEEDLE_HP))
+  if (needles)
   {
     if (depth)
       hipLaunchKernelGGL(project_needle_hp_depth_kernel, dim3((N + kNeedleChunk - 1) / kNeedleChunk), dim3(256), 0, st, fp,
-                         records, v_records, out.v_means, out.v_scales, out.v_quats, touched, kNeedleRatio);
+                         records, v_records, out.v_means, out.v_scales, out.v_quats, touched, kNeedleRatio, needle_clears);
     else
       hipLaunchKernelGGL(project_needle_hp_kernel, dim3((N + kNeedleChunk - 1) / kNeedleChunk), dim3(256), 0, st, fp,
-                         records, v_records, out.v_means, out.v_scales, out.v_quats, touched, kNeedleRatio);
+                         records, v_records, out.v_means, out.v_scales, out.v_quats, touched, kNeedleRatio, needle_clears);
   }
   return gs_launch_status();
 }
 
 __global__ __launch_bounds__(256) void xy_grad_cams_kernel(int N, int P, int B, const float* __restrict__ v_records,
-                                                           const unsigned char* __restrict__ touched,
-                                                           float* __restrict__ v_xy) {
+                                                           unsigned char* __restrict__ touched,
+                                                           float* __restrict__ v_xy, int clear_touched) {
   const int i = blockIdx.x * blockDim.x + threadIdx.x;
   if (i >= N) return;
   const int Pc = P / B;
@@ -1196,6 +1281,7 @@
     for (int p = b * Pc; p < (b + 1) * Pc; ++p) {
       const size_t idx = (size_t)p * N + i;
       if (!touched[idx]) continue;
+      if (clear_touched) touched[idx] = 0;
       const float2 g = *reinterpret_cast<const float2*>(v_records + idx * kGradFloats);
       vxs += g.x; vys += g.y;
     }
@@ -1234,15 +1320,15 @@
   return pose_scratch_bytes(N, std::max(P, 2), false, with_touched != 0) + 256;
 }
 
-GS_EXPORT int gs_project_fused_bwd(int N, int P, const float* means, const float* scales, float glob_scale,
-                                   const float* quats, const float* opacities, const float* sh, int K_stride,
-                                   int sh_degree, const float* viewmats, float fx, float fy, float cx, float cy,
-                                   int H, int W, float clip, int antialiased, const float* records,
-                                   const float* v_records, float* v_means, float* v_scales, float* v_quats,
-                                   float* v_opacities, float* v_sh, float* v_viewmats,
-                                   const unsigned char* touched, float* v_xy_sum, int grad_flags, const float* sh_rest,
-                                   int param_flags, float* v_sh_rest, void* pose_scratch, long long pose_scratch_bytes_,
-                                   void* stream) {
+static int project_fused_bwd_impl(int N, int P, const float* means, const float* scales, float glob_scale,
+                                  const float* quats, const float* opacities, const float* sh, int K_stride,
+                                  int sh_degree, const float* viewmats, float fx, float fy, float cx, float cy,
+                                  int H, int W, float clip, int antialiased, const float* records,
+                                  const float* v_records, float* v_means, float* v_scales, float* v_quats,
+                                  float* v_opacities, float* v_sh, float* v_viewmats,
+                                  const unsigned char* touched, float* v_xy_sum, int grad_flags, const float* sh_rest,
+                                  int param_flags, float* v_sh_rest, void* pose_scratch, long long pose_scratch_bytes_,
+                                  void* stream, unsigned char* dirty) {
   if (N <= 0 || P <= 0 || sh_degree < 0 || sh_degree > 4 || (sh_degree + 1) * (sh_degree + 1) > K_stride ||
       (sh_rest != nullptr) != (v_sh_rest != nullptr) || ((grad_flags & GS_FLAG_ZERO_FILL) && !touched))
     return GS_ERR_INVALID;
@@ -1254,13 +1340,44 @@
   fp.flags = per_cam ? (grad_flags & ~(GS_FLAG_XY_PER_CAMERA | (0x1ff << 8))) : grad_flags;
   fp.act = param_flags; fp.sh_rest = sh_rest;
   const FusedOut out = {v_means, v_scales, v_quats, v_opacities, v_sh, v_sh_rest, v_viewmats,
-                        per_cam ? nullptr : v_xy_sum, nullptr, nullptr};
+                        per_cam ? nullptr : v_xy_sum, nullptr, nullptr, dirty, 0};
   const int rc = launch_fused_bwd(fp, sh_degree, records, v_records, out, touched, pose_scratch, pose_scratch_bytes_,
-                                  (hipStream_t)stream);
+                                  (hipStream_t)stream, dirty ? (per_cam ? 2 : 1) : 0);
   if (rc != GS_OK || !per_cam) return rc;
   hipLaunchKernelGGL(xy_grad_cams_kernel, dim3((N + 255) / 256), dim3(256), 0, (hipStream_t)stream, N, P, cams, v_records,
-                     touched, v_xy_sum);
-  return gs_launch_status();
+                     const_cast<unsigned char*>(touched), v_xy_sum, dirty ? 1 : 0);
+  return gs_launch_status();
+}
+
+GS_EXPORT int gs_project_fused_bwd(int N, int P, const float* means, const float* scales, float glob_scale,
+                                   const float* quats, const float* opacities, const float* sh, int K_stride,
+                                   int sh_degree, const float* viewmats, float fx, float fy, float cx, float cy,
+                                   int H, int W, float clip, int antialiased, const float* records,
+                                   const float* v_records, float* v_means, float* v_scales, float* v_quats,
+                                   float* v_opacities, float* v_sh, float* v_viewmats,
+                                   const unsigned char* touched, float* v_xy_sum, int grad_flags, const float* sh_rest,
+                                   int param_flags, float* v_sh_rest, void* pose_scratch, long long pose_scratch_bytes_,
+                                   void* stream) {
+  return project_fused_bwd_impl(N, P, means, scales, glob_scale, quats, opacities, sh, K_stride, sh_degree, viewmats, fx,
+                                fy, cx, cy, H, W, clip, antialiased, records, v_records, v_means, v_scales, v_quats,
+                                v_opacities, v_sh, v_viewmats, touched, v_xy_sum, grad_flags, sh_rest, param_flags,
+                                v_sh_rest, pose_scratch, pose_scratch_bytes_, stream, nullptr);
+}
+
+GS_EXPORT int gs_project_fused_bwd_pooled(int N, int P, const float* means, const float* scales, float glob_scale,
+                                          const float* quats, const float* opacities, const float* sh, int K_stride,
+                                          int sh_degree, const float* viewmats, float fx, float fy, float cx, float cy,
+                                          int H, int W, float clip, int antialiased, const float* records,
+                                          const float* v_records, float* v_means, float* v_scales, float* v_quats,
+                                          float* v_opacities, float* v_sh, float* v_viewmats, unsigned char* touched,
+                                          float* v_xy_sum, int grad_flags, const float* sh_rest, int param_flags,
+                                          float* v_sh_rest, void* pose_scratch, long long pose_scratch_bytes_,
+                                          void* stream, unsigned char* dirty) {
+  if (!touched || !dirty) return GS_ERR_INVALID;
+  return project_fused_bwd_impl(N, P, means, scales, glob_scale, quats, opacities, sh, K_stride, sh_degree, viewmats, fx,
+                                fy, cx, cy, H, W, clip, antialiased, records, v_records, v_means, v_scales, v_quats,
+                                v_opacities, v_sh, v_viewmats, touched, v_xy_sum, grad_flags | GS_FLAG_ZERO_FILL, sh_rest,
+                                param_flags, v_sh_rest, pose_scratch, pose_scratch_bytes_, stream, dirty);
 }
 
 GS_EXPORT int gs_project_pixvel_fwd(int N, int P, const float* means, const float* scales, float glob_scale,
diff --git a/3dgs-deblur_amd/dp.py b/3dgs-deblur_amd/dp.py
--- a/3dgs-deblur_amd/dp.py
+++ b/3dgs-deblur_amd/dp.py
@@ -96,6 +96,11 @@
             self._stream = ctypes.c_void_p(torch.cuda.current_stream(self.dev).cuda_stream)
             self._vp = ctypes.c_void_p
 
+    def _raw_write(self) -> None:
+        from . import ops
+        for g in self.grads:
+            ops.grad_pool_invalidate(g)
+
     def row_mask(self) -> torch.Tensor:
         if self.hip:
             mask = torch.empty(self.N, dtype=torch.uint8, device=self.dev)
@@ -146,6 +151,7 @@
     def scatter_add_payload(self, payload: torch.Tensor, cap: int, scale: float) -> None:
         if self.hip:
             payload = payload.contiguous()
+            self._raw_write()
             self._check(self._L.gs_dp_scatter_add_payload(cap, self._vp(payload.data_ptr()), len(self.grads), self._ptrs,
                                                           self._w, float(scale), self._stream), "dp_scatter_add_payload")
             return
@@ -156,6 +162,7 @@
         if M == 0:
             return
         if self.hip:
+            self._raw_write()
             self._check(self._L.gs_dp_scatter_add_rows(M, self._vp(payload.data_ptr()), len(self.grads), self._ptrs,
                                                        self._w, float(scale), self._stream), "dp_scatter_add_rows")
             return
diff --git a/3dgs-deblur_amd/ops.py b/3dgs-deblur_amd/ops.py
--- a/3dgs-deblur_amd/ops.py
+++ b/3dgs-deblur_amd/ops.py
@@ -572,6 +572,80 @@
 def release_arenas() -> None:
     with _state_lock:
         _arena_pool.clear()
+        _grad_pool.clear()
+
+
+GRAD_POOL = True
+_grad_pool = {}
+_GRAD_POOL_KEEP = 2
+
+
+def _storage_use_count(t: Tensor) -> int:
+    fn = getattr(torch._C, "_storage_Use_Count", None)
+    if fn is None:
+        return 1 << 30
+    return int(fn(t.untyped_storage()._cdata))
+
+
+_STORAGE_FREE = _storage_use_count(torch.empty(1))
+
+
+class _GradEntry:
+    __slots__ = ("pool_key", "shape_key", "flat", "dirty", "touched", "version", "valid")
+
+    def __init__(self, pool_key, shape_key, flat, dirty, touched):
+        self.pool_key, self.shape_key = pool_key, shape_key
+        self.flat, self.dirty, self.touched = flat, dirty, touched
+        self.version, self.valid = flat._version, False
+
+    def recyclable(self) -> bool:
+        return (self.valid and self.flat._version == self.version
+                and _storage_use_count(self.flat) <= _STORAGE_FREE)
+
+
+def _grad_pool_acquire(dev, N: int, P: int, K: int, split: bool, alloc=None) -> _GradEntry:
+    stream = torch.cuda.current_stream(dev).cuda_stream if torch.device(dev).type == "cuda" else 0
+    pool_key, shape_key = (str(dev), stream), (int(N), int(P), int(K), bool(split))
+    with _state_lock:
+        entries = _grad_pool.setdefault(pool_key, [])
+        hit = None
+        for e in list(entries):
+            if e.shape_key == shape_key and e.recyclable():
+                hit = hit or e
+            elif not e.valid or e.flat._version != e.version or e.shape_key != shape_key:
+                entries.remove(e)
+        if hit is not None:
+            entries.remove(hit)
+            hit.valid = False
+            return hit
+    n_flat = (3 + 3 + 4 + 1 + 3 * K) * N
+    if alloc is not None:
+        flat, dirty, touched = alloc(n_flat, N, P)
+    else:
+        flat = torch.empty(n_flat, device=dev)
+        dirty = torch.ones(N, dtype=torch.uint8, device=dev)
+        touched = torch.zeros(P * N, dtype=torch.uint8, device=dev)
+    return _GradEntry(pool_key, shape_key, flat, dirty, touched)
+
+
+def _grad_pool_commit(entry: _GradEntry) -> None:
+    with _state_lock:
+        entry.version, entry.valid = entry.flat._version, True
+        entries = _grad_pool.setdefault(entry.pool_key, [])
+        if entry not in entries:
+            entries.append(entry)
+        while len(entries) > _GRAD_POOL_KEEP:
+            entries.pop(0)
+
+
+def grad_pool_invalidate(t: Tensor) -> None:
+    ptr = t.untyped_storage().data_ptr()
+    with _state_lock:
+        for entries in _grad_pool.values():
+            for e in list(entries):
+                if e.flat.untyped_storage().data_ptr() == ptr:
+                    e.valid = False
+                    entries.remove(e)
 
 
 _pinned_cache = {}
@@ -937,11 +1011,11 @@
         V, lin, ang, times = ctx.saved_tensors
         P = times.numel()
         dev = V.device
-        acc = torch.zeros(22, device=dev)
+        acc = torch.empty(22, device=dev)
         v_V, v_lin, v_ang = acc[:16].view(4, 4), acc[16:19], acc[19:22]
-        _check(_L().gs_subpose_viewmats_bwd(P, _ptr(V), _ptr(lin), _ptr(ang), _ptr(times),
-                                            _ptr(v_out.contiguous().float()), _ptr(v_V), _ptr(v_lin), _ptr(v_ang),
-                                            _stream()), "subpose_viewmats_bwd")
+        _check(_L().gs_subpose_viewmats_bwd_store(P, _ptr(V), _ptr(lin), _ptr(ang), _ptr(times),
+                                                  _ptr(v_out.contiguous().float()), _ptr(v_V), _ptr(v_lin), _ptr(v_ang),
+                                                  _stream()), "subpose_viewmats_bwd_store")
         return v_V, v_lin, v_ang, None
 
 
@@ -1092,7 +1166,12 @@
         if backend is None:
             if rs is not None and R != 1:
                 raise ValueError("exact rolling shutter renders with rs_bands == 1")
-            if any(ctx.needs_input_grad):
+            if any(ctx.needs_input_grad) and GRAD_POOL and not pixvel:
+                entry = _grad_pool_acquire(dev, N, P, K, sh_rest is not None)
+                ctx.prealloc = {"entry": entry, "touched": entry.touched,
+                                "v_records": torch.empty(P * N, GRAD, device=dev),
+                                "pose_scratch": _pose_scratch(N, P, True, dev)}
+            elif any(ctx.needs_input_grad):
                 t_len = (P * N + 15) // 16 * 16
                 zbuf = torch.zeros(t_len + 4 * (16 * P + 12), dtype=torch.uint8, device=dev)
                 zf = zbuf[t_len:].view(torch.float32)
@@ -1203,7 +1282,11 @@
         all_tuples = ctx.frame is not None or all(sl["gi_of_e"] is not None for sl in ctx.slices)
         pre = ctx.prealloc if ctx.prealloc else {}
         ctx.prealloc = None
-        if all_tuples and "touched" in pre:
+        entry = None
+        if all_tuples and pre.get("entry") is not None and ctx.frame is not None:
+            entry = pre["entry"]
+            v_records, touched = pre["v_records"], entry.touched
+        elif all_tuples and "touched" in pre:
             v_records, touched = pre["v_records"], pre["touched"]
         elif all_tuples:
             v_records = torch.empty(P * N, GRAD, device=dev)
@@ -1224,7 +1307,7 @@
         sh_rest = ctx.sh_rest
         sizes = [3 * N, 3 * N, 4 * N, N] + ([3 * K * N] if sh_rest is None else [3 * N, 3 * (K - 1) * N])
         shapes = [(N, 3), (N, 3), (N, 4), (N,)] + ([(N, K, 3)] if sh_rest is None else [tuple(sh.shape), (N, K - 1, 3)])
-        flat = torch.empty(sum(sizes), device=dev)
+        flat = torch.empty(sum(sizes), device=dev) if entry is None else entry.flat
         outs = [t.view(shape) for t, shape in zip(flat.split(sizes), shapes)]
         v_means, v_scales, v_quats, v_opac, v_sh = outs[:5]
         v_sh_rest = outs[5] if sh_rest is not None else None
@@ -1254,6 +1337,16 @@
                        "project_pixvel_bwd")
                 if v_tw is not None:
                     v_lin, v_ang = v_tw[0:3], v_tw[3:6]
+            elif entry is not None:
+                v_V = torch.empty(P, 4, 4, device=dev) if need_v else None
+                _check(L.gs_project_fused_bwd_pooled(N, P, _ptr(means3d), _ptr(scales), glob, _ptr(quats),
+                                                     _ptr(opacities), _ptr(sh), K, deg, _ptr(V), fx, fy, cx, cy, H, W,
+                                                     clip, aa, _ptr(records), _ptr(v_records), _ptr(v_means),
+                                                     _ptr(v_scales), _ptr(v_quats), _ptr(v_opac), _ptr(v_sh), _ptr(v_V),
+                                                     _ptr(touched), _ptr(xy_out), _proj_grad_flags() | fill_flag | xy_cams,
+                                                     _ptr(sh_rest), pf, _ptr(v_sh_rest), _ptr(psc), psc_n, _stream(),
+                                                     _ptr(entry.dirty)), "project_fused_bwd_pooled")
+                _grad_pool_commit(entry)
             else:
                 v_V = (pre["v_V"].view(P, 4, 4) if "v_V" in pre else torch.zeros(P, 4, 4, device=dev)) if need_v else None
                 _check(L.gs_project_fused_bwd(N, P, _ptr(means3d), _ptr(scales), glob, _ptr(quats), _ptr(opacities),
diff --git a/include/gsdeblur.h b/include/gsdeblur.h
--- a/include/gsdeblur.h
+++ b/include/gsdeblur.h
@@ -15,6 +15,9 @@
 int gs_subpose_viewmats_bwd(int P, const float* viewmat, const float* lin_vel, const float* ang_vel,
                             const float* times, const float* v_out , float* v_viewmat,
                             float* v_lin, float* v_ang, void* stream);
+int gs_subpose_viewmats_bwd_store(int P, const float* viewmat, const float* lin_vel, const float* ang_vel,
+                                  const float* times, const float* v_out , float* v_viewmat,
+                                  float* v_lin, float* v_ang, void* stream);
 
 int gs_project_fwd(int N, const float* means3d , const float* scales , float glob_scale,
                    const float* quats , const float* viewmat , float fx, float fy,
@@ -66,6 +69,15 @@
                          void* pose_scratch ,
                          long long pose_scratch_bytes,
                          void* stream);
+int gs_project_fused_bwd_pooled(int N, int P, const float* means3d, const float* scales, float glob_scale,
+                                const float* quats, const float* opacities, const float* sh, int K_stride,
+                                int sh_degree, const float* viewmats, float fx, float fy, float cx, float cy,
+                                int img_height, int img_width, float clip_thresh, int antialiased,
+                                const float* records, const float* v_records, float* v_means3d, float* v_scales,
+                                float* v_quats, float* v_opacities, float* v_sh, float* v_viewmats,
+                                unsigned char* touched, float* v_xy_sum, int grad_flags, const float* sh_rest,
+                                int param_flags, float* v_sh_rest, void* pose_scratch, long long pose_scratch_bytes,
+                                void* stream, unsigned char* dirty );
 
 int gs_project_pixvel_fwd(int N, int P, const float* means3d, const float* scales, float glob_scale,
                           const float* quats, const float* opacities, const float* sh, int K_stride, int sh_degree,
```

New measurement: 1237 (median of 6 runs). +2.8%, better.
